# Genie-Kim/PintheMemory

Measured on AMD Instinct MI355X. Metric: train imgs/sec 768x768 bs=8 R50-DeepLabV3+ +mem, higher is better.
Workload: dtype f32

## Files before the change

### include/pinmem_hip.h

```cpp
#ifndef PINMEM_HIP_H
#define PINMEM_HIP_H
#include <stddef.h>
#include <stdint.h>

#ifdef __cplusplus
extern "C" {
#endif

typedef enum pm_status { PM_OK = 0, PM_EINVAL = -1, PM_EWORKSPACE = -2, PM_ELAUNCH = -3, PM_EUNSUPPORTED = -4 } pm_status;

typedef enum pm_dtype { PM_F32 = 0, PM_BF16 = 1 } pm_dtype;
#define PM_TF_ZERO_PAD64 1

typedef struct pm_tensor {
  void* ptr;
  int32_t n, h, w, c;
  int64_t pitch;
  int32_t dtype;
  int32_t flags;
} pm_tensor;

#define PM_ABI_VERSION 400

typedef struct pm_conv_params {
// ... 11 lines not shown
  int64_t struct_size;
  const float* bias;
  const float* scale;
  const float* shift;
  const float* residual;
  int64_t residual_pitch;
  int32_t relu;
  float* bn_partials;
  int64_t bn_partials_bytes;
} pm_conv_epilogue;

const char* pm_last_error(void);
int pm_version(void);

size_t pm_conv_workspace(const pm_tensor* x, const pm_tensor* y, const pm_conv_params* p, int which );
size_t pm_conv_winograd_v_bytes(const pm_tensor* x, const pm_tensor* y, const pm_conv_params* p);
size_t pm_conv_wxf_bytes(const pm_tensor* x, const pm_tensor* y, const pm_conv_params* p);
size_t pm_conv_wxf_bytes_dgrad(const pm_tensor* dy, const pm_tensor* dx, const pm_conv_params* p);
typedef struct pm_wxf_job {
  const float* w;
  void* wxf;
  int64_t wxf_bytes;
  int32_t cout, kh, kw, cin;
  int32_t dgrad;
  int32_t reserved;
} pm_wxf_job;
int pm_conv_wxf_refresh_bf16(const pm_wxf_job* jobs, int n, void* stream);
int pm_conv_wxf_refresh_f32(const pm_wxf_job* jobs, int n, void* stream);
size_t pm_conv_bn_partials_bytes(const pm_tensor* x, const pm_tensor* y, const pm_conv_params* p);
int pm_conv_fwd(const pm_tensor* x, const float* w_krsc, const pm_tensor* y, const pm_conv_params* p,
                const pm_conv_epilogue* ep, void* ws, size_t ws_bytes, void* stream);
int pm_conv_bwd_data(const pm_tensor* dy, const float* w_krsc, const pm_tensor* dx, const pm_conv_params* p,
                     const pm_tensor* add, void* ws, size_t ws_bytes, void* stream);
int pm_conv_bwd_weight(const pm_tensor* x, const pm_tensor* dy, float* dw_krsc, float* dbias, const pm_conv_params* p,
                       void* ws, size_t ws_bytes, void* stream);

typedef struct pm_routing {
  int32_t struct_size;
  int32_t winograd;
  int32_t winograd_fused;
  int32_t conv16;
  int32_t conv16_wide;
  int32_t conv16_persistent;
  int32_t wgrad16;
  int32_t bf16_wgrad;
  int32_t split;
} pm_routing;
int pm_routing_get(pm_routing* out);
int pm_routing_set(const pm_routing* r);


int pm_set_winograd(int mode);
int pm_set_winograd_fused(int on);
int pm_set_conv16(int on);
int pm_set_bf16_wgrad(int on);
int pm_set_wgrad16(int on);
int pm_set_split(int on);

int pm_profile_enable(int on);
int pm_profile_dump(const char* csv_path);
int pm_profile_read(int mode, int bm, int bn, int km, int nst, double* total_ms, double* total_flops, int64_t* launches, int clear);
int pm_profile_read_prec(int mode, int bm, int bn, int km, int nst, int prec, double* total_ms, double* total_flops, int64_t* launches, int clear);
int pm_profile_read_bytes(int mode, int bm, int bn, int km, int nst, int prec, double* total_bytes);

size_t pm_bn_workspace(const pm_tensor* x);
int pm_bn_stats(const pm_tensor* x, float* moments, void* ws, size_t ws_bytes, void* stream);
int pm_bn_stats_finalize(const pm_tensor* x, float eps, float* mean, float* invstd, float* running_mean , float* running_var ,
                         float momentum, void* ws, size_t ws_bytes, void* stream);
int pm_bn_merge(const float* parts, int world, int c, float* moments, void* stream);
int pm_bn_merge_finalize(const float* parts, int world, int c, float eps, float* mean, float* invstd, float* running_mean ,
                         float* running_var , float momentum, void* stream);
int pm_bn_finalize(const float* moments, int c, float eps, float* mean, float* invstd,
                   float* running_mean, float* running_var, float momentum, void* stream);
int pm_bn_apply(const pm_tensor* x, const float* mean, const float* invstd, const float* gamma, const float* beta,
                const pm_tensor* residual , int relu, const pm_tensor* y, void* stream);
int pm_bn_apply_mask(const pm_tensor* x, const float* mean, const float* invstd, const float* gamma, const float* beta,
                     const pm_tensor* residual , int relu, const pm_tensor* y, uint8_t* mask , void* stream);
int pm_bn_bwd_reduce_mask(const pm_tensor* dy, const uint8_t* mask, const pm_tensor* x, const float* mean, const float* invstd,
                          const pm_tensor* gmask , float* sums, void* ws, size_t ws_bytes, void* stream);
int pm_bn_bwd_reduce(const pm_tensor* dy, const pm_tensor* y , const pm_tensor* x, const float* mean, const float* invstd,
                     const float* gamma , const float* beta , int relu, const pm_tensor* gmask ,
                     float* sums, void* ws, size_t ws_bytes, void* stream);
int pm_bn_bwd_apply(const pm_tensor* dy, const pm_tensor* y , const pm_tensor* x, const float* mean, const float* invstd,
                    const float* gamma, const float* beta , const float* sums, float count, int relu, const pm_tensor* dx,
                    const pm_tensor* dres , void* stream);
int pm_bn_partials_finalize(const float* partials, int64_t pixels, int c, float eps, float* mean, float* invstd, float* running_mean ,
                            float* running_var , float momentum, float* moments , void* stream);
int pm_bn_fold(const float* gamma, const float* beta, const float* running_mean, const float* running_var, const float* conv_bias,
               int c, float eps, float* scale, float* shift, void* stream);
int pm_bn_fold_multi(const void* table, const int* cs, const int* offs, int n, int max_c, int total, float eps, float* arena, void* stream);
int pm_relu_bwd(const pm_tensor* dy, const pm_tensor* y, const pm_tensor* dx, void* stream);
int pm_add(const pm_tensor* a, const pm_tensor* b, const pm_tensor* y, void* stream);
int pm_add_n(const pm_tensor* const* xs, int n, const pm_tensor* y, void* stream);
int pm_copy(const pm_tensor* src, const pm_tensor* dst, void* stream);
int pm_scale_shift_act(const pm_tensor* x, const float* scale, const float* shift, const pm_tensor* residual, int relu,
                       const pm_tensor* y, void* stream);

int pm_cast(const pm_tensor* x, const pm_tensor* y, void* stream);

int pm_maxpool3x3s2_fwd(const pm_tensor* x, const pm_tensor* y, uint8_t* argmax, void* stream);
int pm_maxpool3x3s2_bwd(const pm_tensor* dy, const uint8_t* argmax, const pm_tensor* dx, void* stream);
int pm_global_avgpool_fwd(const pm_tensor* x, const pm_tensor* y , void* stream);
int pm_global_avgpool_bwd(const pm_tensor* dy, const pm_tensor* dx, int accumulate, void* stream);

int pm_resize_bilinear_fwd(const pm_tensor* x, const pm_tensor* y, void* stream);
int pm_resize_bilinear_bwd(const pm_tensor* dy, const pm_tensor* dx, int accumulate, void* stream);
size_t pm_resize_bilinear_bwd_workspace(const pm_tensor* dy, const pm_tensor* dx);
int pm_resize_bilinear_bwd_separable(const pm_tensor* dy, const pm_tensor* dx, int accumulate, void* ws, size_t ws_bytes, void* stream);

int pm_resize_bilinear_hp_fwd(const pm_tensor* x, const pm_tensor* y, int flip_w, void* stream);
int pm_softmax_mean_update(const pm_tensor* logits, double* buffer, int counter, void* stream);
int pm_sliding_stitch(const pm_tensor* logits, const int32_t* tiles_xyxy, int ntiles, int H, int W, int flip_w, double* acc, int accumulate, void* stream);
int pm_argmax_f64(const double* buffer, int n, int h, int w, int c, int64_t* out_cls, double* out_prob , void* stream);

int pm_image_u8_to_nhwc4(const uint8_t* img_nhw3, int64_t pixels, const float* mean3, const float* std3, float* out_nhwc4, void* stream);
int pm_labels_u8_to_i64(const uint8_t* lab, int64_t n, int64_t* out, void* stream);

int pm_nchw_to_nhwc(const float* x_nchw, int c_src, const pm_tensor* y, void* stream);
int pm_nhwc_to_nchw(const pm_tensor* x, float* y_nchw, void* stream);
int pm_label_nearest(const int64_t* lab, int n, int H, int W, int64_t* out, int h, int w, void* stream);

size_t pm_upsample_ce_workspace(int n, int H, int W);
int pm_upsample_ce_fwd(const pm_tensor* logits, float inv_temp, const int64_t* labels, int H, int W, float* loss_out,
                       void* ws, size_t ws_bytes, void* stream);
size_t pm_upsample_ce_bwd_workspace(const pm_tensor* logits, int H, int W);
int pm_upsample_ce_bwd(const pm_tensor* logits, float inv_temp, const int64_t* labels, int H, int W, const float* loss_out,
                       const float* gscale, const pm_tensor* dlogits, void* ws, size_t ws_bytes, void* stream);

size_t pm_upsample_ce_field_bytes(const pm_tensor* logits, int H, int W);
int pm_upsample_ce_fwd_field(const pm_tensor* logits, float inv_temp, const int64_t* labels, int H, int W, float* loss_out, float* field,
                             void* ws , size_t ws_bytes, void* stream);
int pm_upsample_ce_bwd_field(const pm_tensor* logits , float inv_temp, int H, int W, const float* loss_out, const float* gscale,
                             const float* field, const pm_tensor* dlogits, void* stream);

// ... 52 lines not shown
```

### pinthememory_amd/csrc/bn.hip

```cpp
#include "pm_common.h"

namespace {

constexpr int CB = 64;
constexpr int RL = 16;

__device__ __forceinline__ float bn_affine(float v, float mu, float is, float ga, float be) {
  const float s = is * ga;
  return fmaf(v, s, fmaf(-mu, s, be));
}

inline int chunk_rows(long P, int C) {
  const long colblocks = std::max<long>(1, (C + CB - 1) / CB);
  const long want = std::max<long>(512, 2048 / colblocks);
  long r = (P + want - 1) / want;
  r = std::max<long>(r, 64);
  return (int)((r + RL - 1) / RL * RL);
}

__global__ __launch_bounds__(256) void bn_stats_partial(const float* __restrict__ x, long pitch, long P, int C, int rows, float* __restrict__ part) {
  __shared__ float sm[RL][CB][2];
  const int g = threadIdx.x & 15, r = threadIdx.x >> 4;
  const int c = blockIdx.y * CB + g * 4;
  const long p0 = (long)blockIdx.x * rows, p1 = min(P, p0 + rows);
  float s1[4] = {0, 0, 0, 0}, s2[4] = {0, 0, 0, 0};
  if (c < C) {
    const float4 k = PM_LD4(x + c);
    for (long p = p0 + r; p < p1; p += RL) {
      const float4 v = PM_LD4(x + p * pitch + c);
      const float d0 = v.x - k.x, d1 = v.y - k.y, d2 = v.z - k.z, d3 = v.w - k.w;
      s1[0] += d0, s1[1] += d1, s1[2] += d2, s1[3] += d3;
      s2[0] += d0 * d0, s2[1] += d1 * d1, s2[2] += d2 * d2, s2[3] += d3 * d3;
    }
  }
#pragma unroll
  for (int j = 0; j < 4; ++j) sm[r][g * 4 + j][0] = s1[j], sm[r][g * 4 + j][1] = s2[j];
  __syncthreads();
  if (threadIdx.x < CB * 2) {
    const int cc = threadIdx.x >> 1, w = threadIdx.x & 1;
    float s = 0.f;
#pragma unroll
    for (int i = 0; i < RL; ++i) s += sm[i][cc][w];
    const int ch = blockIdx.y * CB + cc;
// ... 107 lines not shown
    float4 ga = make_float4(0.f, 0.f, 0.f, 0.f), be = ga;
    if (RELU == 2) ga = PM_LD4(gamma + c), be = PM_LD4(beta + c);
    for (long p = p0 + r; p < p1; p += RL) {
      float4 d = PM_LD4(dy + p * dpitch + c);
      const float4 v = PM_LD4(x + p * xpitch + c);
      if (RELU == 1) {
        const float4 o = PM_LD4(y + p * ypitch + c);
        d.x = o.x > 0.f ? d.x : 0.f, d.y = o.y > 0.f ? d.y : 0.f, d.z = o.z > 0.f ? d.z : 0.f, d.w = o.w > 0.f ? d.w : 0.f;
      } else if (RELU == 3) {
        const unsigned mb = reinterpret_cast<const unsigned char*>(y)[p * (C >> 2) + (c >> 2)];
        d.x = (mb & 1u) ? d.x : 0.f, d.y = (mb & 2u) ? d.y : 0.f, d.z = (mb & 4u) ? d.z : 0.f, d.w = (mb & 8u) ? d.w : 0.f;
      } else if (RELU == 2) {
        d.x = bn_affine(v.x, mu.x, is.x, ga.x, be.x) > 0.f ? d.x : 0.f, d.y = bn_affine(v.y, mu.y, is.y, ga.y, be.y) > 0.f ? d.y : 0.f;
        d.z = bn_affine(v.z, mu.z, is.z, ga.z, be.z) > 0.f ? d.z : 0.f, d.w = bn_affine(v.w, mu.w, is.w, ga.w, be.w) > 0.f ? d.w : 0.f;
      }
      if (GOUT) PM_ST4(gout + p * gpitch + c, d);
      s1[0] += d.x, s1[1] += d.y, s1[2] += d.z, s1[3] += d.w;
      s2[0] += d.x * ((v.x - mu.x) * is.x), s2[1] += d.y * ((v.y - mu.y) * is.y);
      s2[2] += d.z * ((v.z - mu.z) * is.z), s2[3] += d.w * ((v.w - mu.w) * is.w);
    }
  }
#pragma unroll
  for (int j = 0; j < 4; ++j) sm[r][g * 4 + j][0] = s1[j], sm[r][g * 4 + j][1] = s2[j];
  __syncthreads();
  if (threadIdx.x < CB * 2) {
    const int cc = threadIdx.x >> 1, w = threadIdx.x & 1;
    float s = 0.f;
#pragma unroll
    for (int i = 0; i < RL; ++i) s += sm[i][cc][w];
    const int ch = blockIdx.y * CB + cc;
    if (ch < C) part[((long)blockIdx.x * C + ch) * 2 + w] = s;
  }
}
__global__ __launch_bounds__(256) void bn_bwd_final(const float* __restrict__ part, int nb, int C, float* __restrict__ sums) {
  const int c = blockIdx.x * FC + (threadIdx.x & (FC - 1)), lane = threadIdx.x / FC;
  double s1, s2;
  final_sums(part, nb, C, c, lane, s1, s2);
  if (lane != 0 || c >= C) return;
  sums[c] = (float)s1;
  sums[C + c] = (float)s2;
}

template <bool FIN>
__global__ void bn_merge_kernel(const float* __restrict__ parts, int W, int C, float* __restrict__ out, float eps, float* __restrict__ mean,
                                float* __restrict__ invstd, float* running_mean, float* running_var, float momentum) {
  const int c = blockIdx.x * blockDim.x + threadIdx.x;
  if (c >= C) return;
  double n = 0.0, s = 0.0;
  for (int r = 0; r < W; ++r) {
    const double cnt = parts[(long)r * 3 * C + 2 * C + c];
    n += cnt, s += cnt * (double)parts[(long)r * 3 * C + c];
  }
  const double gmean = s / n;
  double m2d = 0.0;
  for (int r = 0; r < W; ++r) {
    const double cnt = parts[(long)r * 3 * C + 2 * C + c], d = (double)parts[(long)r * 3 * C + c] - gmean;
    m2d += (double)parts[(long)r * 3 * C + C + c] + cnt * d * d;
  }
  const float m = (float)gmean, m2 = (float)m2d, nf = (float)n;
  if constexpr (!FIN) {
    out[c] = m, out[C + c] = m2, out[2 * C + c] = nf;
  } else {
    const float var = m2 / nf;
    mean[c] = m;
    invstd[c] = 1.f / sqrtf(var + eps);
    if (running_mean) running_mean[c] = (1.f - momentum) * running_mean[c] + momentum * m;
// ... 96 lines not shown
extern "C" int pm_bn_partials_finalize(const float* partials, int64_t pixels, int c, float eps, float* mean, float* invstd, float* running_mean,
                                       float* running_var, float momentum, float* moments, void* stream) {
  PM_REQUIRE(partials && pixels > 0 && c > 0 && (moments || (mean && invstd)), PM_EINVAL, "bn_partials_finalize: bad args");
  PM_REQUIRE(moments || pixels > 1, PM_EINVAL, "bn_partials_finalize: expected more than 1 value per channel when training, got %ld", (long)pixels);
  hipStream_t st = (hipStream_t)stream;
  if (moments)
    hipLaunchKernelGGL(bn_partials_final<true>, dim3(pm_cdiv(c, FC)), dim3(256), 0, st, partials, (long)pixels, c, eps, (float*)nullptr, (float*)nullptr,
                       (float*)nullptr, (float*)nullptr, 0.f, moments);
  else
    hipLaunchKernelGGL(bn_partials_final<false>, dim3(pm_cdiv(c, FC)), dim3(256), 0, st, partials, (long)pixels, c, eps, mean, invstd, running_mean, running_var,
                       momentum, (float*)nullptr);
  return pm_check_launch("bn_partials_finalize");
}

extern "C" int pm_bn_fold(const float* gamma, const float* beta, const float* rm, const float* rv, const float* conv_bias, int c, float eps, float* scale,
                          float* shift, void* stream) {
  PM_REQUIRE(gamma && beta && rm && rv && scale && shift && c > 0, PM_EINVAL, "bn_fold: bad args");
  hipLaunchKernelGGL(bn_fold_kernel, dim3(pm_cdiv(c, 64)), dim3(64), 0, (hipStream_t)stream, gamma, beta, rm, rv, conv_bias, c, eps, scale, shift);
  return pm_check_launch("bn_fold");
}

extern "C" int pm_bn_fold_multi(const void* table, const int* cs, const int* offs, int n, int max_c, int total, float eps, float* arena, void* stream) {
  PM_REQUIRE(table && cs && offs && arena && n > 0 && max_c > 0 && total > 0, PM_EINVAL, "bn_fold_multi: bad args");
  hipLaunchKernelGGL(bn_fold_multi_kernel, dim3(n, pm_cdiv(max_c, 256)), dim3(256), 0, (hipStream_t)stream, (const unsigned long long*)table, cs, offs, total, eps,
                     arena);
  return pm_check_launch("bn_fold_multi");
}

extern "C" int pm_bn_apply(const pm_tensor* x, const float* mean, const float* invstd, const float* gamma, const float* beta, const pm_tensor* res,
                           int relu, const pm_tensor* y, void* stream) {
  return pm_bn_apply_mask(x, mean, invstd, gamma, beta, res, relu, y, nullptr, stream);
}

extern "C" int pm_bn_apply_mask(const pm_tensor* x, const float* mean, const float* invstd, const float* gamma, const float* beta, const pm_tensor* res,
                                int relu, const pm_tensor* y, uint8_t* mask, void* stream) {
  PM_REQUIRE(x && y, PM_EINVAL, "bn_apply: null");
  if (pm_is_bf16(x)) return pm16_bn_apply_mask(x, mean, invstd, gamma, beta, res, relu, y, mask, (hipStream_t)stream);
  if (int e = check_bn(x, "bn_apply")) return e;
  if (int e = check_bn(y, "bn_apply")) return e;
  PM_REQUIRE(pm_same_shape(x, y) && mean && invstd && gamma && beta, PM_EINVAL, "bn_apply: bad args");
  if (res) {
    if (int e = check_bn(res, "bn_apply")) return e;
    PM_REQUIRE(pm_same_shape(x, res), PM_EINVAL, "bn_apply: residual shape mismatch");
  }
  const float *px = (const float*)x->ptr, *pr = res ? (const float*)res->ptr : nullptr;
  float* py = (float*)y->ptr;
  const long a = x->pitch, b = res ? res->pitch : 0, c = y->pitch, cq = x->c >> 2;
  return pm_ew_launch(true, pm_pixels(x), x->c, (hipStream_t)stream, "bn_apply", [=] __device__(long p, int ch) {
    const float4 v = PM_LD4(px + p * a + ch), mu = PM_LD4(mean + ch), is = PM_LD4(invstd + ch), ga = PM_LD4(gamma + ch), be = PM_LD4(beta + ch);
    float4 o = make_float4(bn_affine(v.x, mu.x, is.x, ga.x, be.x), bn_affine(v.y, mu.y, is.y, ga.y, be.y), bn_affine(v.z, mu.z, is.z, ga.z, be.z),
                           bn_affine(v.w, mu.w, is.w, ga.w, be.w));
    if (pr) {
      const float4 q = PM_LD4(pr + p * b + ch);
      o.x += q.x, o.y += q.y, o.z += q.z, o.w += q.w;
    }
    if (mask) mask[p * cq + (ch >> 2)] = (unsigned char)((o.x > 0.f ? 1 : 0) | (o.y > 0.f ? 2 : 0) | (o.z > 0.f ? 4 : 0) | (o.w > 0.f ? 8 : 0));
    if (relu) o.x = fmaxf(o.x, 0.f), o.y = fmaxf(o.y, 0.f), o.z = fmaxf(o.z, 0.f), o.w = fmaxf(o.w, 0.f);
    PM_ST4(py + p * c + ch, o);
  });
}

extern "C" int pm_bn_bwd_reduce(const pm_tensor* dy, const pm_tensor* y, const pm_tensor* x, const float* mean, const float* invstd, const float* gamma,
                                const float* beta, int relu, const pm_tensor* gmask, float* sums, void* ws, size_t ws_bytes, void* stream) {
  PM_REQUIRE(dy && x, PM_EINVAL, "bn_bwd_reduce: null");
  PM_REQUIRE(relu >= 0 && relu <= 2, PM_EINVAL, "bn_bwd_reduce: relu mode %d (0 none, 1 mask from y, 2 mask rebuilt from x)", relu);
  if (pm_is_bf16(x)) return pm16_bn_bwd_reduce(dy, y, nullptr, x, mean, invstd, gamma, beta, relu, gmask, sums, ws, ws_bytes, (hipStream_t)stream);
  if (int e = check_bn(dy, "bn_bwd_reduce")) return e;
  if (int e = check_bn(x, "bn_bwd_reduce")) return e;
  PM_REQUIRE(pm_same_shape(dy, x) && mean && invstd && sums, PM_EINVAL, "bn_bwd_reduce: bad args");
  PM_REQUIRE(relu >= 0 && relu <= 2, PM_EINVAL, "bn_bwd_reduce: relu mode %d (0 none, 1 mask from y, 2 mask rebuilt from x)", relu);
  PM_REQUIRE(relu != 1 || (y && pm_vec4(y) && pm_same_shape(y, x)), PM_EINVAL, "bn_bwd_reduce: relu mode 1 needs the forward output");
  PM_REQUIRE(relu != 2 || (gamma && beta), PM_EINVAL, "bn_bwd_reduce: relu mode 2 needs gamma and beta");
  PM_REQUIRE(!gmask || (relu != 0 && pm_vec4(gmask) && pm_same_shape(gmask, x)), PM_EINVAL, "bn_bwd_reduce: gmask needs a ReLU mode and the shape of x");
  PM_REQUIRE(ws && ws_bytes >= pm_bn_workspace(x), PM_EWORKSPACE, "bn_bwd_reduce: workspace too small");
  const long P = pm_pixels(x);
  const int rows = chunk_rows(P, x->c), nb = pm_cdiv(P, rows);
  hipStream_t st = (hipStream_t)stream;
  dim3 grid(nb, pm_cdiv(x->c, CB));
  const float *pdy = (const float*)dy->ptr, *py = relu == 1 ? (const float*)y->ptr : nullptr, *px = (const float*)x->ptr;
  const long yp = relu == 1 ? y->pitch : 0;
  float* pg = gmask ? (float*)gmask->ptr : nullptr;
  const long gp = gmask ? gmask->pitch : 0;
#define PM_BN_BWD_PARTIAL(R, G)                                                                                                                         \
  hipLaunchKernelGGL((bn_bwd_partial<R, G>), grid, dim3(256), 0, st, pdy, (long)dy->pitch, py, yp, px, (long)x->pitch, mean, invstd, gamma, beta, pg, gp, P, \
                     x->c, rows, (float*)ws)
  if (relu == 0) PM_BN_BWD_PARTIAL(0, false);
  else if (relu == 1 && gmask) PM_BN_BWD_PARTIAL(1, true);
  else if (relu == 1) PM_BN_BWD_PARTIAL(1, false);
  else if (gmask) PM_BN_BWD_PARTIAL(2, true);
  else PM_BN_BWD_PARTIAL(2, false);
#undef PM_BN_BWD_PARTIAL
  hipLaunchKernelGGL(bn_bwd_final, dim3(pm_cdiv(x->c, FC)), dim3(256), 0, st, (const float*)ws, nb, x->c, sums);
// ... 37 lines not shown
  PM_REQUIRE(relu != 1 || (y && pm_vec4(y) && pm_same_shape(y, x)), PM_EINVAL, "bn_bwd_apply: relu mode 1 needs the forward output");
  PM_REQUIRE(relu != 2 || beta, PM_EINVAL, "bn_bwd_apply: relu mode 2 needs beta");
  PM_REQUIRE(!dres || (pm_vec4(dres) && pm_same_shape(dres, x)), PM_EINVAL, "bn_bwd_apply: dres shape mismatch");
  const float *pd = (const float*)dy->ptr, *po = relu == 1 ? (const float*)y->ptr : nullptr, *px = (const float*)x->ptr;
  float *pdx = (float*)dx->ptr, *pdr = dres ? (float*)dres->ptr : nullptr;
  const long a = dy->pitch, b = relu == 1 ? y->pitch : 0, c = x->pitch, d = dx->pitch, e2 = dres ? dres->pitch : 0;
  const bool from_x = relu == 2;
  const int C = x->c;
  const bool dev_count = !(count > 0.f);
  const float host_inv_n = dev_count ? 0.f : 1.f / count;
  return pm_ew_launch(true, pm_pixels(x), C, (hipStream_t)stream, "bn_bwd_apply", [=] __device__(long p, int ch) {
    const float inv_n = dev_count ? 1.f / sums[2 * C] : host_inv_n;
    float4 g = PM_LD4(pd + p * a + ch);
    if (po) {
      const float4 o = PM_LD4(po + p * b + ch);
      g.x = o.x > 0.f ? g.x : 0.f, g.y = o.y > 0.f ? g.y : 0.f, g.z = o.z > 0.f ? g.z : 0.f, g.w = o.w > 0.f ? g.w : 0.f;
    }
    const float4 v = PM_LD4(px + p * c + ch), mu = PM_LD4(mean + ch), is = PM_LD4(invstd + ch), ga = PM_LD4(gamma + ch);
    if (from_x) {
      const float4 be = PM_LD4(beta + ch);
      g.x = bn_affine(v.x, mu.x, is.x, ga.x, be.x) > 0.f ? g.x : 0.f, g.y = bn_affine(v.y, mu.y, is.y, ga.y, be.y) > 0.f ? g.y : 0.f;
      g.z = bn_affine(v.z, mu.z, is.z, ga.z, be.z) > 0.f ? g.z : 0.f, g.w = bn_affine(v.w, mu.w, is.w, ga.w, be.w) > 0.f ? g.w : 0.f;
    }
    if (pdr) PM_ST4(pdr + p * e2 + ch, g);
    const float4 s1 = PM_LD4(sums + ch), s2 = PM_LD4(sums + C + ch);
    float4 r;
    r.x = (g.x - s1.x * inv_n - (v.x - mu.x) * is.x * (s2.x * inv_n)) * (is.x * ga.x);
    r.y = (g.y - s1.y * inv_n - (v.y - mu.y) * is.y * (s2.y * inv_n)) * (is.y * ga.y);
    r.z = (g.z - s1.z * inv_n - (v.z - mu.z) * is.z * (s2.z * inv_n)) * (is.z * ga.z);
    r.w = (g.w - s1.w * inv_n - (v.w - mu.w) * is.w * (s2.w * inv_n)) * (is.w * ga.w);
    PM_ST4(pdx + p * d + ch, r);
  });
}
```

### pinthememory_amd/csrc/conv_igemm.hip

```cpp
#include <stdlib.h>
#include <algorithm>
#include <type_traits>
#include <vector>

#include "pm_common.h"

#include "conv_igemm_kernel.h"

namespace {

template <int ZL, bool O16 = false>
__global__ __launch_bounds__(256) void splitk_reduce_vec_kernel(const float* __restrict__ ws, int ksplit, long slab, int M, int Nn,
                                                                float* __restrict__ C, long c_pitch, const float* bias,
                                                                const float* scale, const float* shift, const float* residual,
                                                                long res_pitch, int relu) {
  constexpr int GP = 256 / ZL;
  __shared__ float4 red[ZL > 1 ? ZL : 1][GP];
  const int gl = threadIdx.x % GP, zl = threadIdx.x / GP;
  const long groups = (long)M * Nn / 4;
  for (long g0 = (long)blockIdx.x * GP; g0 < groups; g0 += (long)gridDim.x * GP) {
    const long grp = g0 + gl;
    float4 v = make_float4(0.f, 0.f, 0.f, 0.f);
    if (grp < groups)
#pragma unroll 8
      for (int z = zl; z < ksplit; z += ZL) {
        const float4 q = PM_LD4(ws + (long)z * slab + grp * 4);
        v.x += q.x, v.y += q.y, v.z += q.z, v.w += q.w;
      }
    if constexpr (ZL > 1) {
      red[zl][gl] = v;
      __syncthreads();
      if (zl == 0) {
#pragma unroll
        for (int l = 1; l < ZL; ++l) {
          const float4 q = red[l][gl];
          v.x += q.x, v.y += q.y, v.z += q.z, v.w += q.w;
        }
      }
    }
    if (zl == 0 && grp < groups) {
      const long i = grp * 4;
      const int row = (int)(i / Nn), col = (int)(i - (long)row * Nn);
      if (bias) {
        const float4 b = PM_LD4(bias + col);
        v.x += b.x, v.y += b.y, v.z += b.z, v.w += b.w;
      }
      if (scale) {
        const float4 sc = PM_LD4(scale + col), sh = PM_LD4(shift + col);
        v.x = v.x * sc.x + sh.x, v.y = v.y * sc.y + sh.y, v.z = v.z * sc.z + sh.z, v.w = v.w * sc.w + sh.w;
      }
      if (residual) {
        if constexpr (O16) {
          const uint2 q = *reinterpret_cast<const uint2*>(reinterpret_cast<const pm_bf16*>(residual) + (long)row * res_pitch + col);
          v.x += __uint_as_float(q.x << 16), v.y += __uint_as_float(q.x & 0xffff0000u), v.z += __uint_as_float(q.y << 16), v.w += __uint_as_float(q.y & 0xffff0000u);
        } else {
          const float4 r = PM_LD4(residual + (long)row * res_pitch + col);
          v.x += r.x, v.y += r.y, v.z += r.z, v.w += r.w;
        }
      }
      if (relu) v.x = fmaxf(v.x, 0.f), v.y = fmaxf(v.y, 0.f), v.z = fmaxf(v.z, 0.f), v.w = fmaxf(v.w, 0.f);
      if constexpr (O16) *reinterpret_cast<uint2*>(reinterpret_cast<pm_bf16*>(C) + (long)row * c_pitch + col) = make_uint2(pm_pack_bf16(v.x, v.y), pm_pack_bf16(v.z, v.w));
      else PM_ST4(C + (long)row * c_pitch + col, v);
    }
    if constexpr (ZL > 1) __syncthreads();
  }
}

__global__ __launch_bounds__(256) void splitk_reduce_kernel(const float* __restrict__ ws, int ksplit, long slab, int M, int Nn,
                                                            float* __restrict__ C, long c_pitch, const float* bias,
                                                            const float* scale, const float* shift, const float* residual,
                                                            long res_pitch, int relu) {
  const long total = (long)M * Nn;
  for (long i = (long)blockIdx.x * 256 + threadIdx.x; i < total; i += (long)gridDim.x * 256) {
    const int row = (int)(i / Nn), col = (int)(i - (long)row * Nn);
    float v = 0.f;
    for (int z = 0; z < ksplit; ++z) v += ws[(long)z * slab + i];
    if (bias) v += bias[col];
    if (scale) v = v * scale[col] + shift[col];
    if (residual) v += residual[(long)row * res_pitch + col];
    if (relu) v = fmaxf(v, 0.f);
    C[(long)row * c_pitch + col] = v;
  }
}

int splitk_reduce(const float* ws, int ksplit, long M, long Nn, float* C, long c_pitch, const float* bias, const float* scale, const float* shift,
                  const float* residual, long res_pitch, int relu, hipStream_t st, bool out16 = false) {
  const long total = M * Nn;
  if (out16) {
    PM_REQUIRE((Nn % 4 == 0) && (c_pitch % 4 == 0) && (res_pitch % 4 == 0) && pm_aligned16(ws) && (reinterpret_cast<uintptr_t>(C) & 7) == 0 &&
                   (reinterpret_cast<uintptr_t>(residual) & 7) == 0 && (!bias || pm_aligned16(bias)) && (!scale || (pm_aligned16(scale) && pm_aligned16(shift))),
               PM_EUNSUPPORTED, "splitk_reduce(bf16): unaligned output");
    const long groups = total / 4;
    const int zl = (ksplit >= 32 && groups < (1 << 18)) ? 16 : (ksplit >= 8 && groups < (1 << 20) ? 4 : 1);
    const int nb = (int)std::min<long>((groups + 256 / zl - 1) / (256 / zl), 8192);
    if (zl == 16)
      hipLaunchKernelGGL((splitk_reduce_vec_kernel<16, true>), dim3(nb), dim3(256), 0, st, ws, ksplit, total, (int)M, (int)Nn, C, c_pitch, bias, scale, shift, residual, res_pitch, relu);
    else if (zl == 4)
      hipLaunchKernelGGL((splitk_reduce_vec_kernel<4, true>), dim3(nb), dim3(256), 0, st, ws, ksplit, total, (int)M, (int)Nn, C, c_pitch, bias, scale, shift, residual, res_pitch, relu);
    else
      hipLaunchKernelGGL((splitk_reduce_vec_kernel<1, true>), dim3(nb), dim3(256), 0, st, ws, ksplit, total, (int)M, (int)Nn, C, c_pitch, bias, scale, shift, residual, res_pitch, relu);
    return pm_check_launch("splitk_reduce(bf16)");
  }
  const bool vec = (Nn % 4 == 0) && (c_pitch % 4 == 0) && (res_pitch % 4 == 0) && pm_aligned16(ws) && pm_aligned16(C) &&
                   (!bias || pm_aligned16(bias)) && (!scale || (pm_aligned16(scale) && pm_aligned16(shift))) && (!residual || pm_aligned16(residual));
  if (!vec) {
    const int nb = (int)std::min<long>((total + 255) / 256, 4096);
    hipLaunchKernelGGL(splitk_reduce_kernel, dim3(nb), dim3(256), 0, st, ws, ksplit, total, (int)M, (int)Nn, C, c_pitch, bias, scale, shift, residual,
                       res_pitch, relu);
  } else {
    const long groups = total / 4;
    const int zl = (ksplit >= 32 && groups < (1 << 18)) ? 16 : (ksplit >= 8 && groups < (1 << 20) ? 4 : 1);
    const int gp = 256 / zl;
    const int nb = (int)std::min<long>((groups + gp - 1) / gp, 8192);
    if (zl == 16)
      hipLaunchKernelGGL(splitk_reduce_vec_kernel<16>, dim3(nb), dim3(256), 0, st, ws, ksplit, total, (int)M, (int)Nn, C, c_pitch, bias, scale, shift, residual, res_pitch, relu);
    else if (zl == 4)
      hipLaunchKernelGGL(splitk_reduce_vec_kernel<4>, dim3(nb), dim3(256), 0, st, ws, ksplit, total, (int)M, (int)Nn, C, c_pitch, bias, scale, shift, residual, res_pitch, relu);
    else
      hipLaunchKernelGGL(splitk_reduce_vec_kernel<1>, dim3(nb), dim3(256), 0, st, ws, ksplit, total, (int)M, (int)Nn, C, c_pitch, bias, scale, shift, residual, res_pitch, relu);
  }
  return pm_check_launch("splitk_reduce");
}

inline int colsum_rows(long P, int C) {
  const long col_blocks = std::max<long>(1, (C + 63) / 64);
  const long want = col_blocks == 1 ? 256 : std::max<long>(1, 1024 / col_blocks);
  return (int)std::min<long>(2048, std::max<long>(64, (P + want - 1) / want));
}

__global__ __launch_bounds__(256) void colsum_partial_kernel(const float* __restrict__ x, long pitch, long P, int C, int rows_per_block,
                                                             float* __restrict__ part) {
  __shared__ float sm[4][64];
  const int c = blockIdx.y * 64 + (threadIdx.x & 63), r = threadIdx.x >> 6;
  const long p0 = (long)blockIdx.x * rows_per_block, p1 = min(P, p0 + rows_per_block);
  float s = 0.f;
  if (c < C)
    for (long p = p0 + r; p < p1; p += 4) s += x[p * pitch + c];
  sm[r][threadIdx.x & 63] = s;
  __syncthreads();
  if (r == 0 && c < C) part[(long)blockIdx.x * C + c] = sm[0][threadIdx.x] + sm[1][threadIdx.x] + sm[2][threadIdx.x] + sm[3][threadIdx.x];
}
__global__ __launch_bounds__(256) void colsum_partial_narrow_kernel(const float* __restrict__ x, int p4, long P, int C, int rows_per_block,
                                                                    float* __restrict__ part) {
  __shared__ float4 sm[256];
  const int RL = 256 / p4, t = threadIdx.x;
  const int g = t % p4, rl = t / p4;
  const long p0 = (long)blockIdx.x * rows_per_block, p1 = min(P, p0 + rows_per_block);
  float4 s = make_float4(0.f, 0.f, 0.f, 0.f);
  if (rl < RL)
    for (long p = p0 + rl; p < p1; p += RL) {
      const float4 v = PM_LD4(x + (p * p4 + g) * 4);
      s.x += v.x, s.y += v.y, s.z += v.z, s.w += v.w;
// ... 193 lines not shown
  }
  void done() {
    if (!g_prof_on) return;
    (void)hipEventRecord(rec.b, st);
    g_prof.push_back(rec);
  }
};

inline bool split_takes(int mode, const Plan& p, const ConvK& k, int batch) {
  return pm_route.split != 0 && p.bn >= 64 && !k.io16 && (batch > 1 || split_k_ok(mode, k.K));
}

template <int MODE>
int launch(const ConvK& k0, const Plan& p, hipStream_t st, int batch = 1, double flops = -1.0) {
  ConvK k = k0;
  k.tiles_m = p.tiles_m;
  k.tiles_n = p.tiles_n;
  k.ksplit = p.ksplit;
  k.kper = p.kper;
  dim3 grid(p.tiles_m * p.tiles_n, batch, p.ksplit);
  if (batch != 1) k.stage_ep = 0;
  if (k.prec == 0 && split_takes(MODE, p, k, batch)) k.prec = 5;
  {
    const int units = batch * p.ksplit, rem = units & 7, ntile = p.tiles_m * p.tiles_n;
    k.batch_xcd = units >= 8 && (rem == 0 || ((rem == 1 || rem == 2 || rem == 4) && ntile % (8 / rem) == 0));
  }
  const int km = (MODE == MODE_WGRAD && k.kmode == K_FAST) ? K_MID : ((k.prec == 5 && MODE != MODE_WGRAD && k.kmode == K_FAST && k.kh * k.kw == 1 && k.stride == 1 && k.pad == 0 && !k.sub) ? K_PW : k.kmode);
  ProfScope prof(st, MODE, p.bm, p.bn, km, k.prec, lds_stages(MODE, k.kmode, p.bn, k.kper), k.M, k.Nn, k.K, batch, p.ksplit,
                 flops >= 0.0 ? flops : 2.0 * (double)k.M * (double)k.Nn * (double)k.K * batch,
                 (double)batch * ((double)k.a_bytes + (double)k.b_bytes + ((k.io16 && p.ksplit == 1) ? 2.0 : 4.0) * (double)k.M * (double)k.Nn * (double)p.ksplit));
  if constexpr (MODE != MODE_WGRAD) {
    if (pm_route.split && (k.prec == 0 || k.prec == 5) && !k.io16 && batch == 1 && p.ksplit == 1 && !k.stats && k.kh * k.kw == 1 && k.stride == 1 && k.pad == 0 && !k.sub) {
      pm_gemm_pw g;
      g.A = k.A, g.B = k.B, g.C = k.C, g.bias = k.bias, g.scale = k.scale, g.shift = k.shift, g.residual = k.residual;
      g.a_pitch = MODE == MODE_FWD ? k.x_pitch : k.y_pitch, g.c_pitch = k.c_pitch, g.res_pitch = k.res_pitch;
      g.b_sn = MODE == MODE_FWD ? k.K : 1, g.b_sk = MODE == MODE_FWD ? 1 : k.Nn;
      g.M = k.M, g.Nn = k.Nn, g.K = k.K, g.relu = k.relu;
      if (pm_pwstream_ok(&g)) {
        prof.rec.bm = 32, prof.rec.bn = 64, prof.rec.km = 4, prof.rec.prec = 5, prof.rec.nst = 0;
        const int e = pm_pwstream_launch(&g, st);
        prof.done();
        return e;
      }
    }
  }
  constexpr bool akc = MODE != MODE_WGRAD, bkc = MODE == MODE_FWD;
  if (k.prec == 5) {
    if (int e = pm_conv_split_launch(MODE, p.bm, p.bn, k, grid.x, grid.y, grid.z, pm_conv_split_stage_bytes(MODE, p.bm, p.bn), st)) return e;
    prof.rec.nst = 1;
    prof.done();
    return pm_check_launch("conv_split");
  }
  const bool tr = MODE == MODE_WGRAD && (k.prec == 3 || k.prec == 4) && p.bn >= 64;
  auto smem = [&](int bm, int bn) {
    if (tr) return (size_t)2 * ((k.prec == 4 ? 2 : 1) * BK * (bm + 32) + (k.prec == 4 ? 2 : 1) * BK * (bn + 32)) * 2;
    return (size_t)2 * ((akc ? bm * LDK : BK * bm) + (bkc ? bn * LDK : BK * bn)) * sizeof(float);
  };
  if (p.bm == 64) {
    if (p.bn == 128) launch_one<MODE, 64, 128, 2, 2>(k, grid, smem(64, 128), st);
    else launch_one<MODE, 64, 64, 2, 2>(k, grid, smem(64, 64), st);
  } else if (p.bn == 128) {
    launch_one<MODE, 128, 128, 2, 2>(k, grid, smem(128, 128), st);
  } else if (p.bn == 64) {
    launch_one<MODE, 128, 64, 2, 2>(k, grid, smem(128, 64), st);
  } else {
    launch_one<MODE, 128, 32, 4, 1>(k, grid, smem(128, 32), st);
  }
// ... 2 lines not shown
}

int check_common(const pm_tensor* x, const pm_tensor* y, const pm_conv_params* p) {
  PM_REQUIRE(x && y && p && x->ptr && y->ptr, PM_EINVAL, "conv: null tensor");
  PM_REQUIRE(p->struct_size == (int32_t)sizeof(pm_conv_params), PM_EINVAL, "conv: pm_conv_params.struct_size %d != %zu -- caller built against another pinmem_hip.h (library ABI %d)",
             p->struct_size, sizeof(pm_conv_params), PM_ABI_VERSION);
  PM_REQUIRE(p->kh >= 1 && p->kw >= 1 && p->dil >= 1 && p->pad >= 0, PM_EINVAL, "conv: bad geometry");
  PM_REQUIRE(p->stride == 1 || p->stride == 2, PM_EUNSUPPORTED, "conv: stride %d unsupported (1 or 2)", p->stride);
  const int ho = (x->h + 2 * p->pad - p->dil * (p->kh - 1) - 1) / p->stride + 1;
  const int wo = (x->w + 2 * p->pad - p->dil * (p->kw - 1) - 1) / p->stride + 1;
  PM_REQUIRE(ho == y->h && wo == y->w && x->n == y->n, PM_EINVAL, "conv: output %dx%d does not match geometry (%dx%d)", y->h, y->w, ho, wo);
  PM_REQUIRE((x->dtype == PM_F32 || x->dtype == PM_BF16) && (y->dtype == PM_F32 || y->dtype == PM_BF16), PM_EUNSUPPORTED, "conv: dtype %d / %d", x->dtype, y->dtype);
  for (const pm_tensor* t : {x, y}) {
    if (pm_is_bf16(t)) PM_REQUIRE(pm_vec8(t), PM_EINVAL, "conv: bf16 tensors must be 16B aligned with pitch %% 8 == 0 and channels %% 8 == 0");
    else PM_REQUIRE(pm_vec_ok(t), PM_EINVAL, "conv: tensors must be 16B aligned with pitch %% 4 == 0");
  }
  PM_REQUIRE(x->c % 4 == 0, PM_EUNSUPPORTED, "conv: Cin %% 4 != 0 unsupported (pad the input channels)");
  PM_REQUIRE((y->c % 4 == 0) || (p->kh * p->kw == 1), PM_EUNSUPPORTED, "conv: Cout %% 4 != 0 only for 1x1");
  PM_REQUIRE(x->pitch >= x->c && y->pitch >= y->c, PM_EINVAL, "conv: pitch < channels");
  PM_REQUIRE(pm_pixels(x) * x->pitch < (1ll << 29) && pm_pixels(y) * y->pitch < (1ll << 29) && (int64_t)y->c * x->c * p->kh * p->kw < (1ll << 29),
             PM_EUNSUPPORTED, "conv: tensor too large for 32-bit byte offsets (2 GiB per tensor)");
  return PM_OK;
}

void fill_geom(ConvK& k, const pm_tensor* x, const pm_tensor* y, const pm_conv_params* p) {
  k.N = x->n, k.H = x->h, k.W = x->w, k.Cin = x->c, k.x_pitch = x->pitch;
  k.Ho = y->h, k.Wo = y->w, k.Cout = y->c, k.y_pitch = y->pitch;
  k.kh = p->kh, k.kw = p->kw, k.stride = p->stride, k.pad = p->pad, k.dil = p->dil;
  k.sshift = p->stride == 2 ? 1 : 0;
  k.prec = p->prec != 0 ? 1 : 0;
  k.T_eff = p->kh * p->kw, k.tk_w = p->kw, k.ky0 = k.kx0 = 0, k.ksy = k.ksx = 1;
  k.sub = k.sub_cy = k.sub_cx = 0, k.Hc = x->h, k.Wc = x->w;
  k.bias = k.scale = k.shift = k.residual = nullptr;
  k.res_pitch = 0, k.relu = 0, k.stats = nullptr, k.io16 = 0;
  k.stage_ep = 1;
  k.spl_prio = 1;
  k.n_group = 8;
  k.batch_xcd = 0;
  k.a_bs = k.b_bs = k.c_bs = 0;
}

struct WinoPlan {
  bool use;
  pm_wino_geom g;
  int Kp, P;
  size_t v_bytes, m_bytes, u_bytes;
  Plan pl;
};
inline bool wino_wgrad_pays(int cin, int cout) { return (long)cin * cout >= 256 * 256; }
WinoPlan wino_plan(const pm_tensor* xin, int cout, const pm_conv_params* p, bool wgrad = false) {
  WinoPlan wp{};
  if (wgrad && !wino_wgrad_pays(xin->c, cout)) return wp;
  if (pm_route.winograd == 0 || p->kh != 3 || p->kw != 3 || p->stride != 1 || p->pad != p->dil || p->prec != 0) return wp;
  const int cin = xin->c;
  if (cin < 128 || cout < 128 || (cout & 3) || (cin & 3)) return wp;
  int m = 0;
  double best_ratio = 0.6;
  for (int cand = pm_route.winograd; cand >= 2; cand -= 2) {
    const pm_wino_geom g = pm_wino_make_geom(xin->n, xin->h, xin->w, p->dil, cand);
    const double cover = (double)(cand * g.TY * p->dil) * (double)(cand * g.TX * p->dil) / ((double)xin->h * xin->w);
    const double ratio = cover * (cand + 2) * (cand + 2) / (9.0 * cand * cand);
    if (ratio <= best_ratio) best_ratio = ratio, m = cand, wp.g = g;
  }
  if (!m) return wp;
  wp.P = (m + 2) * (m + 2);
  wp.Kp = (cin + BK - 1) / BK * BK;
  if (wp.g.tiles * (long)std::max(wp.Kp, cout) * 4 >= (1ll << 31)) return wp;
// ... 463 lines not shown

int dgrad_s2_parity(const pm_tensor* dy0, const float* w, const pm_tensor* dx, const pm_conv_params* p, const pm_tensor* add, const ConvRoute& r, void* ws, hipStream_t st) {
  pm_tensor dy32;
  if (int e = upcast(dy0, (char*)ws + r.dy32_off, &dy32, st)) return e;
  const pm_tensor* dy = &dy32;
  float* tmp = (float*)((char*)ws + r.class_off);
  float* slab = (float*)((char*)ws + r.slab_off);
  for (int cls = 0; cls < 4; ++cls) {
    if (!r.s2p.valid[cls]) continue;
    const S2Class& c = r.s2p.c[cls];
    const Plan& pl = r.s2p.pl[cls];
    ConvK k;
    fill_geom(k, dx, dy, p);
    k.A = (const float*)dy->ptr, k.B = w;
    k.M = (int)c.M, k.Nn = dx->c, k.K = c.nky * c.nkx * dy->c;
    k.a_bytes = (unsigned)(pm_pixels(dy) * dy->pitch * 4), k.b_bytes = (unsigned)((long)dy->c * p->kh * p->kw * dx->c * 4);
    k.kmode = dy->c >= BK ? K_MID : K_SMALL;
    k.T_eff = c.nky * c.nkx, k.tk_w = c.nkx, k.ky0 = c.ky0, k.kx0 = c.kx0, k.ksy = c.ksy, k.ksx = c.ksx;
    k.sub = 1, k.sub_cy = c.cy, k.sub_cx = c.cx, k.Hc = c.Hc, k.Wc = c.Wc;
    float* out = (float*)((char*)tmp + cls * r.s2p.tmp_bytes);
    if (pl.ksplit > 1) {
      k.C = slab, k.c_pitch = dx->c, k.c_split = c.M * dx->c;
      if (int e = launch<MODE_DGRAD>(k, pl, st)) return e;
      if (int e = splitk_reduce(slab, pl.ksplit, c.M, dx->c, out, (long)dx->c, nullptr, nullptr, nullptr, nullptr, 0l, 0, st)) return e;
    } else {
      k.C = out, k.c_pitch = dx->c, k.c_split = 0;
      if (int e = launch<MODE_DGRAD>(k, pl, st)) return e;
    }
  }
  return s2_interleave(tmp, (long)(r.s2p.tmp_bytes / sizeof(float)), r.s2p.valid, dx, add, st, "dgrad_s2_interleave");
}

template <int MODE>
int conv_direct(const pm_tensor* x, const pm_tensor* y, const float* w, const pm_conv_params* p, const Plan& pl, const pm_conv_epilogue& e, void* ws, hipStream_t st) {
  const pm_tensor *xin = MODE == MODE_FWD ? x : y, *out = MODE == MODE_FWD ? y : x;
  long M, Nn, K;
  gemm_dims(MODE, x, y, p, M, Nn, K);
  ConvK k;
  fill_geom(k, x, y, p);
  k.io16 = pm_is_bf16(out) ? 1 : 0;
  k.A = (const float*)xin->ptr, k.B = w;
  k.M = (int)M, k.Nn = (int)Nn, k.K = (int)K;
  k.a_bytes = (unsigned)(pm_pixels(xin) * xin->pitch * 4), k.b_bytes = (unsigned)((long)y->c * p->kh * p->kw * x->c * 4);
  k.kmode = (xin->c % BK == 0 && (MODE == MODE_FWD || p->stride == 1)) ? 0 : (xin->c >= BK ? 1 : 2);
  if (pl.ksplit > 1) {
    k.C = (float*)ws, k.c_pitch = Nn, k.c_split = M * Nn;
    if (int err = launch<MODE>(k, pl, st)) return err;
    return splitk_reduce((const float*)ws, pl.ksplit, M, Nn, (float*)out->ptr, (long)out->pitch, e.bias, e.scale, e.shift, e.residual, (long)e.residual_pitch, e.relu, st, k.io16 != 0);
  }
  k.C = (float*)out->ptr, k.c_pitch = out->pitch, k.c_split = 0;
  k.bias = e.bias, k.scale = e.scale, k.shift = e.shift, k.residual = e.residual, k.res_pitch = e.residual_pitch, k.relu = e.relu;
  k.stats = e.bn_partials;
  return launch<MODE>(k, pl, st);
}

int conv_wgrad_direct(const pm_tensor* x, const pm_tensor* dy, float* dw, const pm_conv_params* p, const ConvRoute& r, void* ws, hipStream_t st) {
  long M, Nn, K;
  gemm_dims(MODE_WGRAD, x, dy, p, M, Nn, K);
  if (r.w16.use) {
    pm_wgrad16 w16 = r.w16.k;
    w16.C = w16.ksplit > 1 ? (float*)ws : dw;
    ProfScope prof(st, MODE_WGRAD, w16.bm, w16.bn, 2, 4, 3, M, Nn, K, 1, w16.ksplit, 2.0 * (double)M * (double)Nn * (double)K);
    const int e = pm_wgrad16_launch(&w16, st);
    prof.done();
    if (e || w16.ksplit == 1) return e;
    return splitk_reduce((const float*)ws, w16.ksplit, M, Nn, dw, (long)Nn, nullptr, nullptr, nullptr, nullptr, 0l, 0, st);
  }
  ConvK k;
  fill_geom(k, x, dy, p);
  if (p->prec == 2) k.prec = 3;
  if (r.native16) {
    PM_REQUIRE(x->c % 8 == 0 && dy->c % 8 == 0 && r.pl.bn >= 64, PM_EUNSUPPORTED, "conv_bwd_weight(bf16): channels %% 8 != 0 or a tile narrower than 64");
    k.prec = 4;
  }
  const int esz = r.native16 ? 2 : 4;
  k.A = (const float*)dy->ptr, k.B = (const float*)x->ptr;
  k.M = (int)M, k.Nn = (int)Nn, k.K = (int)K;
  k.a_bytes = (unsigned)(pm_pixels(dy) * dy->pitch * esz), k.b_bytes = (unsigned)(pm_pixels(x) * x->pitch * esz), k.kmode = dy->w >= (r.native16 ? 2 * BK : BK) ? 1 : 2;
  k.C = r.pl.ksplit > 1 ? (float*)ws : dw, k.c_pitch = Nn, k.c_split = r.pl.ksplit > 1 ? M * Nn : 0;
  if (int e = launch<MODE_WGRAD>(k, r.pl, st)) return e;
  if (r.pl.ksplit == 1) return PM_OK;
  return splitk_reduce((const float*)ws, r.pl.ksplit, M, Nn, dw, (long)Nn, nullptr, nullptr, nullptr, nullptr, 0l, 0, st);
}

// ... 165 lines not shown
  const pm_conv_params* p = &tp;
  PM_REQUIRE(!ep || ep->struct_size == (int64_t)sizeof(pm_conv_epilogue), PM_EINVAL,
             "conv_fwd: pm_conv_epilogue.struct_size %ld != %zu -- caller built against another pinmem_hip.h (library ABI %d)", ep ? (long)ep->struct_size : 0l,
             sizeof(pm_conv_epilogue), PM_ABI_VERSION);
  PM_REQUIRE(w && pm_aligned16(w), PM_EINVAL, "conv_fwd: weight null or unaligned");
  pm_conv_epilogue e0 = {(int64_t)sizeof(pm_conv_epilogue), nullptr, nullptr, nullptr, nullptr, 0, 0};
  if (ep) e0 = *ep;
  PM_REQUIRE((e0.scale == nullptr) == (e0.shift == nullptr), PM_EINVAL, "conv_fwd: scale and shift go together");
  const ConvRoute r = route_conv(MODE_FWD, x, y, p);
  if (e0.bn_partials) {
    PM_REQUIRE(!e0.relu && !e0.residual, PM_EINVAL, "conv_fwd: bn_partials are the statistics of the convolution output (no residual / ReLU)");
    PM_REQUIRE(r.bn_bytes != 0 && (size_t)e0.bn_partials_bytes >= r.bn_bytes, PM_EINVAL, "conv_fwd: this call cannot emit bn_partials (ask pm_conv_bn_partials_bytes): %zu needed", r.bn_bytes);
  }
  PM_REQUIRE(ws_bytes >= r.ws_bytes && (ws || r.ws_bytes == 0), PM_EWORKSPACE, "conv_fwd: workspace %zu < %zu", ws_bytes, r.ws_bytes);
  hipStream_t st = (hipStream_t)stream;
  switch (r.kind) {
    case R_WINO: {
      float* keep = (p->wino_v && (size_t)p->wino_v_bytes >= r.wino.v_bytes) ? (float*)p->wino_v : nullptr;
      float* uext = (p->wxf && (size_t)p->wxf_bytes >= r.wino.u_bytes) ? (float*)p->wxf : nullptr;
      return wino_conv(x, w, y->c, x->c, false, y, r.wino, e0, ws, st, keep, uext, p->wxf_valid != 0);
    }
    case R_BF16: {
      char* wext = (p->wxf && (size_t)p->wxf_bytes >= r.b16.wb_bytes) ? (char*)p->wxf : nullptr;
      return conv_bf16(x, w, y->c, x->c, false, y, &r.pe, r.b16, e0, ws, st, wext, p->wxf_valid != 0);
    }
    default:
      PM_REQUIRE(pm_is_f32(x), PM_EUNSUPPORTED, "conv_fwd: a bf16 input needs at least 32 channels (got %d)", x->c);
      return conv_direct<MODE_FWD>(x, y, w, p, r.pl, e0, ws, st);
  }
}

extern "C" int pm_conv_bwd_data(const pm_tensor* dy, const float* w, const pm_tensor* dx, const pm_conv_params* p0, const pm_tensor* add,
                                void* ws, size_t ws_bytes, void* stream) {
  if (int e = check_common(dx, dy, p0)) return e;
  const pm_conv_params tp = tier_params(p0, dy, dx);
  const pm_conv_params* p = &tp;
  PM_REQUIRE(!add || (add->ptr && pm_same_shape(add, dx) && add->dtype == dx->dtype), PM_EINVAL, "conv_bwd_data: `add` must match dx (shape and dtype)");
  PM_REQUIRE(!add || !pm_is_bf16(add) || pm_vec8(add), PM_EINVAL, "conv_bwd_data: bf16 `add` must be 16B aligned with pitch %% 8 == 0");
  PM_REQUIRE(w && pm_aligned16(w), PM_EINVAL, "conv_bwd_data: weight null or unaligned");
  const ConvRoute r = route_conv(MODE_DGRAD, dx, dy, p);
  PM_REQUIRE(ws_bytes >= r.ws_bytes && (ws || r.ws_bytes == 0), PM_EWORKSPACE, "conv_bwd_data: workspace %zu < %zu", ws_bytes, r.ws_bytes);
  hipStream_t st = (hipStream_t)stream;
  const pm_conv_epilogue e1 = {(int64_t)sizeof(pm_conv_epilogue), nullptr, nullptr, nullptr, add ? (const float*)add->ptr : nullptr, add ? add->pitch : 0, 0};
  switch (r.kind) {
    case R_S2_NATIVE: return dgrad_s2_bf16(dy, w, dx, p, add, r.s2n, ws, st);
    case R_S2_PARITY: return dgrad_s2_parity(dy, w, dx, p, add, r, ws, st);
    case R_BF16: {
      char* wext = (p->wxf && (size_t)p->wxf_bytes >= r.b16.wb_bytes) ? (char*)p->wxf : nullptr;
      return conv_bf16(dy, w, dy->c, dx->c, true, dx, &r.pe, r.b16, e1, ws, st, wext, p->wxf_valid != 0);
    }
    case R_WINO: return wino_conv(dy, w, dy->c, dx->c, true, dx, r.wino, e1, ws, st);
    default:
      PM_REQUIRE(pm_is_f32(dy), PM_EUNSUPPORTED, "conv_bwd_data: a bf16 dy needs at least 32 channels and a stride-1 geometry the forward form covers");
      return conv_direct<MODE_DGRAD>(dx, dy, w, p, r.pl, e1, ws, st);
  }
}

extern "C" int pm_conv_bwd_weight(const pm_tensor* x0, const pm_tensor* dy0, float* dw, float* dbias, const pm_conv_params* p0, void* ws,
                                  size_t ws_bytes, void* stream) {
  if (int e = check_common(x0, dy0, p0)) return e;
  const pm_conv_params tp = tier_params(p0, x0, dy0);
  const pm_conv_params* p = &tp;
  PM_REQUIRE(dw && pm_aligned16(dw), PM_EINVAL, "conv_bwd_weight: dw null or unaligned");
  const ConvRoute r = route_conv(MODE_WGRAD, x0, dy0, p);
  PM_REQUIRE(ws && ws_bytes >= r.ws_bytes, PM_EWORKSPACE, "conv_bwd_weight: workspace %zu < %zu", ws_bytes, r.ws_bytes);
  hipStream_t st = (hipStream_t)stream;
  const pm_tensor *x = x0, *dy = dy0;
  pm_tensor x32, dy32;
  if (!r.native16 && pm_is_bf16(x0)) {
    if (int e = upcast(x0, (char*)ws + r.x32_off, &x32, st)) return e;
    x = &x32;
  }
  if (pm_is_bf16(dy0) && (!r.native16 || dbias)) {
    if (int e = upcast(dy0, (char*)ws + r.dy32_off, &dy32, st)) return e;
    if (!r.native16) dy = &dy32;
  }
  int e;
  switch (r.kind) {
    case R_BF16_WGRAD: e = conv_wgrad_bf16(x, dy, dw, p, r.b16w, ws, st); break;
    case R_WINO_WGRAD: e = wino_wgrad(x, dy, dw, r.wino, r.wino_w, ws, st, (p->wino_v && (size_t)p->wino_v_bytes >= r.wino.v_bytes) ? (float*)p->wino_v : nullptr); break;
    default: e = conv_wgrad_direct(x, dy, dw, p, r, ws, st);
  }
  if (e || !dbias) return e;
  const pm_tensor* dyb = pm_is_bf16(dy0) ? &dy32 : dy0;
  const long P = pm_pixels(dyb);
  const int rpb = colsum_rows(P, dyb->c), nb = pm_cdiv(P, rpb);
  float* part = (float*)((char*)ws + r.bias_off);
// ... 8 lines not shown
```

### pinthememory_amd/csrc/conv_igemm_kernel.h

```cpp
#pragma once
#include <stdint.h>
#include <type_traits>

#include "pm_common.h"

typedef float f32x16 __attribute__((ext_vector_type(16)));
typedef __bf16 bf16x8 __attribute__((ext_vector_type(8)));

struct ConvK {
  const float* A;
  const float* B;
  float* C;
  int N, H, W, Cin;
  int Ho, Wo, Cout;
  long x_pitch, y_pitch;
  int kh, kw, stride, pad, dil, sshift;
  int M, Nn, K;
  int ksplit;
  int kper;
  long c_pitch;
  long c_split;
  long a_bs, b_bs, c_bs;
  int tiles_m, tiles_n;
  unsigned a_bytes, b_bytes;
  int kmode;
  int prec;
  int T_eff, tk_w, ky0, kx0, ksy, ksx;
  int sub, sub_cy, sub_cx, Hc, Wc;
  const float* bias;
  const float* scale;
  const float* shift;
  const float* residual;
  long res_pitch;
  int relu;
  float* stats;
  int io16;
  int stage_ep;
  int n_group;
  int batch_xcd;
  int spl_prio;
};

int pm_conv_split_launch(int mode, int bm, int bn, const ConvK& k, unsigned gx, unsigned gy, unsigned gz, size_t smem, hipStream_t st);
size_t pm_conv_split_stage_bytes(int mode, int bm, int bn);

namespace {

enum { MODE_FWD = 0, MODE_DGRAD = 1, MODE_WGRAD = 2 };
constexpr int BK = 32;
constexpr int LDK = 36;


typedef float v4f __attribute__((ext_vector_type(4)));
constexpr int OOB = 0x7fffffff;

__device__ __forceinline__ float4 bload(__amdgpu_buffer_rsrc_t r, int off) {
  const v4f v = __builtin_bit_cast(v4f, __builtin_amdgcn_raw_buffer_load_b128(r, off, 0, 0));
  return make_float4(v.x, v.y, v.z, v.w);
}

__device__ __forceinline__ int xcd_remap(int bid, int nwg) {
  const int q = nwg >> 3, r = nwg & 7, xcd = bid & 7, idx = bid >> 3;
  const int base = xcd < r ? xcd * (q + 1) : r * (q + 1) + (xcd - r) * q;
  return base + idx;
}

// ... 762 lines not shown
  const bool vec = a.stage_ep && ((a.c_pitch | a.Nn | (a.residual ? a.res_pitch : 0)) & 3) == 0 &&
                   ((reinterpret_cast<uintptr_t>(Cb) | reinterpret_cast<uintptr_t>(a.residual)) & 15) == 0;
  if (vec) {
    constexpr int WC = BN / WN, LDC = WC + 4, LPR = WC / 4, RPI = 64 / LPR;
    static_assert(32 % RPI == 0, "row segments must tile the 32-row slab");
    __syncthreads();
    float* Ws = smem + wave * 32 * LDC;
    const int rr0 = lane / LPR, cc = (lane % LPR) * 4;
    const int col = n0 + wn * WC + cc;
    const bool cok = col < a.Nn;
    const bool aff = !plain && (a.bias || a.scale), res = !plain && a.residual, relu = !plain && a.relu;
    float bi[4] = {0.f, 0.f, 0.f, 0.f}, sc[4] = {1.f, 1.f, 1.f, 1.f}, sh[4] = {0.f, 0.f, 0.f, 0.f};
    if (aff && cok) {
#pragma unroll
      for (int e = 0; e < 4; ++e) {
        if (a.bias) bi[e] = a.bias[col + e];
        if (a.scale) sc[e] = a.scale[col + e], sh[e] = a.shift[col + e];
      }
    }
#pragma unroll
    for (int i = 0; i < TM; ++i) {
#pragma unroll
      for (int n = 0; n < TN; ++n)
#pragma unroll
        for (int q = 0; q < 16; ++q) Ws[((q & 3) + 8 * (q >> 2) + 4 * half) * LDC + n * 32 + l31] = acc[i][n][q];
#pragma unroll
      for (int r0 = 0; r0 < 32; r0 += RPI) {
        const int rr = r0 + rr0;
        const long row = m0 + wm * (BM / WM) + i * 32 + rr;
        float4 v = *reinterpret_cast<const float4*>(Ws + rr * LDC + cc);
        if (row < a.M && cok) {
          if (aff) v.x = (v.x + bi[0]) * sc[0] + sh[0], v.y = (v.y + bi[1]) * sc[1] + sh[1], v.z = (v.z + bi[2]) * sc[2] + sh[2], v.w = (v.w + bi[3]) * sc[3] + sh[3];
          if (res) {
            const float4 qv = PM_LD4(a.residual + row * a.res_pitch + col);
            v.x += qv.x, v.y += qv.y, v.z += qv.z, v.w += qv.w;
          }
          if (relu) v.x = fmaxf(v.x, 0.f), v.y = fmaxf(v.y, 0.f), v.z = fmaxf(v.z, 0.f), v.w = fmaxf(v.w, 0.f);
          PM_ST4(Cb + row * a.c_pitch + col, v);
        }
      }
      if constexpr (STATS) {
        const long slab_row0 = m0 + wm * (BM / WM) + i * 32;
        const float cnt = (float)max(0l, min(32l, (long)a.M - slab_row0));
        auto slab_row = [&](int r0, bool& rok) {
          float4 v = *reinterpret_cast<const float4*>(Ws + (r0 + rr0) * LDC + cc);
          v.x = (v.x + bi[0]) * sc[0] + sh[0], v.y = (v.y + bi[1]) * sc[1] + sh[1], v.z = (v.z + bi[2]) * sc[2] + sh[2], v.w = (v.w + bi[3]) * sc[3] + sh[3];
          rok = slab_row0 + r0 + rr0 < a.M;
          return v;
        };
        float s1[4] = {0.f, 0.f, 0.f, 0.f};
#pragma unroll
        for (int r0 = 0; r0 < 32; r0 += RPI) {
          bool rok;
          const float4 v = slab_row(r0, rok);
          s1[0] += rok ? v.x : 0.f, s1[1] += rok ? v.y : 0.f, s1[2] += rok ? v.z : 0.f, s1[3] += rok ? v.w : 0.f;
        }
#pragma unroll
        for (int o = LPR; o < 64; o <<= 1)
#pragma unroll
          for (int e = 0; e < 4; ++e) s1[e] += __shfl_xor(s1[e], o, 64);
        float mu[4], m2[4] = {0.f, 0.f, 0.f, 0.f};
#pragma unroll
        for (int e = 0; e < 4; ++e) mu[e] = cnt > 0.f ? s1[e] / cnt : 0.f;
#pragma unroll
        for (int r0 = 0; r0 < 32; r0 += RPI) {
          bool rok;
          const float4 v = slab_row(r0, rok);
// ... 82 lines not shown
```

### pinthememory_amd/csrc/pm_common.h

```cpp
#pragma once
#include <hip/hip_runtime.h>
#include <algorithm>
#include <atomic>
#include <stdarg.h>
#include <stdint.h>
#include <stdio.h>

#include "../../include/pinmem_hip.h"

void pm_set_error(const char* fmt, ...);

#define PM_REQUIRE(cond, code, ...)      \
  do {                                   \
    if (!(cond)) {                       \
      pm_set_error(__VA_ARGS__);         \
      return (code);                     \
    }                                    \
  } while (0)

static inline int pm_check_launch(const char* what) {
  hipError_t e = hipGetLastError();
  if (e != hipSuccess) {
    pm_set_error("%s: launch failed: %s", what, hipGetErrorString(e));
    return PM_ELAUNCH;
// ... 77 lines not shown
  int relu;
  float* stats;
  int bm, bn, tiles_m, tiles_n, ksplit, ksteps_per;
  long c_split;
  int wide;
};
void pm_conv16_plan(pm_conv16* k);
int pm_conv16w_launch(const pm_conv16* k, hipStream_t st);
int pm_conv16w_persistent(const pm_conv16* k);
size_t pm_conv16_slab_bytes(const pm_conv16* k);
double pm_conv16_executed_fraction(const pm_conv16* k);
int pm_conv16_launch(const pm_conv16* k, hipStream_t st);

struct pm_wgrad16 {
  const pm_bf16* X;
  const pm_bf16* DY;
  float* C;
  int N, H, W, Ho, Wo;
  long x_pitch, dy_pitch;
  int Cin, Cout, kh, kw, stride, pad, dil;
  int M, Nn, P;
  int kper, ksplit;
  long c_split;
  int bm, bn, tiles_m, tiles_n;
};
bool pm_wgrad16_plan(pm_wgrad16* k);
int pm_wgrad16_launch(const pm_wgrad16* k, hipStream_t st);

struct pm_gemm_pw {
  const float* A;
  const float* B;
  float* C;
  const float *bias, *scale, *shift, *residual;
  long a_pitch, c_pitch, res_pitch;
  int b_sn, b_sk;
  long M;
  int Nn, K, relu;
};
bool pm_pwstream_ok(const pm_gemm_pw* g);
int pm_pwstream_launch(const pm_gemm_pw* g, hipStream_t st);

constexpr int PM_MAX_DEVICES = 64;
inline int pm_device_cus(int dev) {
  static std::atomic<int> cached[PM_MAX_DEVICES];
  const bool keep = dev >= 0 && dev < PM_MAX_DEVICES;
  int n = keep ? cached[dev].load(std::memory_order_relaxed) : 0;
  if (n > 0) return n;
  if (hipDeviceGetAttribute(&n, hipDeviceAttributeMultiprocessorCount, dev) != hipSuccess || n <= 0) n = 256;
  if (keep) cached[dev].store(n, std::memory_order_relaxed);
  return n;
}
struct pm_lds_optin {
  std::atomic<bool> done[PM_MAX_DEVICES] = {};
  int operator()(const void* kernel, int lds_bytes) {
    int dev = 0;
    if (hipGetDevice(&dev) != hipSuccess) dev = 0;
    const bool keep = dev >= 0 && dev < PM_MAX_DEVICES;
    if (!keep || !done[dev].load(std::memory_order_acquire)) {
      if (hipFuncSetAttribute(kernel, hipFuncAttributeMaxDynamicSharedMemorySize, lds_bytes) != hipSuccess) (void)hipGetLastError();
      else if (keep) done[dev].store(true, std::memory_order_release);
    }
    return pm_device_cus(dev);
  }
};

extern pm_routing pm_route;
// ... 34 lines not shown
  };
#pragma unroll
  for (int r0 = 0; r0 < 32; r0 += RPI) {
    float v[8];
    const bool rok = slab_row(r0, v);
#pragma unroll
    for (int e = 0; e < 8; ++e) s1[e] += rok ? v[e] : 0.f;
  }
#pragma unroll
  for (int o = LPR; o < 64; o <<= 1)
#pragma unroll
    for (int e = 0; e < 8; ++e) s1[e] += __shfl_xor(s1[e], o, 64);
#pragma unroll
  for (int e = 0; e < 8; ++e) mu[e] = cnt > 0.f ? s1[e] / cnt : 0.f;
#pragma unroll
  for (int r0 = 0; r0 < 32; r0 += RPI) {
    float v[8];
    const bool rok = slab_row(r0, v);
#pragma unroll
    for (int e = 0; e < 8; ++e) {
      const float d = v[e] - mu[e];
      m2[e] += rok ? d * d : 0.f;
    }
  }
#pragma unroll
  for (int o = LPR; o < 64; o <<= 1)
#pragma unroll
    for (int e = 0; e < 8; ++e) m2[e] += __shfl_xor(m2[e], o, 64);
  if (rr0 == 0 && cok && cnt > 0.f) {
    float* dst = stats + ((slab_row0 >> 5) * Nn + col) * 2;
#pragma unroll
    for (int e = 0; e < 8; e += 2) *reinterpret_cast<float4*>(dst + 2 * e) = make_float4(mu[e], m2[e], mu[e + 1], m2[e + 1]);
  }
}

__device__ __forceinline__ float pm_wave_sum(float v) {
#pragma unroll
  for (int o = 32; o > 0; o >>= 1) v += __shfl_xor(v, o, 64);
  return v;
}
__device__ __forceinline__ float pm_wave_max(float v) {
#pragma unroll
  for (int o = 32; o > 0; o >>= 1) v = fmaxf(v, __shfl_xor(v, o, 64));
  return v;
}

struct pm_lerp {
  int i0, i1;
  float w0, w1;
};
__host__ __device__ __forceinline__ float pm_ac_scale(int in, int out) {
  return out > 1 ? (float)(in - 1) / (float)(out - 1) : 0.f;
}
__device__ __forceinline__ pm_lerp pm_ac_lerp(float scale, int dst, int in) {
  float src = scale * (float)dst;
  int i0 = (int)src;
  if (i0 > in - 1) i0 = in - 1;
  int i1 = i0 + (i0 < in - 1 ? 1 : 0);
  float l1 = src - (float)i0;
  if (l1 < 0.f) l1 = 0.f;
  if (l1 > 1.f) l1 = 1.f;
  pm_lerp r;
  r.i0 = i0;
  r.i1 = i1;
  r.w1 = l1;
  r.w0 = 1.f - l1;
// ... 26 lines not shown
```

### pinthememory_amd/csrc/pool_resize.hip

```cpp
#include "pm_common.h"

namespace {

template <bool VEC>
__global__ __launch_bounds__(256) void maxpool_fwd_kernel(const float* __restrict__ x, long xp, int H, int W, float* __restrict__ y, long yp, int Ho,
                                                          int Wo, int C, long total, uint8_t* __restrict__ arg) {
  constexpr int V = VEC ? 4 : 1;
  const int cg = C / V;
  for (long i = (long)blockIdx.x * 256 + threadIdx.x; i < total; i += (long)gridDim.x * 256) {
    const long op = i / cg;
    const int ch = (int)(i - op * cg) * V;
    const int ox = (int)(op % Wo), oy = (int)((op / Wo) % Ho), n = (int)(op / ((long)Wo * Ho));
    float best[V];
    uint8_t bi[V];
#pragma unroll
    for (int v = 0; v < V; ++v) best[v] = -INFINITY, bi[v] = 0;
    bool first = true;
#pragma unroll
    for (int ky = 0; ky < 3; ++ky) {
      const int iy = oy * 2 - 1 + ky;
      if ((unsigned)iy >= (unsigned)H) continue;
#pragma unroll
      for (int kx = 0; kx < 3; ++kx) {
        const int ix = ox * 2 - 1 + kx;
        if ((unsigned)ix >= (unsigned)W) continue;
        const float* p = x + ((long)(n * H + iy) * W + ix) * xp + ch;
        float v[V];
        if constexpr (VEC) {
          const float4 q = PM_LD4(p);
          v[0] = q.x;
          if (V > 1) v[1 % V] = q.y, v[2 % V] = q.z, v[3 % V] = q.w;
        } else {
          v[0] = *p;
        }
#pragma unroll
        for (int e = 0; e < V; ++e)
          if (first || v[e] > best[e] || v[e] != v[e]) best[e] = v[e], bi[e] = (uint8_t)(ky * 3 + kx);
        first = false;
      }
    }
    float* o = y + op * yp + ch;
    uint8_t* a = arg + op * C + ch;
#pragma unroll
    for (int e = 0; e < V; ++e) o[e] = best[e], a[e] = bi[e];
  }
}

__global__ __launch_bounds__(256) void maxpool_bwd_vec_kernel(const float* __restrict__ dy, long dp, int Ho, int Wo, const uint8_t* __restrict__ arg,
                                                              float* __restrict__ dx, long xp, int H, int W, int C, long total) {
  const int cg = C >> 2;
  for (long i = (long)blockIdx.x * 256 + threadIdx.x; i < total; i += (long)gridDim.x * 256) {
    const long ip = i / cg;
    const int ch = (int)(i - ip * cg) * 4;
    const int ix = (int)(ip % W), iy = (int)((ip / W) % H), n = (int)(ip / ((long)W * H));
    float4 g = make_float4(0.f, 0.f, 0.f, 0.f);
    const int oy_hi = min((iy + 1) >> 1, Ho - 1), ox_hi = min((ix + 1) >> 1, Wo - 1);
    for (int oy = iy >> 1; oy <= oy_hi; ++oy) {
      const int ky = iy + 1 - 2 * oy;
      if (ky < 0 || ky > 2) continue;
      for (int ox = ix >> 1; ox <= ox_hi; ++ox) {
        const int kx = ix + 1 - 2 * ox;
        if (kx < 0 || kx > 2) continue;
        const long op = (long)(n * Ho + oy) * Wo + ox;
        const unsigned a = *reinterpret_cast<const unsigned*>(arg + op * C + ch), want = (unsigned)(ky * 3 + kx);
        const float4 d = PM_LD4(dy + op * dp + ch);
        g.x += (a & 255u) == want ? d.x : 0.f;
        g.y += ((a >> 8) & 255u) == want ? d.y : 0.f;
        g.z += ((a >> 16) & 255u) == want ? d.z : 0.f;
        g.w += (a >> 24) == want ? d.w : 0.f;
      }
    }
    PM_ST4(dx + ip * xp + ch, g);
  }
}

__global__ __launch_bounds__(256) void maxpool_bwd_kernel(const float* __restrict__ dy, long dp, int Ho, int Wo, const uint8_t* __restrict__ arg,
                                                          float* __restrict__ dx, long xp, int H, int W, int C, long total) {
  for (long i = (long)blockIdx.x * 256 + threadIdx.x; i < total; i += (long)gridDim.x * 256) {
    const long ip = i / C;
    const int ch = (int)(i - ip * C);
    const int ix = (int)(ip % W), iy = (int)((ip / W) % H), n = (int)(ip / ((long)W * H));
    float g = 0.f;
    const int oy_hi = min((iy + 1) >> 1, Ho - 1), ox_hi = min((ix + 1) >> 1, Wo - 1);
    for (int oy = max(iy >> 1, 0); oy <= oy_hi; ++oy) {
      const int ky = iy + 1 - 2 * oy;
      if (ky < 0 || ky > 2) continue;
      for (int ox = max(ix >> 1, 0); ox <= ox_hi; ++ox) {
        const int kx = ix + 1 - 2 * ox;
        if (kx < 0 || kx > 2) continue;
        const long op = (long)(n * Ho + oy) * Wo + ox;
        if (arg[op * C + ch] == (uint8_t)(ky * 3 + kx)) g += dy[op * dp + ch];
      }
    }
    dx[ip * xp + ch] = g;
  }
}

__global__ __launch_bounds__(256) void gap_fwd_kernel(const float* __restrict__ x, long xp, long HW, int C, float* __restrict__ y, long yp, float scale,
                                                      int accumulate) {
  __shared__ float sm[16][64];
  const int g = threadIdx.x & 15, r = threadIdx.x >> 4;
  const int c = blockIdx.y * 64 + g * 4, n = blockIdx.x;
  float s[4] = {0, 0, 0, 0};
  if (c < C) {
// ... 221 lines not shown
    for (int Y = ylo; Y <= yhi; ++Y) {
      const float wy = tap_weight(pm_ac_lerp(sy, Y, h), y);
      if (wy == 0.f) continue;
      const float4 q = PM_LD4(T + (((long)n * H + Y) * w + x) * C + ch);
      g.x += wy * q.x, g.y += wy * q.y, g.z += wy * q.z, g.w += wy * q.w;
    }
    float* o = dx + ip * xp + ch;
    if (accumulate) {
      const float4 q = PM_LD4(o);
      g.x += q.x, g.y += q.y, g.z += q.z, g.w += q.w;
    }
    PM_ST4(o, g);
  }
}

}

extern "C" int pm_maxpool3x3s2_fwd(const pm_tensor* x, const pm_tensor* y, uint8_t* argmax, void* stream) {
  PM_REQUIRE(x && y && argmax && x->ptr && y->ptr, PM_EINVAL, "maxpool_fwd: null");
  PM_REQUIRE(y->h == (x->h + 2 - 3) / 2 + 1 && y->w == (x->w + 2 - 3) / 2 + 1 && x->n == y->n && x->c == y->c, PM_EINVAL, "maxpool_fwd: shape mismatch");
  if (pm_is_bf16(x) && pm_is_bf16(y)) return pm16_maxpool_fwd(x, y, argmax, (hipStream_t)stream);
  PM_REQUIRE_F32(x, "maxpool_fwd"); PM_REQUIRE_F32(y, "maxpool_fwd");
  const bool v = pm_vec4(x) && pm_vec4(y);
  const long total = pm_pixels(y) * (v ? y->c / 4 : y->c);
  if (v)
    hipLaunchKernelGGL(maxpool_fwd_kernel<true>, dim3(grid_for(total)), dim3(256), 0, (hipStream_t)stream, (const float*)x->ptr, (long)x->pitch, x->h, x->w,
                       (float*)y->ptr, (long)y->pitch, y->h, y->w, y->c, total, argmax);
  else
    hipLaunchKernelGGL(maxpool_fwd_kernel<false>, dim3(grid_for(total)), dim3(256), 0, (hipStream_t)stream, (const float*)x->ptr, (long)x->pitch, x->h, x->w,
                       (float*)y->ptr, (long)y->pitch, y->h, y->w, y->c, total, argmax);
  return pm_check_launch("maxpool_fwd");
}

extern "C" int pm_maxpool3x3s2_bwd(const pm_tensor* dy, const uint8_t* argmax, const pm_tensor* dx, void* stream) {
  PM_REQUIRE(dy && dx && argmax && dy->ptr && dx->ptr && dy->n == dx->n && dy->c == dx->c, PM_EINVAL, "maxpool_bwd: bad args");
  if (pm_is_bf16(dy) && pm_is_bf16(dx)) return pm16_maxpool_bwd(dy, argmax, dx, (hipStream_t)stream);
  PM_REQUIRE_F32(dy, "maxpool_bwd"); PM_REQUIRE_F32(dx, "maxpool_bwd");
  const long total = pm_pixels(dx) * dx->c;
  if (pm_vec4(dy) && pm_vec4(dx) && (reinterpret_cast<uintptr_t>(argmax) & 3u) == 0)
    hipLaunchKernelGGL(maxpool_bwd_vec_kernel, dim3(grid_for(total / 4)), dim3(256), 0, (hipStream_t)stream, (const float*)dy->ptr, (long)dy->pitch, dy->h, dy->w,
                       argmax, (float*)dx->ptr, (long)dx->pitch, dx->h, dx->w, dx->c, total / 4);
  else
    hipLaunchKernelGGL(maxpool_bwd_kernel, dim3(grid_for(total)), dim3(256), 0, (hipStream_t)stream, (const float*)dy->ptr, (long)dy->pitch, dy->h, dy->w, argmax,
                       (float*)dx->ptr, (long)dx->pitch, dx->h, dx->w, dx->c, total);
  return pm_check_launch("maxpool_bwd");
}

extern "C" int pm_global_avgpool_fwd(const pm_tensor* x, const pm_tensor* y, void* stream) {
  PM_REQUIRE(x && y && y->ptr && y->h == 1 && y->w == 1 && y->n == x->n && y->c == x->c, PM_EINVAL, "global_avgpool_fwd: bad args");
  if (pm_is_bf16(x) && pm_is_bf16(y)) return pm16_gap_fwd(x, y, (hipStream_t)stream);
  PM_REQUIRE_F32(x, "global_avgpool_fwd"); PM_REQUIRE_F32(y, "global_avgpool_fwd");
  PM_REQUIRE(pm_vec4(x), PM_EINVAL, "global_avgpool_fwd: bad args");
  hipLaunchKernelGGL(gap_fwd_kernel, dim3(x->n, pm_cdiv(x->c, 64)), dim3(256), 0, (hipStream_t)stream, (const float*)x->ptr, (long)x->pitch,
                     (long)x->h * x->w, x->c, (float*)y->ptr, (long)y->pitch, 1.f / (float)((long)x->h * x->w), 0);
  return pm_check_launch("global_avgpool_fwd");
}

extern "C" int pm_global_avgpool_bwd(const pm_tensor* dy, const pm_tensor* dx, int accumulate, void* stream) {
  PM_REQUIRE(dy && dx && dy->ptr && dy->h == 1 && dy->w == 1 && dy->n == dx->n && dy->c == dx->c, PM_EINVAL, "global_avgpool_bwd: bad args");
  if (pm_is_bf16(dy) && pm_is_bf16(dx)) return pm16_gap_bwd(dy, dx, accumulate, (hipStream_t)stream);
  PM_REQUIRE_F32(dy, "global_avgpool_bwd"); PM_REQUIRE_F32(dx, "global_avgpool_bwd");
  PM_REQUIRE(pm_vec4(dx), PM_EINVAL, "global_avgpool_bwd: bad args");
  const float* pd = (const float*)dy->ptr;
  float* px = (float*)dx->ptr;
  const long dp = dy->pitch, xp = dx->pitch, HW = (long)dx->h * dx->w;
  const float inv = 1.f / (float)HW;
// ... 135 lines not shown
```

### pinthememory_amd/csrc/pwstream.hip

```cpp
#include <hip/hip_runtime.h>

#include <algorithm>

#include "pm_common.h"

namespace {

typedef float f32x16 __attribute__((ext_vector_type(16)));
typedef __bf16 bf16x8 __attribute__((ext_vector_type(8)));
typedef float v4f __attribute__((ext_vector_type(4)));

struct PwsK {
  const float* A;
  const float* B;
  float* C;
  const float *bias, *scale, *shift, *residual;
  long a_pitch, c_pitch, res_pitch;
  unsigned a_bytes, c_bytes, res_bytes;
  int b_sn, b_sk;
  int M, Nn, row_tiles, relu;
};

__device__ __forceinline__ v4f pws_load(__amdgpu_buffer_rsrc_t r, unsigned off) {
  return __builtin_bit_cast(v4f, __builtin_amdgcn_raw_buffer_load_b128(r, (int)off, 0, 0));
}

__device__ __forceinline__ void pws_split4(const v4f& v, unsigned* hi, unsigned* mid, unsigned* lo) {
  const unsigned u0 = __float_as_uint(v.x), u1 = __float_as_uint(v.y), u2 = __float_as_uint(v.z), u3 = __float_as_uint(v.w);
  hi[0] = __builtin_amdgcn_perm(u1, u0, 0x07060302), hi[1] = __builtin_amdgcn_perm(u3, u2, 0x07060302);
  const float r0 = v.x - __uint_as_float(u0 & 0xffff0000u), r1 = v.y - __uint_as_float(u1 & 0xffff0000u);
  const float r2 = v.z - __uint_as_float(u2 & 0xffff0000u), r3 = v.w - __uint_as_float(u3 & 0xffff0000u);
  const unsigned q0 = __float_as_uint(r0), q1 = __float_as_uint(r1), q2 = __float_as_uint(r2), q3 = __float_as_uint(r3);
  mid[0] = __builtin_amdgcn_perm(q1, q0, 0x07060302), mid[1] = __builtin_amdgcn_perm(q3, q2, 0x07060302);
  const float s0 = r0 - __uint_as_float(q0 & 0xffff0000u), s1 = r1 - __uint_as_float(q1 & 0xffff0000u);
  const float s2 = r2 - __uint_as_float(q2 & 0xffff0000u), s3 = r3 - __uint_as_float(q3 & 0xffff0000u);
  lo[0] = __builtin_amdgcn_perm(__float_as_uint(s1), __float_as_uint(s0), 0x07060302);
  lo[1] = __builtin_amdgcn_perm(__float_as_uint(s3), __float_as_uint(s2), 0x07060302);
}

template <int KG, int NB>
__global__ __launch_bounds__(256, 2) void pwstream_kernel(PwsK a) {
  extern __shared__ __attribute__((aligned(16))) char lds[];
  const int t = threadIdx.x, lane = t & 63, wave = __builtin_amdgcn_readfirstlane(t >> 6), l31 = lane & 31, h = lane >> 5;
  const int slabs = a.Nn >> 6;
  const int xcd = blockIdx.x & 7, j = blockIdx.x >> 3;
  const int slab = j % slabs, grp = xcd + 8 * (j / slabs), groups = 8 * ((int)(gridDim.x >> 3) / slabs);
  const int n0 = slab * 64;

  {
    const int cb = (t >> 6) & 1, n = n0 + cb * 32 + l31;
#pragma unroll
    for (int e = 0; e < KG / 2; ++e) {
      const int m = (t >> 7) + 2 * e;
      v4f w0, w1;
      const float* bp = a.B + (long)n * a.b_sn + (long)(16 * m + 4 * h) * a.b_sk;
      w0.x = bp[0], w0.y = bp[a.b_sk], w0.z = bp[2 * a.b_sk], w0.w = bp[3 * a.b_sk];
      bp += 8 * a.b_sk;
      w1.x = bp[0], w1.y = bp[a.b_sk], w1.z = bp[2 * a.b_sk], w1.w = bp[3 * a.b_sk];
      unsigned hi[4], mid[4], lo[4];
      pws_split4(w0, hi, mid, lo), pws_split4(w1, hi + 2, mid + 2, lo + 2);
      char* dst = lds + ((m * 2 + cb) * 3) * 1024 + lane * 16;
      *reinterpret_cast<uint4*>(dst) = make_uint4(hi[0], hi[1], hi[2], hi[3]);
      *reinterpret_cast<uint4*>(dst + 1024) = make_uint4(mid[0], mid[1], mid[2], mid[3]);
      *reinterpret_cast<uint4*>(dst + 2048) = make_uint4(lo[0], lo[1], lo[2], lo[3]);
    }
  }
  float* epi = reinterpret_cast<float*>(lds + KG * 2 * 3 * 1024);
  if (t < 64) epi[t] = a.bias ? a.bias[n0 + t] : 0.f;
  else if (t < 128) epi[t] = a.scale ? a.scale[n0 + t - 64] : 1.f;
  else if (t < 192) epi[t] = a.scale ? a.shift[n0 + t - 128] : 0.f;
  __syncthreads();

  const __amdgpu_buffer_rsrc_t rA = __builtin_amdgcn_make_buffer_rsrc(const_cast<float*>(a.A), 0, (int)a.a_bytes, 0x00020000);
  const __amdgpu_buffer_rsrc_t rC = __builtin_amdgcn_make_buffer_rsrc(a.C, 0, (int)a.c_bytes, 0x00020000);
  const __amdgpu_buffer_rsrc_t rR = __builtin_amdgcn_make_buffer_rsrc(const_cast<float*>(a.residual ? a.residual : a.A), 0, (int)(a.residual ? a.res_bytes : 0u), 0x00020000);
  const unsigned a_row = (unsigned)(a.a_pitch * 4), c_row = (unsigned)(a.c_pitch * 4), r_row = (unsigned)(a.res_pitch * 4);
  const bool aff = a.bias || a.scale, res = a.residual != nullptr, relu = a.relu != 0;
  const int first = grp * 4 + wave, stride = groups * 4;
  v4f raw[NB][2 * KG];
  auto load = [&](v4f* dst, int tile) {
    const unsigned off = (unsigned)(tile * 32 + l31) * a_row + (unsigned)h * 16u;
#pragma unroll
    for (int q = 0; q < 2 * KG; ++q) dst[q] = pws_load(rA, off + (unsigned)q * 32u);
  };
  auto tile_out = [&](const v4f* src, int tile) {
    asm volatile("" ::: "memory");
    f32x16 acc[2];
#pragma unroll
    for (int cb = 0; cb < 2; ++cb)
#pragma unroll
      for (int r = 0; r < 16; ++r) acc[cb][r] = 0.f;
#pragma unroll
    for (int m = 0; m < KG; ++m) {
      if (m) asm volatile("" ::: "memory");
      unsigned ah[4], am[4], al[4];
      pws_split4(src[2 * m], ah, am, al), pws_split4(src[2 * m + 1], ah + 2, am + 2, al + 2);
      const bf16x8 fah = __builtin_bit_cast(bf16x8, make_uint4(ah[0], ah[1], ah[2], ah[3]));
      const bf16x8 fam = __builtin_bit_cast(bf16x8, make_uint4(am[0], am[1], am[2], am[3]));
      const bf16x8 fal = __builtin_bit_cast(bf16x8, make_uint4(al[0], al[1], al[2], al[3]));
#pragma unroll
      for (int cb = 0; cb < 2; ++cb) {
        const char* src_b = lds + ((m * 2 + cb) * 3) * 1024 + lane * 16;
        const bf16x8 fbh = *reinterpret_cast<const bf16x8*>(src_b);
        const bf16x8 fbm = *reinterpret_cast<const bf16x8*>(src_b + 1024);
        const bf16x8 fbl = *reinterpret_cast<const bf16x8*>(src_b + 2048);
        acc[cb] = __builtin_amdgcn_mfma_f32_32x32x16_bf16(fbh, fal, acc[cb], 0, 0, 0);
        acc[cb] = __builtin_amdgcn_mfma_f32_32x32x16_bf16(fbl, fah, acc[cb], 0, 0, 0);
        acc[cb] = __builtin_amdgcn_mfma_f32_32x32x16_bf16(fbm, fam, acc[cb], 0, 0, 0);
        acc[cb] = __builtin_amdgcn_mfma_f32_32x32x16_bf16(fbh, fam, acc[cb], 0, 0, 0);
        acc[cb] = __builtin_amdgcn_mfma_f32_32x32x16_bf16(fbm, fah, acc[cb], 0, 0, 0);
        acc[cb] = __builtin_amdgcn_mfma_f32_32x32x16_bf16(fbh, fah, acc[cb], 0, 0, 0);
      }
    }
    char* stg = lds + KG * 2 * 3 * 1024 + 3 * 64 * 4 + wave * (32 * 144);
    const int rr = lane >> 3, cg = lane & 7;
#pragma unroll
    for (int cb = 0; cb < 2; ++cb) {
#pragma unroll
      for (int j = 0; j < 4; ++j)
        *reinterpret_cast<v4f*>(stg + l31 * 144 + (8 * j + 4 * h) * 4) = v4f{acc[cb][4 * j], acc[cb][4 * j + 1], acc[cb][4 * j + 2], acc[cb][4 * j + 3]};
      const int c = cb * 32 + cg * 4;
      v4f bi, sc, sh;
      if (aff) bi = *reinterpret_cast<const v4f*>(epi + c), sc = *reinterpret_cast<const v4f*>(epi + 64 + c), sh = *reinterpret_cast<const v4f*>(epi + 128 + c);
#pragma unroll
      for (int ps = 0; ps < 4; ++ps) {
        const unsigned row = (unsigned)(tile * 32 + rr + 8 * ps);
        v4f v = *reinterpret_cast<const v4f*>(stg + (rr + 8 * ps) * 144 + cg * 16);
        if (aff) v = (v + bi) * sc + sh;
        if (res) v += __builtin_bit_cast(v4f, __builtin_amdgcn_raw_buffer_load_b128(rR, (int)(row * r_row + (unsigned)(n0 + c) * 4u), 0, 0));
        if (relu) v.x = fmaxf(v.x, 0.f), v.y = fmaxf(v.y, 0.f), v.z = fmaxf(v.z, 0.f), v.w = fmaxf(v.w, 0.f);
        __builtin_amdgcn_raw_buffer_store_b128(__builtin_bit_cast(__attribute__((ext_vector_type(4))) unsigned, v), rC, (int)(row * c_row + (unsigned)(n0 + c) * 4u), 0, 0);
      }
    }
  };

  int tile = first;
#pragma unroll
  for (int b = 0; b < NB - 1; ++b)
    if (tile + b * stride < a.row_tiles) load(raw[b], tile + b * stride);
  while (tile < a.row_tiles) {
#pragma unroll
    for (int b = 0; b < NB; ++b) {
      const int ahead = tile + (NB - 1) * stride;
      if (ahead < a.row_tiles) load(raw[(b + NB - 1) % NB], ahead);
      tile_out(raw[b], tile);
      tile += stride;
      if (tile >= a.row_tiles) break;
    }
  }
}

template <int KG, int NB>
void pws_launch(const PwsK& k, int grid, hipStream_t st) {
  const size_t smem = (size_t)KG * 2 * 3 * 1024 + 3 * 64 * sizeof(float) + 4 * 32 * 144;
  static pm_lds_optin optin;
  (void)optin(reinterpret_cast<const void*>(&pwstream_kernel<KG, NB>), 80 * 1024);
  hipLaunchKernelGGL((pwstream_kernel<KG, NB>), dim3(grid), dim3(256), smem, st, k);
}

}

bool pm_pwstream_ok(const pm_gemm_pw* g) {
  constexpr long MIN_ROWS = 65536;
  if (g->K != 64 && g->K != 128) return false;
  const int slabs = g->Nn / 64;
  if (g->Nn % 64 || (slabs != 1 && slabs != 2 && slabs != 4 && slabs != 8)) return false;
  if (g->M < MIN_ROWS || (g->a_pitch & 3) || ((uintptr_t)g->A & 15) || (g->c_pitch & 3) || ((uintptr_t)g->C & 15)) return false;
  if (g->residual && ((g->res_pitch & 3) || ((uintptr_t)g->residual & 15))) return false;
  if ((double)g->M * (double)g->a_pitch * 4.0 >= 4.0e9 || (double)g->M * (double)g->c_pitch * 4.0 >= 4.0e9) return false;
  if (g->residual && (double)g->M * (double)g->res_pitch * 4.0 >= 4.0e9) return false;
  return true;
}

int pm_pwstream_launch(const pm_gemm_pw* g, hipStream_t st) {
  PwsK k;
  k.A = g->A, k.B = g->B, k.C = g->C, k.bias = g->bias, k.scale = g->scale, k.shift = g->shift, k.residual = g->residual;
  k.a_pitch = g->a_pitch, k.c_pitch = g->c_pitch, k.res_pitch = g->res_pitch;
  k.a_bytes = (unsigned)((g->M - 1) * g->a_pitch * 4 + (long)g->K * 4);
  k.c_bytes = (unsigned)((g->M - 1) * g->c_pitch * 4 + (long)g->Nn * 4);
  k.res_bytes = g->residual ? (unsigned)((g->M - 1) * g->res_pitch * 4 + (long)g->Nn * 4) : 0u;
  k.b_sn = g->b_sn, k.b_sk = g->b_sk, k.M = (int)g->M, k.Nn = g->Nn, k.row_tiles = (int)((g->M + 31) / 32), k.relu = g->relu;

  const int slabs = g->Nn / 64, grid = 8 * slabs * std::max(1, 64 / slabs);
  if (g->K == 64) pws_launch<4, 2>(k, grid, st);
  else pws_launch<8, 2>(k, grid, st);
  return pm_check_launch("pwstream");
}
```

### pinthememory_amd/hip/kernels.py

```python
import ctypes
from ctypes import byref

import os

import torch

from . import lib as L
from .lib import PmConvEpilogue, PmConvParams, check, ptr, stream, tdesc, workspace


def _lib():
    return L.load()


CONV_PREC = 0
ACT_DTYPE = torch.float32


def set_conv_precision(name):
    global CONV_PREC, ACT_DTYPE
    CONV_PREC = {'f32': 0, 'fp32': 0, 'bf16': 2, 'bf16_operands': 2, 'bf16_staged': 1}[name]
    ACT_DTYPE = torch.bfloat16 if name == 'bf16' else torch.float32


# ... 196 lines not shown
    if keep_v is not None:
        nbv = nbv if KEEP_WINOGRAD_V else 0
        v = torch.empty(nbv // 4, dtype=torch.float32, device=x.device) if nbv else None
        keep_v.append(v)
        if v is not None:
            p.wino_v, p.wino_v_bytes = v.data_ptr(), nbv
    u_ent = None
    if (kh == 3 and CONV_PREC == 0) or CONV_PREC == 2:
        u_ent = _wino_u(p, w_krsc, nbu)
    if _XFORM_COUNT[1] and p.wxf_valid == 0 and nbu:
        _XFORM_COUNT[0] += 1
    ws = workspace(nb, x.device) if nb else None
    part = None
    if bn_partials is not None:
        ep16 = BN_EPILOGUE16 or (BN_EP16_MIN_BYTES > 0 and y.numel() * 2 >= BN_EP16_MIN_BYTES)
        ep32 = BN_EPILOGUE or (BN_EP_MIN_BYTES > 0 and y.numel() * 4 >= BN_EP_MIN_BYTES)
        npb = npb if ((ep16 if y.dtype == torch.bfloat16 else ep32) and residual is None and not relu and scale is None) else 0
        part = torch.empty(npb // 4, dtype=torch.float32, device=x.device) if npb else None
        bn_partials.append(part)
    ep = None
    if bias is not None or scale is not None or residual is not None or relu or part is not None:
        rd = tdesc(residual) if residual is not None else None
        ep = L.conv_epilogue(ptr(bias), ptr(scale), ptr(shift), rd.ptr if rd else None, rd.pitch if rd else 0, 1 if relu else 0, ptr(part),
                            part.numel() * 4 if part is not None else 0)
    check(lib.pm_conv_fwd(byref(xd), w_krsc.data_ptr(), byref(yd), byref(p), byref(ep) if ep else None, ptr(ws), nb, stream()), 'pm_conv_fwd')
    if u_ent is not None:
        ent, version = u_ent
        cur = L.stream_obj()
        ent[3], ent[4] = cur.record_event(), cur.cuda_stream
        ent[1] = version
    return y


def conv_bwd_data(dy, w_krsc, x_shape, stride, pad, dil, add=None, dtype=None):
    cout, kh, kw, cin = w_krsc.shape
    dx = new(x_shape, dy, dtype=dtype)
    dyd, dxd = tdesc(dy), tdesc(dx)
    p = L.conv_params(kh, kw, stride, pad, dil, CONV_PREC)
    lib = _lib()
    nb, nbu = _sizes(('d', dy.shape, dy.stride(), dy.dtype, dyd.flags, w_krsc.shape, dx.shape, dx.stride(), dx.dtype, stride, pad, dil, CONV_PREC, _GEN[0]),
                     lambda: (lib.pm_conv_workspace(byref(dxd), byref(dyd), byref(p), 1), lib.pm_conv_wxf_bytes_dgrad(byref(dyd), byref(dxd), byref(p))))
    ws = workspace(nb, dy.device) if nb else None
    ad = tdesc(add) if add is not None else None
    u_ent = _wino_u(p, w_krsc, nbu, dgrad=True) if CONV_PREC == 2 else None
    check(lib.pm_conv_bwd_data(byref(dyd), w_krsc.data_ptr(), byref(dxd), byref(p), byref(ad) if ad else None, ptr(ws), nb, stream()), 'pm_conv_bwd_data')
    if u_ent is not None:
        ent, version = u_ent
        cur = L.stream_obj()
        ent[3], ent[4] = cur.record_event(), cur.cuda_stream
        ent[1] = version
    return dx


def conv_bwd_weight(x, dy, w_shape_krsc, stride, pad, dil, want_bias=False, wino_v=None, on_stream=None):
    cout, kh, kw, cin = w_shape_krsc
    dw = torch.empty(w_shape_krsc, dtype=torch.float32, device=x.device)
    db = torch.empty(cout, dtype=torch.float32, device=x.device) if want_bias else None
    xd, dyd = tdesc(x), tdesc(dy)
    p = L.conv_params(kh, kw, stride, pad, dil, CONV_PREC)
    if wino_v is not None:
        p.wino_v, p.wino_v_bytes = wino_v.data_ptr(), wino_v.numel() * 4
    lib = _lib()
    nb = _sizes(('w', x.shape, x.stride(), x.dtype, dy.shape, dy.stride(), dy.dtype, w_shape_krsc, stride, pad, dil, CONV_PREC, wino_v is not None, _GEN[0]),
                lambda: lib.pm_conv_workspace(byref(xd), byref(dyd), byref(p), 2))
    raw = stream() if on_stream is None else on_stream.cuda_stream
    ws = workspace(nb, x.device, on_stream)
    check(lib.pm_conv_bwd_weight(byref(xd), byref(dyd), dw.data_ptr(), ptr(db), byref(p), ptr(ws), nb, raw), 'pm_conv_bwd_weight')
    return dw, db


def bn_stats(x):
    c = x.shape[3]
    mom = torch.empty(3 * c, dtype=torch.float32, device=x.device)
    xd = tdesc(x)
    lib = _lib()
    nb = _sizes(('bn', x.shape, x.dtype), lambda: lib.pm_bn_workspace(byref(xd)))
    ws = workspace(nb, x.device)
    check(lib.pm_bn_stats(byref(xd), mom.data_ptr(), ptr(ws), nb, stream()), 'pm_bn_stats')
# ... 42 lines not shown


def bn_finalize(moments, c, eps, running_mean=None, running_var=None, momentum=0.1):
    mean = torch.empty(c, dtype=torch.float32, device=moments.device)
    invstd = torch.empty_like(mean)
    check(_lib().pm_bn_finalize(moments.data_ptr(), c, eps, mean.data_ptr(), invstd.data_ptr(), ptr(running_mean), ptr(running_var), momentum, stream()),
          'pm_bn_finalize')
    return mean, invstd


def bn_fold_multi(table, cs, offs, n, max_c, total, eps):
    arena = torch.empty(2 * total, dtype=torch.float32, device=table.device)
    check(_lib().pm_bn_fold_multi(table.data_ptr(), cs.data_ptr(), offs.data_ptr(), n, max_c, total, eps, arena.data_ptr(), stream()), 'pm_bn_fold_multi')
    return arena


def bn_fold(gamma, beta, running_mean, running_var, eps, conv_bias=None):
    c = gamma.numel()
    scale = torch.empty(c, dtype=torch.float32, device=gamma.device)
    shift = torch.empty_like(scale)
    check(_lib().pm_bn_fold(gamma.data_ptr(), beta.data_ptr(), running_mean.data_ptr(), running_var.data_ptr(), ptr(conv_bias), c, eps, scale.data_ptr(),
                            shift.data_ptr(), stream()), 'pm_bn_fold')
    return scale, shift


def bn_apply(x, mean, invstd, gamma, beta, residual=None, relu=False, out=None, want_mask=False):
    y = out if out is not None else torch.empty_like(x, memory_format=torch.contiguous_format)
    rd = tdesc(residual) if residual is not None else None
    grp = 8 if x.dtype == torch.bfloat16 else 4
    mask = torch.empty((x.shape[0] * x.shape[1] * x.shape[2], x.shape[3] // grp), dtype=torch.uint8, device=x.device) if want_mask else None
    check(_lib().pm_bn_apply_mask(byref(tdesc(x)), mean.data_ptr(), invstd.data_ptr(), gamma.data_ptr(), beta.data_ptr(), byref(rd) if rd else None,
                                  1 if relu else 0, byref(tdesc(y)), ptr(mask), stream()), 'pm_bn_apply_mask')
    return (y, mask) if want_mask else y


def bn_bwd_reduce_mask(dy, mask, x, mean, invstd, want_gmask=True, with_count=False):
    c = x.shape[3]
    sums = torch.empty(2 * c + (1 if with_count else 0), dtype=torch.float32, device=x.device)
    if with_count:
        sums[2 * c:].fill_(float(x.shape[0] * x.shape[1] * x.shape[2]))
    xd = tdesc(x)
    lib = _lib()
    nb = _sizes(('bn', x.shape, x.dtype), lambda: lib.pm_bn_workspace(byref(xd)))
    ws = workspace(nb, x.device)
    gm = torch.empty(x.shape, dtype=x.dtype, device=x.device) if want_gmask else None
    gd = tdesc(gm) if want_gmask else None
    check(lib.pm_bn_bwd_reduce_mask(byref(tdesc(dy)), mask.data_ptr(), byref(xd), mean.data_ptr(), invstd.data_ptr(), byref(gd) if gd else None,
                                    sums.data_ptr(), ptr(ws), nb, stream()), 'pm_bn_bwd_reduce_mask')
    return sums, gm


def scale_shift_act(x, scale, shift, residual=None, relu=False):
    y = torch.empty(x.shape, dtype=torch.float32, device=x.device)
    rd = tdesc(residual) if residual is not None else None
    check(_lib().pm_scale_shift_act(byref(tdesc(x)), scale.data_ptr(), shift.data_ptr(), byref(rd) if rd else None, 1 if relu else 0, byref(tdesc(y)), stream()),
          'pm_scale_shift_act')
    return y


def bn_bwd_reduce(dy, y, x, mean, invstd, relu, gamma=None, beta=None, want_gmask=False, with_count=False):
    relu = int(relu)
    c = x.shape[3]
    sums = torch.empty(2 * c + (1 if with_count else 0), dtype=torch.float32, device=x.device)
    if with_count:
        sums[2 * c:].fill_(float(x.shape[0] * x.shape[1] * x.shape[2]))
    xd = tdesc(x)
# ... 22 lines not shown
def relu_bwd(dy, y):
    dx = torch.empty(y.shape, dtype=torch.float32, device=y.device)
    check(_lib().pm_relu_bwd(byref(tdesc(dy)), byref(tdesc(y)), byref(tdesc(dx)), stream()), 'pm_relu_bwd')
    return dx


def add_n(xs):
    from .lib import PmTensor
    from ctypes import POINTER, pointer
    descs = [tdesc(x) for x in xs]
    arr = (POINTER(PmTensor) * len(xs))(*[pointer(d) for d in descs])
    y = torch.empty(xs[0].shape, dtype=xs[0].dtype, device=xs[0].device)
    check(_lib().pm_add_n(arr, len(xs), byref(tdesc(y)), stream()), 'pm_add_n')
    return y


def add(a, b, out=None):
    y = out if out is not None else torch.empty(a.shape, dtype=a.dtype, device=a.device)
    check(_lib().pm_add(byref(tdesc(a)), byref(tdesc(b)), byref(tdesc(y)), stream()), 'pm_add')
    return y


def copy(src, dst):
    check(_lib().pm_copy(byref(tdesc(src)), byref(tdesc(dst)), stream()), 'pm_copy')
    return dst


def maxpool_fwd(x):
    n, h, w, c = x.shape
    y = torch.empty((n, (h - 1) // 2 + 1, (w - 1) // 2 + 1, c), dtype=x.dtype, device=x.device)
    arg = torch.empty(y.shape, dtype=torch.uint8, device=x.device)
    check(_lib().pm_maxpool3x3s2_fwd(byref(tdesc(x)), byref(tdesc(y)), arg.data_ptr(), stream()), 'pm_maxpool3x3s2_fwd')
    return y, arg


def maxpool_bwd(dy, arg, x_shape):
    dx = torch.empty(x_shape, dtype=dy.dtype, device=dy.device)
    check(_lib().pm_maxpool3x3s2_bwd(byref(tdesc(dy)), arg.data_ptr(), byref(tdesc(dx)), stream()), 'pm_maxpool3x3s2_bwd')
    return dx


def global_avgpool_fwd(x):
    n, h, w, c = x.shape
    y = torch.empty((n, 1, 1, c), dtype=x.dtype, device=x.device)
    check(_lib().pm_global_avgpool_fwd(byref(tdesc(x)), byref(tdesc(y)), stream()), 'pm_global_avgpool_fwd')
    return y


def global_avgpool_bwd(dy, x_shape):
    dx = torch.empty(x_shape, dtype=dy.dtype, device=dy.device)
    check(_lib().pm_global_avgpool_bwd(byref(tdesc(dy)), byref(tdesc(dx)), 0, stream()), 'pm_global_avgpool_bwd')
    return dx


def resize_fwd(x, size, out=None):
    n, h, w, c = x.shape
    own_pad = c % 4 != 0 and x.stride(2) == (c + 3) // 4 * 4
    y = out if out is not None else new((n, size[0], size[1], c), x, pitch_pad=True, zero_pad=not own_pad)
    check(_lib().pm_resize_bilinear_fwd(byref(tdesc(x)), byref(tdesc(y)), stream()), 'pm_resize_bilinear_fwd')
    return y


RESIZE_SEPARABLE = os.environ.get('PM_RESIZE_SEP', '1') == '1'


def resize_bwd(dy, x_shape, separable=None):
# ... 393 lines not shown
```

### pinthememory_amd/hip/lib.py

```python
import ctypes
import os
from ctypes import POINTER, byref, c_char_p, c_float, c_int, c_int32, c_int64, c_size_t, c_void_p

import torch

_HERE = os.path.dirname(os.path.dirname(os.path.abspath(__file__)))
LIB_PATH = os.environ.get('PM_LIB') or os.path.join(_HERE, 'libpinmem_hip.so')


class PmTensor(ctypes.Structure):
    _fields_ = [('ptr', c_void_p), ('n', c_int32), ('h', c_int32), ('w', c_int32), ('c', c_int32), ('pitch', c_int64), ('dtype', c_int32), ('flags', c_int32)]


PM_F32, PM_BF16 = 0, 1
PM_TF_ZERO_PAD64 = 1


class PmSgdEntry(ctypes.Structure):
    _fields_ = [('param', c_void_p), ('grad', c_void_p), ('momentum_buffer', c_void_p), ('numel', c_int64)]


class PmWxfJob(ctypes.Structure):
    _fields_ = [('w', c_void_p), ('wxf', c_void_p), ('wxf_bytes', c_int64), ('cout', c_int32), ('kh', c_int32), ('kw', c_int32), ('cin', c_int32),
                ('dgrad', c_int32), ('reserved', c_int32)]
# ... 14 lines not shown
    _fields_ = [('struct_size', c_int64), ('bias', c_void_p), ('scale', c_void_p), ('shift', c_void_p), ('residual', c_void_p),
                ('residual_pitch', c_int64), ('relu', c_int32), ('bn_partials', c_void_p), ('bn_partials_bytes', c_int64)]


def conv_params(kh, kw, stride, pad, dil, prec=0):
    return PmConvParams(ctypes.sizeof(PmConvParams), kh, kw, stride, pad, dil, prec)


def conv_epilogue(*fields):
    return PmConvEpilogue(ctypes.sizeof(PmConvEpilogue), *fields)


ABI_VERSION = 400


class PinmemError(RuntimeError):
    pass


_T, _P, _E = POINTER(PmTensor), POINTER(PmConvParams), POINTER(PmConvEpilogue)
_vp, _sz, _i, _f, _i64 = c_void_p, c_size_t, c_int, c_float, c_int64

SIGNATURES = {
    'pm_last_error': (c_char_p, []),
    'pm_version': (c_int, []),
    'pm_conv_winograd_v_bytes': (_sz, [_T, _T, _P]),
    'pm_conv_wxf_bytes': (_sz, [_T, _T, _P]),
    'pm_conv_wxf_bytes_dgrad': (_sz, [_T, _T, _P]),
    'pm_conv_wxf_refresh_bf16': (_i, [_vp, _i, _vp]),
    'pm_conv_wxf_refresh_f32': (_i, [_vp, _i, _vp]),
    'pm_conv_workspace': (_sz, [_T, _T, _P, _i]),
    'pm_conv_fwd': (_i, [_T, _vp, _T, _P, _E, _vp, _sz, _vp]),
    'pm_conv_bwd_data': (_i, [_T, _vp, _T, _P, _T, _vp, _sz, _vp]),
    'pm_conv_bwd_weight': (_i, [_T, _T, _vp, _vp, _P, _vp, _sz, _vp]),
    'pm_set_winograd': (_i, [_i]),
    'pm_set_winograd_fused': (_i, [_i]),
    'pm_set_conv16': (_i, [_i]),
    'pm_profile_enable': (_i, [_i]),
    'pm_profile_dump': (_i, [ctypes.c_char_p]),
    'pm_profile_read': (_i, [_i, _i, _i, _i, _i, POINTER(ctypes.c_double), POINTER(ctypes.c_double), POINTER(c_int64), _i]),
    'pm_profile_read_prec': (_i, [_i, _i, _i, _i, _i, _i, POINTER(ctypes.c_double), POINTER(ctypes.c_double), POINTER(c_int64), _i]),
    'pm_profile_read_bytes': (_i, [_i, _i, _i, _i, _i, _i, POINTER(ctypes.c_double)]),
    'pm_bn_workspace': (_sz, [_T]),
    'pm_bn_stats': (_i, [_T, _vp, _vp, _sz, _vp]),
    'pm_bn_merge': (_i, [_vp, _i, _i, _vp, _vp]),
    'pm_bn_merge_finalize': (_i, [_vp, _i, _i, _f, _vp, _vp, _vp, _vp, _f, _vp]),
    'pm_bn_finalize': (_i, [_vp, _i, _f, _vp, _vp, _vp, _vp, _f, _vp]),
    'pm_bn_stats_finalize': (_i, [_T, _f, _vp, _vp, _vp, _vp, _f, _vp, _sz, _vp]),
    'pm_bn_fold': (_i, [_vp, _vp, _vp, _vp, _vp, _i, _f, _vp, _vp, _vp]),
    'pm_bn_fold_multi': (_i, [_vp, _vp, _vp, _i, _i, _i, _f, _vp, _vp]),
    'pm_bn_apply': (_i, [_T, _vp, _vp, _vp, _vp, _T, _i, _T, _vp]),
    'pm_bn_apply_mask': (_i, [_T, _vp, _vp, _vp, _vp, _T, _i, _T, _vp, _vp]),
    'pm_bn_bwd_reduce_mask': (_i, [_T, _vp, _T, _vp, _vp, _T, _vp, _vp, _sz, _vp]),
    'pm_bn_bwd_reduce': (_i, [_T, _T, _T, _vp, _vp, _vp, _vp, _i, _T, _vp, _vp, _sz, _vp]),
    'pm_bn_bwd_apply': (_i, [_T, _T, _T, _vp, _vp, _vp, _vp, _vp, _f, _i, _T, _T, _vp]),
    'pm_relu_bwd': (_i, [_T, _T, _T, _vp]),
    'pm_add': (_i, [_T, _T, _T, _vp]),
    'pm_add_n': (_i, [POINTER(_T), _i, _T, _vp]),
    'pm_copy': (_i, [_T, _T, _vp]),
    'pm_scale_shift_act': (_i, [_T, _vp, _vp, _T, _i, _T, _vp]),
    'pm_maxpool3x3s2_fwd': (_i, [_T, _T, _vp, _vp]),
    'pm_maxpool3x3s2_bwd': (_i, [_T, _vp, _T, _vp]),
    'pm_global_avgpool_fwd': (_i, [_T, _T, _vp]),
    'pm_global_avgpool_bwd': (_i, [_T, _T, _i, _vp]),
    'pm_resize_bilinear_fwd': (_i, [_T, _T, _vp]),
    'pm_resize_bilinear_bwd': (_i, [_T, _T, _i, _vp]),
    'pm_resize_bilinear_bwd_workspace': (_sz, [_T, _T]),
    'pm_resize_bilinear_bwd_separable': (_i, [_T, _T, _i, _vp, _sz, _vp]),
    'pm_resize_bilinear_hp_fwd': (_i, [_T, _T, _i, _vp]),
    'pm_softmax_mean_update': (_i, [_T, _vp, _i, _vp]),
    'pm_sliding_stitch': (_i, [_T, _vp, _i, _i, _i, _i, _vp, _i, _vp]),
    'pm_argmax_f64': (_i, [_vp, _i, _i, _i, _i, _vp, _vp, _vp]),
    'pm_image_u8_to_nhwc4': (_i, [_vp, _i64, POINTER(c_float), POINTER(c_float), _vp, _vp]),
    'pm_labels_u8_to_i64': (_i, [_vp, _i64, _vp, _vp]),
    'pm_nchw_to_nhwc': (_i, [_vp, _i, _T, _vp]),
    'pm_nhwc_to_nchw': (_i, [_T, _vp, _vp]),
    'pm_label_nearest': (_i, [_vp, _i, _i, _i, _vp, _i, _i, _vp]),
    'pm_upsample_ce_workspace': (_sz, [_i, _i, _i]),
    'pm_upsample_ce_fwd': (_i, [_T, _f, _vp, _i, _i, _vp, _vp, _sz, _vp]),
    'pm_upsample_ce_bwd_workspace': (_sz, [_T, _i, _i]),
    'pm_upsample_ce_bwd': (_i, [_T, _f, _vp, _i, _i, _vp, _vp, _T, _vp, _sz, _vp]),
    'pm_upsample_ce_field_bytes': (_sz, [_T, _i, _i]),
    'pm_upsample_ce_fwd_field': (_i, [_T, _f, _vp, _i, _i, _vp, _vp, _vp, _sz, _vp]),
    'pm_upsample_ce_bwd_field': (_i, [_T, _f, _i, _i, _vp, _vp, _vp, _T, _vp]),
    'pm_upsample_wce_loss_floats': (_sz, [_i]),
    'pm_upsample_wce_workspace': (_sz, [_i, _i, _i]),
    'pm_upsample_wce_fwd': (_i, [_T, _f, _vp, _i, _i, _vp, _i64, _i, _vp, _vp, _sz, _vp]),
    'pm_upsample_wce_fwd_field': (_i, [_T, _f, _vp, _i, _i, _vp, _i64, _i, _vp, _vp, _vp, _sz, _vp]),
    'pm_upsample_wce_bwd_field': (_i, [_T, _f, _i, _i, _i, _vp, _vp, _vp, _T, _vp]),
    'pm_label_class_weights_workspace': (_sz, [_i]),
    'pm_label_class_weights': (_i, [_vp, _i, _i, _i, _i, ctypes.c_double, _i, _i, _vp, _vp, _sz, _vp]),
    'pm_mem_read_fwd': (_i, [_T, _vp, _i, _vp, _T, _vp, _vp, _vp]),
    'pm_mem_read_fwd_pq_workspace': (_sz, [_i64, _i]),
    'pm_mem_read_fwd_pq': (_i, [_T, _vp, _i, _vp, _vp, _T, _vp, _vp, _vp, _vp, _sz, _vp]),
    'pm_mem_colsoftmax_workspace': (_sz, [_i64, _i]),
# ... 120 lines not shown
```

### pinthememory_amd/hip/ops.py

```python
import os as _os

import torch

from . import kernels as K
from . import lib as L
from .. import dist as D


def nhwc(t):
    v = t.permute(0, 2, 3, 1)
    n, h, w, c = v.shape
    sn, sh, sw, sc = v.stride()
    pitch = sw if w > 1 else (sh if h > 1 else (sn if n > 1 else c))
    ok = (sc == 1 or c == 1) and pitch >= c and (h == 1 or w == 1 or sh == w * pitch) and (n == 1 or h * w == 1 or sn == h * w * pitch)
    if ok and v.dtype == torch.float32:
        return v
    if v.dtype == torch.bfloat16:
        if ok and pitch % 8 == 0 and c % 8 == 0 and v.data_ptr() % 16 == 0:
            return v
        return v.contiguous()
    if h * w == 1:
        return v.contiguous().float()
    return K.nchw_to_nhwc(t.float())

# ... 129 lines not shown
    if not commit_done or not torch.cuda.is_available():
        return
    ev = commit_done.pop(torch.cuda.current_device(), None)
    if ev is not None:
        torch.cuda.current_stream().wait_event(ev)


BN_FUSED_FINALIZE = _os.environ.get('PM_BN_FUSED', '1') == '1'


RELU_MASK_BYTES = _os.environ.get('PM_BN_MASK', '1') == '1'


MERGE_SYNCBN = _os.environ.get('PM_MERGE_SYNCBN', '1') == '1'


def _bn_train_stats_multi(ys, bns, partials):
    c = ys[0].shape[3]
    moms = []
    for y, part in zip(ys, partials):
        pixels = y.shape[0] * y.shape[1] * y.shape[2]
        moms.append(K.bn_partials_moments(part, pixels, c) if part is not None else K.bn_stats(y))
    n = len(ys)
    flat, world = D.gather_moments(torch.cat(moms), bns[0].group)
    parts = flat.view(world, n, 3 * c)
    return [K.bn_merge_finalize(parts[:, i].contiguous().view(-1), world, c, bn.eps, bn.running_mean, bn.running_var, bn.momentum) for i, bn in enumerate(bns)]


def _mergeable(bns, ys):
    return (MERGE_SYNCBN and BN_FUSED_FINALIZE and D.is_dist() and len(bns) > 1 and all(b.group is not None and b.group is bns[0].group for b in bns)
            and len({y.shape[3] for y in ys}) == 1)


def _bn_train_fwd(y, gamma, beta, bn, residual, relu, out=None, partials=None, want_mask=False):
    c = y.shape[3]
    pixels = y.shape[0] * y.shape[1] * y.shape[2]
    if bn.group is None and BN_FUSED_FINALIZE:
        if partials is not None:
            mean, invstd = K.bn_partials_finalize(partials, pixels, c, bn.eps, bn.running_mean, bn.running_var, bn.momentum)
        else:
            mean, invstd = K.bn_stats_finalize(y, bn.eps, bn.running_mean, bn.running_var, bn.momentum)
    elif bn.group is not None and D.is_dist() and BN_FUSED_FINALIZE:
        mom = K.bn_partials_moments(partials, pixels, c) if partials is not None else K.bn_stats(y)
        flat, world = D.gather_moments(mom, bn.group)
        mean, invstd = K.bn_merge_finalize(flat, world, c, bn.eps, bn.running_mean, bn.running_var, bn.momentum)
    else:
        mom = K.bn_partials_moments(partials, pixels, c) if partials is not None else K.bn_stats(y)
        if bn.group is not None:
            mom = D.merge_moments(mom, c, bn.group)
        mean, invstd = K.bn_finalize(mom, c, bn.eps, bn.running_mean, bn.running_var, bn.momentum)
    if want_mask:
        o, mask = K.bn_apply(y, mean, invstd, gamma, beta, residual=residual, relu=relu, out=out, want_mask=True)
        return o, mean, invstd, mask
    return K.bn_apply(y, mean, invstd, gamma, beta, residual=residual, relu=relu, out=out), mean, invstd


def _bn_train_bwd(dv, o, y, mean, invstd, gamma, beta, relu, group, want_dres, has_res, mask=None):
    c = y.shape[3]
    mode = 0 if not relu else (1 if has_res else 2)
    hand_over = mode == 1 and want_dres
    if hand_over and mask is not None:
        sums, gm = K.bn_bwd_reduce_mask(dv, mask, y, mean, invstd, want_gmask=True, with_count=group is not None)
    else:
        sums, gm = K.bn_bwd_reduce(dv, o, y, mean, invstd, mode, gamma, beta, want_gmask=hand_over, with_count=group is not None)
    local = sums
    if group is not None:
        sums = D.all_reduce_sum_copy(local, group)
    count = float(y.shape[0] * y.shape[1] * y.shape[2]) if group is None else -1.0
    if hand_over:
        dy, _ = K.bn_bwd_apply(gm, None, y, mean, invstd, gamma, sums, count, 0, False)
        dres = gm
    else:
        dy, dres = K.bn_bwd_apply(dv, o, y, mean, invstd, gamma, sums, count, mode, want_dres, beta)
    return dy, dres, local[c:2 * c], local[:c]


class _Bottleneck(torch.autograd.Function):

    @staticmethod
    def forward(ctx, x, w1, g1, b1, w2, g2, b2, w3, g3, b3, wd, gd, bd, geoms, bns, deferred):
        xv = nhwc(x)
        k1, k2, k3 = K.krsc(w1), K.krsc(w2), K.krsc(w3)
        ps = []
        y1 = K.conv_fwd(xv, k1, *geoms[0], bn_partials=ps)
        o1, m1, i1 = _bn_train_fwd(y1, g1, b1, bns[0], None, True, partials=ps[0])
        kv = []
        y2 = K.conv_fwd(o1, k2, *geoms[1], keep_v=kv, bn_partials=ps)
        o2, m2, i2 = _bn_train_fwd(y2, g2, b2, bns[1], None, True, partials=ps[1])
        y3 = K.conv_fwd(o2, k3, *geoms[2], bn_partials=ps)
        merged = False
        if wd is not None:
            kd = K.krsc(wd)
            yd = K.conv_fwd(xv, kd, *geoms[3], bn_partials=ps)
            merged = _mergeable([bns[3], bns[2]], [yd, y3])
            if merged:
                (md, idd), (m3, i3) = _bn_train_stats_multi([yd, y3], [bns[3], bns[2]], [ps[3], ps[2]])
                res = K.bn_apply(yd, md, idd, gd, bd, residual=None, relu=False)
            else:
                res, md, idd = _bn_train_fwd(yd, gd, bd, bns[3], None, False, partials=ps[3])
        else:
            kd = yd = md = idd = None
            res = xv
        if merged:
            out, mask3 = K.bn_apply(y3, m3, i3, g3, b3, residual=res, relu=True, want_mask=True) if RELU_MASK_BYTES else (K.bn_apply(y3, m3, i3, g3, b3, residual=res, relu=True), None)
        elif RELU_MASK_BYTES:
            out, m3, i3, mask3 = _bn_train_fwd(y3, g3, b3, bns[2], res, True, partials=ps[2], want_mask=True)
        else:
            (out, m3, i3), mask3 = _bn_train_fwd(y3, g3, b3, bns[2], res, True, partials=ps[2]), None
        ctx.geoms, ctx.groups, ctx.has_ds, ctx.deferred = geoms, [b.group for b in bns], wd is not None, deferred
        ctx.save_for_backward(xv, k1, k2, k3, kd, y1, o1, y2, o2, y3, yd, out, m1, i1, m2, i2, m3, i3, md, idd, g1, g2, g3, gd, b1, b2, b3, kv[0], mask3)
        return nchw(out)

    @staticmethod
    def backward(ctx, dout):
        xv, k1, k2, k3, kd, y1, o1, y2, o2, y3, yd, out, m1, i1, m2, i2, m3, i3, md, idd, g1, g2, g3, gd, b1, b2, b3, v2, mask3 = ctx.saved_tensors
        ge, gr, df = ctx.geoms, ctx.groups, ctx.deferred
        dv = _grad_view(dout)
        pair = None
        if ctx.has_ds and MERGE_SYNCBN and D.is_dist() and gr[2] is not None and gr[3] is gr[2] and y3.shape[3] == yd.shape[3]:
            c3 = y3.shape[3]
            if mask3 is not None:
                s3, gm = K.bn_bwd_reduce_mask(dv, mask3, y3, m3, i3, want_gmask=True, with_count=True)
            else:
                s3, gm = K.bn_bwd_reduce(dv, out, y3, m3, i3, 1, g3, b3, want_gmask=True, with_count=True)
            sd, _ = K.bn_bwd_reduce(gm, None, yd, md, idd, 0, gd, None, want_gmask=False, with_count=True)
            both = D.all_reduce_sum_copy(torch.cat([s3, sd]), gr[2])
            g3sum, gdsum = both[:s3.numel()], both[s3.numel():]
            dy3, _ = K.bn_bwd_apply(gm, None, y3, m3, i3, g3, g3sum, -1.0, 0, False)
            dres, dg3, db3 = gm, s3[c3:2 * c3], s3[:c3]
            dyd, _ = K.bn_bwd_apply(gm, None, yd, md, idd, gd, gdsum, -1.0, 0, False, None)
            pair = (dyd, sd[c3:2 * c3], sd[:c3])
        else:
            dy3, dres, dg3, db3 = _bn_train_bwd(dv, out, y3, m3, i3, g3, b3, True, gr[2], True, True, mask=mask3)
        dw3, _ = _wgrad(o2, dy3, tuple(k3.shape), ge[2], deferred=df[2])
        do2 = K.conv_bwd_data(dy3, k3, tuple(o2.shape), *ge[2])
        dy2, _, dg2, db2 = _bn_train_bwd(do2, o2, y2, m2, i2, g2, b2, True, gr[1], False, False)
        dw2, _ = _wgrad(o1, dy2, tuple(k2.shape), ge[1], deferred=df[1], wino_v=v2)
        do1 = K.conv_bwd_data(dy2, k2, tuple(o1.shape), *ge[1])
        dy1, _, dg1, db1 = _bn_train_bwd(do1, o1, y1, m1, i1, g1, b1, True, gr[0], False, False)
        dw1, _ = _wgrad(xv, dy1, tuple(k1.shape), ge[0], deferred=df[0])
        dwd = dgd = dbd = None
        skip = dres
        if ctx.has_ds:
            if pair is not None:
                dyd, dgd, dbd = pair
            else:
                dyd, _, dgd, dbd = _bn_train_bwd(dres, None, yd, md, idd, gd, None, False, gr[3], False, False)
            dwdk, _ = _wgrad(xv, dyd, tuple(kd.shape), ge[3], deferred=df[3])
            dwd = dwdk.permute(0, 3, 1, 2)
            skip = K.conv_bwd_data(dyd, kd, tuple(xv.shape), *ge[3]) if ctx.needs_input_grad[0] else None
        dx = nchw(K.conv_bwd_data(dy1, k1, tuple(xv.shape), *ge[0], add=skip)) if ctx.needs_input_grad[0] else None
        p = lambda d: d.permute(0, 3, 1, 2)
        return dx, p(dw1), dg1, db1, p(dw2), dg2, db2, p(dw3), dg3, db3, dwd, dgd, dbd, None, None, None


FOLD_BATCH = _os.environ.get('PM_FOLD_BATCH', '1') == '1'
_fold_cache = None
fold_misses = 0
last_prefold_event = None


class prefold:
    def __init__(self, model):
        self.model, self.active = model, False

    def __enter__(self):
        global _fold_cache, last_prefold_event
        last_prefold_event = None
        m = self.model
        if not FOLD_BATCH or m.training or torch.is_grad_enabled() or _fold_cache is not None:
            return self
        bns = getattr(m, '_pm_bn_list', None)
        if bns is None:
            bns = [b for b in m.modules() if isinstance(b, torch.nn.modules.batchnorm._BatchNorm)]
            m.__dict__['_pm_bn_list'] = bns
        bns = [b for b in bns if b.running_mean is not None and b.weight is not None and b.running_mean.is_cuda and not b.training]
        if not bns or len({b.eps for b in bns}) != 1:
            return self
        ptrs = tuple(t.data_ptr() for b in bns for t in (b.weight, b.bias, b.running_mean, b.running_var))
        plan = m.__dict__.get('_pm_fold_plan')
        if plan is None or plan[0] != ptrs:
            dev = bns[0].running_mean.device
            cs = [b.num_features for b in bns]
            offs, tot = [], 0
# ... 40 lines not shown
        y = K.conv_fwd(xv, wk, stride, pad, dil, bias=bias, keep_v=kv if ctx.needs_input_grad[1] else None, bn_partials=ps if bn.training else None)
        if bn.training:
            o, mean, invstd = _bn_train_fwd(y, gamma, beta, bn, rv, relu, ov, partials=ps[0])
        else:
            mean, invstd = bn.running_mean, torch.rsqrt(bn.running_var + bn.eps)
            o = K.bn_apply(y, mean, invstd, gamma, beta, residual=rv, relu=relu, out=ov)
        ctx.group, ctx.has_bias, ctx.has_res = bn.group, bias is not None, residual is not None
        ctx.save_for_backward(xv, wk, y, o, mean, invstd, gamma, beta, kv[0] if kv else None)
        return nchw(o)

    @staticmethod
    def backward(ctx, dout):
        xv, wk, y, o, mean, invstd, gamma, beta, vk = ctx.saved_tensors
        stride, pad, dil = ctx.geom
        dv = _grad_view(dout)
        want_dres = ctx.has_res and ctx.needs_input_grad[5]
        if ctx.train:
            dy, dres, dgamma, dbeta = _bn_train_bwd(dv, o, y, mean, invstd, gamma, beta, ctx.relu, ctx.group, want_dres, ctx.has_res)
        else:
            c = y.shape[3]
            mode = 0 if not ctx.relu else (1 if ctx.has_res else 2)
            sums, g = K.bn_bwd_reduce(dv, o, y, mean, invstd, mode, gamma, beta, want_gmask=mode != 0)
            g = dv if g is None else g
            dy = K.scale_shift_act(g, gamma * invstd, torch.zeros_like(gamma))
            dres, dgamma, dbeta = (g if want_dres else None), sums[c:], sums[:c]
        dx = nchw(K.conv_bwd_data(dy, wk, tuple(xv.shape), stride, pad, dil, dtype=xv.dtype)) if ctx.needs_input_grad[0] else None
        dw = db = None
        if ctx.needs_input_grad[1] or (ctx.has_bias and ctx.needs_input_grad[2]):
            dwk, db = _wgrad(xv, dy, tuple(wk.shape), (stride, pad, dil), want_bias=ctx.has_bias, deferred=ctx.deferred, wino_v=vk)
            dw = dwk.permute(0, 3, 1, 2)
        return dx, dw, db, dgamma, dbeta, (nchw(dres) if dres is not None else None), None, None, None, None, None


class _ConvBnActN(torch.autograd.Function):

    @staticmethod
    def forward(ctx, n, geoms, bns, outs, deferreds, *ts):
        xs, ws, gammas, betas = ts[0:n], ts[n:2 * n], ts[2 * n:3 * n], ts[3 * n:4 * n]
        xvs, wks = [nhwc(x) for x in xs], [K.krsc(w) for w in ws]
        ys, kvs, parts = [], [], []
        for i in range(n):
            kv, ps = [], []
            ys.append(K.conv_fwd(xvs[i], wks[i], *geoms[i], keep_v=kv if ctx.needs_input_grad[5 + n + i] else None, bn_partials=ps))
            kvs.append(kv[0] if kv else None)
            parts.append(ps[0])
        stats = _bn_train_stats_multi(ys, bns, parts)
        os_ = [K.bn_apply(ys[i], stats[i][0], stats[i][1], gammas[i], betas[i], residual=None, relu=True, out=nhwc(outs[i]) if outs[i] is not None else None) for i in range(n)]
        ctx.n, ctx.geoms, ctx.group, ctx.deferreds = n, geoms, bns[0].group, deferreds
        ctx.save_for_backward(*xvs, *wks, *ys, *os_, *[st[0] for st in stats], *[st[1] for st in stats], *gammas, *betas, *kvs)
        return tuple(nchw(o) for o in os_)

    @staticmethod
    def backward(ctx, *douts):
        n = ctx.n
        sv = ctx.saved_tensors
        xvs, wks, ys, os_, means, invs, gammas, betas, kvs = (sv[i * n:(i + 1) * n] for i in range(9))
        c = ys[0].shape[3]
        red = [K.bn_bwd_reduce(_grad_view(douts[i]), os_[i], ys[i], means[i], invs[i], 2, gammas[i], betas[i], want_gmask=False, with_count=True) for i in range(n)]
        tot = D.all_reduce_sum_copy(torch.cat([r[0] for r in red]), ctx.group)
        ln = red[0][0].numel()
        dxs, dws, dgs, dbs = [], [], [], []
        for i in range(n):
            dy, _ = K.bn_bwd_apply(_grad_view(douts[i]), os_[i], ys[i], means[i], invs[i], gammas[i], tot[i * ln:(i + 1) * ln], -1.0, 2, False, betas[i])
            dxs.append(nchw(K.conv_bwd_data(dy, wks[i], tuple(xvs[i].shape), *ctx.geoms[i], dtype=xvs[i].dtype)) if ctx.needs_input_grad[5 + i] else None)
            dwk, _ = _wgrad(xvs[i], dy, tuple(wks[i].shape), ctx.geoms[i], deferred=ctx.deferreds[i], wino_v=kvs[i])
            dws.append(dwk.permute(0, 3, 1, 2))
# ... 357 lines not shown
```

### pinthememory_amd/network/Resnet.py

```python
import torch
import torch.nn as nn

from . import mynn
from ..hip import ops

__all__ = ['ResNet', 'Bottleneck', 'resnet50', 'resnet101']


class Bottleneck(nn.Module):
    expansion = 4

    def __init__(self, inplanes, planes, stride=1, downsample=None, iw=0):
        super().__init__()
        assert iw == 0, 'instance whitening is out of scope of the pinmem hot path'
        self.conv1 = nn.Conv2d(inplanes, planes, kernel_size=1, bias=False)
        self.bn1 = mynn.Norm2d(planes)
        self.conv2 = nn.Conv2d(planes, planes, kernel_size=3, stride=stride, padding=1, bias=False)
        self.bn2 = mynn.Norm2d(planes)
        self.conv3 = nn.Conv2d(planes, planes * self.expansion, kernel_size=1, bias=False)
        self.bn3 = mynn.Norm2d(planes * self.expansion)
        self.downsample = downsample
        self.stride = stride
        self.iw = iw
        self.relu = nn.ReLU(inplace=True)
# ... 30 lines not shown
        self.fc = nn.Linear(512 * block.expansion, num_classes)
        self.wt_layer = wt_layer
        for m in self.modules():
            if isinstance(m, nn.Conv2d):
                nn.init.kaiming_normal_(m.weight, mode='fan_out', nonlinearity='relu')
            elif isinstance(m, (nn.BatchNorm2d, nn.SyncBatchNorm)):
                if m.weight is not None:
                    nn.init.constant_(m.weight, 1)
                if m.bias is not None:
                    nn.init.constant_(m.bias, 0)

    def _make_layer(self, block, planes, blocks, stride=1):
        downsample = None
        if stride != 1 or self.inplanes != planes * block.expansion:
            downsample = nn.Sequential(nn.Conv2d(self.inplanes, planes * block.expansion, kernel_size=1, stride=stride, bias=False),
                                       mynn.Norm2d(planes * block.expansion))
        layers = [block(self.inplanes, planes, stride, downsample, iw=0)]
        self.inplanes = planes * block.expansion
        for _ in range(1, blocks):
            layers.append(block(self.inplanes, planes, iw=0))
        return nn.Sequential(*layers)

    def forward(self, x):
        x = stem(self.conv1, self.bn1, x)
        x_tuple = self.layer4(self.layer3(self.layer2(self.layer1([x, []]))))
        return x_tuple[0]


def stem(conv1, bn1, x):
    import torch.nn.functional as F
    from ..hip import kernels as K
    x4 = ops.nchw(K.nchw_to_nhwc(x.float(), c_pad=4)) if x.shape[1] == 3 else x
    w4 = F.pad(conv1.weight, (0, 0, 0, 0, 0, 4 - conv1.weight.shape[1])) if conv1.weight.shape[1] == 3 else conv1.weight
    y = ops._ConvBnAct.apply(x4, w4, None, bn1.weight, bn1.bias, None, ops._geom(conv1), ops.BNState(bn1), True, None)
    return ops.maxpool3x3s2(y)


def _pretrained(model, name):
    return model


def resnet50(pretrained=True, wt_layer=None, **kwargs):
    return _pretrained(ResNet(Bottleneck, [3, 4, 6, 3], wt_layer=wt_layer, **kwargs), 'resnet50')


def resnet101(pretrained=True, wt_layer=None, **kwargs):
    return _pretrained(ResNet(Bottleneck, [3, 4, 23, 3], wt_layer=wt_layer, **kwargs), 'resnet101')
```

Measured before the change: 153.1.

## Fuse stem BN+ReLU into maxpool and fold downsample BN into residual apply

Adds a custom stem autograd function that fuses BN apply and ReLU into the 3x3/s2 maxpool in forward, and in backward gathers the pooled gradient through argmax directly into the BN reduce and apply kernels. This avoids materialising the full-resolution post-BN activation and its gradient. In bottlenecks with f32 activations, the downsample branch's BN affine is computed inside the main residual apply instead of as a separate pass. The backward uses the ReLU mask to drive a masked BN backward and a masked add in conv dgrad. The change adds several new kernels and code paths with more conditional branching.

```diff
diff --git a/include/pinmem_hip.h b/include/pinmem_hip.h
--- a/include/pinmem_hip.h
+++ b/include/pinmem_hip.h
@@ -67,6 +67,8 @@
                 const pm_conv_epilogue* ep, void* ws, size_t ws_bytes, void* stream);
 int pm_conv_bwd_data(const pm_tensor* dy, const float* w_krsc, const pm_tensor* dx, const pm_conv_params* p,
                      const pm_tensor* add, void* ws, size_t ws_bytes, void* stream);
+int pm_conv_bwd_data_masked(const pm_tensor* dy, const float* w_krsc, const pm_tensor* dx, const pm_conv_params* p,
+                            const pm_tensor* add, const uint8_t* add_mask, void* ws, size_t ws_bytes, void* stream);
 int pm_conv_bwd_weight(const pm_tensor* x, const pm_tensor* dy, float* dw_krsc, float* dbias, const pm_conv_params* p,
                        void* ws, size_t ws_bytes, void* stream);
 
@@ -113,6 +115,11 @@
                      const pm_tensor* residual , int relu, const pm_tensor* y, uint8_t* mask , void* stream);
 int pm_bn_bwd_reduce_mask(const pm_tensor* dy, const uint8_t* mask, const pm_tensor* x, const float* mean, const float* invstd,
                           const pm_tensor* gmask , float* sums, void* ws, size_t ws_bytes, void* stream);
+int pm_bn_apply_mask_affine(const pm_tensor* x, const float* mean, const float* invstd, const float* gamma, const float* beta,
+                            const pm_tensor* r, const float* r_mean, const float* r_invstd, const float* r_gamma, const float* r_beta,
+                            int relu, const pm_tensor* y, uint8_t* mask , void* stream);
+int pm_bn_bwd_apply_mask(const pm_tensor* dy, const uint8_t* mask, const pm_tensor* x, const float* mean, const float* invstd, const float* gamma,
+                         const float* sums, float count, const pm_tensor* dx, void* stream);
 int pm_bn_bwd_reduce(const pm_tensor* dy, const pm_tensor* y , const pm_tensor* x, const float* mean, const float* invstd,
                      const float* gamma , const float* beta , int relu, const pm_tensor* gmask ,
                      float* sums, void* ws, size_t ws_bytes, void* stream);
@@ -135,6 +142,12 @@
 
 int pm_maxpool3x3s2_fwd(const pm_tensor* x, const pm_tensor* y, uint8_t* argmax, void* stream);
 int pm_maxpool3x3s2_bwd(const pm_tensor* dy, const uint8_t* argmax, const pm_tensor* dx, void* stream);
+int pm_maxpool3x3s2_bn_relu_fwd(const pm_tensor* x, const float* mean, const float* invstd, const float* gamma, const float* beta, const pm_tensor* y,
+                                uint8_t* argmax, void* stream);
+int pm_bn_bwd_reduce_pool(const pm_tensor* dy_pooled, const uint8_t* argmax, const pm_tensor* x, const float* mean, const float* invstd, const float* gamma,
+                          const float* beta, float* sums, void* ws, size_t ws_bytes, void* stream);
+int pm_bn_bwd_apply_pool(const pm_tensor* dy_pooled, const uint8_t* argmax, const pm_tensor* x, const float* mean, const float* invstd, const float* gamma,
+                         const float* beta, const float* sums, float count, const pm_tensor* dx, void* stream);
 int pm_global_avgpool_fwd(const pm_tensor* x, const pm_tensor* y , void* stream);
 int pm_global_avgpool_bwd(const pm_tensor* dy, const pm_tensor* dx, int accumulate, void* stream);
 
diff --git a/pinthememory_amd/csrc/bn.hip b/pinthememory_amd/csrc/bn.hip
--- a/pinthememory_amd/csrc/bn.hip
+++ b/pinthememory_amd/csrc/bn.hip
@@ -5,10 +5,7 @@
 constexpr int CB = 64;
 constexpr int RL = 16;
 
-__device__ __forceinline__ float bn_affine(float v, float mu, float is, float ga, float be) {
-  const float s = is * ga;
-  return fmaf(v, s, fmaf(-mu, s, be));
-}
+__device__ __forceinline__ float bn_affine(float v, float mu, float is, float ga, float be) { return pm_bn_affine(v, mu, is, ga, be); }
 
 inline int chunk_rows(long P, int C) {
   const long colblocks = std::max<long>(1, (C + CB - 1) / CB);
@@ -182,6 +179,39 @@
     if (ch < C) part[((long)blockIdx.x * C + ch) * 2 + w] = s;
   }
 }
+__global__ __launch_bounds__(256) void bn_bwd_partial_pool(const float* __restrict__ dyp, long dpitch, int Ho, int Wo, const uint8_t* __restrict__ arg, int H, int W,
+                                                           const float* __restrict__ x, long xpitch, const float* __restrict__ mean, const float* __restrict__ invstd,
+                                                           const float* __restrict__ gamma, const float* __restrict__ beta, long P, int C, int rows,
+                                                           float* __restrict__ part) {
+  __shared__ float sm[RL][CB][2];
+  const int g = threadIdx.x & 15, r = threadIdx.x >> 4;
+  const int c = blockIdx.y * CB + g * 4;
+  const long p0 = (long)blockIdx.x * rows, p1 = min(P, p0 + rows);
+  float s1[4] = {0, 0, 0, 0}, s2[4] = {0, 0, 0, 0};
+  if (c < C) {
+    const float4 mu = PM_LD4(mean + c), is = PM_LD4(invstd + c), ga = PM_LD4(gamma + c), be = PM_LD4(beta + c);
+    for (long p = p0 + r; p < p1; p += RL) {
+      float4 d = pm_maxpool_gather4(dyp, dpitch, Ho, Wo, arg, H, W, C, p, c);
+      const float4 v = PM_LD4(x + p * xpitch + c);
+      d.x = bn_affine(v.x, mu.x, is.x, ga.x, be.x) > 0.f ? d.x : 0.f, d.y = bn_affine(v.y, mu.y, is.y, ga.y, be.y) > 0.f ? d.y : 0.f;
+      d.z = bn_affine(v.z, mu.z, is.z, ga.z, be.z) > 0.f ? d.z : 0.f, d.w = bn_affine(v.w, mu.w, is.w, ga.w, be.w) > 0.f ? d.w : 0.f;
+      s1[0] += d.x, s1[1] += d.y, s1[2] += d.z, s1[3] += d.w;
+      s2[0] += d.x * ((v.x - mu.x) * is.x), s2[1] += d.y * ((v.y - mu.y) * is.y);
+      s2[2] += d.z * ((v.z - mu.z) * is.z), s2[3] += d.w * ((v.w - mu.w) * is.w);
+    }
+  }
+#pragma unroll
+  for (int j = 0; j < 4; ++j) sm[r][g * 4 + j][0] = s1[j], sm[r][g * 4 + j][1] = s2[j];
+  __syncthreads();
+  if (threadIdx.x < CB * 2) {
+    const int cc = threadIdx.x >> 1, w = threadIdx.x & 1;
+    float s = 0.f;
+#pragma unroll
+    for (int i = 0; i < RL; ++i) s += sm[i][cc][w];
+    const int ch = blockIdx.y * CB + cc;
+    if (ch < C) part[((long)blockIdx.x * C + ch) * 2 + w] = s;
+  }
+}
 __global__ __launch_bounds__(256) void bn_bwd_final(const float* __restrict__ part, int nb, int C, float* __restrict__ sums) {
   const int c = blockIdx.x * FC + (threadIdx.x & (FC - 1)), lane = threadIdx.x / FC;
   double s1, s2;
@@ -344,6 +374,35 @@
   return pm_bn_apply_mask(x, mean, invstd, gamma, beta, res, relu, y, nullptr, stream);
 }
 
+namespace {
+
+template <bool RAFF>
+int bn_apply_launch(const pm_tensor* x, const float* mean, const float* invstd, const float* gamma, const float* beta, const pm_tensor* res, const float* rmean,
+                    const float* rinvstd, const float* rgamma, const float* rbeta, int relu, const pm_tensor* y, uint8_t* mask, hipStream_t stream) {
+  const float *px = (const float*)x->ptr, *pr = res ? (const float*)res->ptr : nullptr;
+  float* py = (float*)y->ptr;
+  const long a = x->pitch, b = res ? res->pitch : 0, c = y->pitch, cq = x->c >> 2;
+  return pm_ew_launch(true, pm_pixels(x), x->c, stream, "bn_apply", [=] __device__(long p, int ch) {
+    const float4 v = PM_LD4(px + p * a + ch), mu = PM_LD4(mean + ch), is = PM_LD4(invstd + ch), ga = PM_LD4(gamma + ch), be = PM_LD4(beta + ch);
+    float4 o = make_float4(bn_affine(v.x, mu.x, is.x, ga.x, be.x), bn_affine(v.y, mu.y, is.y, ga.y, be.y), bn_affine(v.z, mu.z, is.z, ga.z, be.z),
+                           bn_affine(v.w, mu.w, is.w, ga.w, be.w));
+    if (pr) {
+      float4 q = PM_LD4(pr + p * b + ch);
+      if constexpr (RAFF) {
+        const float4 rm = PM_LD4(rmean + ch), ri = PM_LD4(rinvstd + ch), rg = PM_LD4(rgamma + ch), rb = PM_LD4(rbeta + ch);
+        q = make_float4(bn_affine(q.x, rm.x, ri.x, rg.x, rb.x), bn_affine(q.y, rm.y, ri.y, rg.y, rb.y), bn_affine(q.z, rm.z, ri.z, rg.z, rb.z),
+                        bn_affine(q.w, rm.w, ri.w, rg.w, rb.w));
+      }
+      o.x += q.x, o.y += q.y, o.z += q.z, o.w += q.w;
+    }
+    if (mask) mask[p * cq + (ch >> 2)] = (unsigned char)((o.x > 0.f ? 1 : 0) | (o.y > 0.f ? 2 : 0) | (o.z > 0.f ? 4 : 0) | (o.w > 0.f ? 8 : 0));
+    if (relu) o.x = fmaxf(o.x, 0.f), o.y = fmaxf(o.y, 0.f), o.z = fmaxf(o.z, 0.f), o.w = fmaxf(o.w, 0.f);
+    PM_ST4(py + p * c + ch, o);
+  });
+}
+
+}
+
 extern "C" int pm_bn_apply_mask(const pm_tensor* x, const float* mean, const float* invstd, const float* gamma, const float* beta, const pm_tensor* res,
                                 int relu, const pm_tensor* y, uint8_t* mask, void* stream) {
   PM_REQUIRE(x && y, PM_EINVAL, "bn_apply: null");
@@ -355,21 +414,19 @@
     if (int e = check_bn(res, "bn_apply")) return e;
     PM_REQUIRE(pm_same_shape(x, res), PM_EINVAL, "bn_apply: residual shape mismatch");
   }
-  const float *px = (const float*)x->ptr, *pr = res ? (const float*)res->ptr : nullptr;
-  float* py = (float*)y->ptr;
-  const long a = x->pitch, b = res ? res->pitch : 0, c = y->pitch, cq = x->c >> 2;
-  return pm_ew_launch(true, pm_pixels(x), x->c, (hipStream_t)stream, "bn_apply", [=] __device__(long p, int ch) {
-    const float4 v = PM_LD4(px + p * a + ch), mu = PM_LD4(mean + ch), is = PM_LD4(invstd + ch), ga = PM_LD4(gamma + ch), be = PM_LD4(beta + ch);
-    float4 o = make_float4(bn_affine(v.x, mu.x, is.x, ga.x, be.x), bn_affine(v.y, mu.y, is.y, ga.y, be.y), bn_affine(v.z, mu.z, is.z, ga.z, be.z),
-                           bn_affine(v.w, mu.w, is.w, ga.w, be.w));
-    if (pr) {
-      const float4 q = PM_LD4(pr + p * b + ch);
-      o.x += q.x, o.y += q.y, o.z += q.z, o.w += q.w;
-    }
-    if (mask) mask[p * cq + (ch >> 2)] = (unsigned char)((o.x > 0.f ? 1 : 0) | (o.y > 0.f ? 2 : 0) | (o.z > 0.f ? 4 : 0) | (o.w > 0.f ? 8 : 0));
-    if (relu) o.x = fmaxf(o.x, 0.f), o.y = fmaxf(o.y, 0.f), o.z = fmaxf(o.z, 0.f), o.w = fmaxf(o.w, 0.f);
-    PM_ST4(py + p * c + ch, o);
-  });
+  return bn_apply_launch<false>(x, mean, invstd, gamma, beta, res, nullptr, nullptr, nullptr, nullptr, relu, y, mask, (hipStream_t)stream);
+}
+
+extern "C" int pm_bn_apply_mask_affine(const pm_tensor* x, const float* mean, const float* invstd, const float* gamma, const float* beta, const pm_tensor* r,
+                                       const float* r_mean, const float* r_invstd, const float* r_gamma, const float* r_beta, int relu, const pm_tensor* y,
+                                       uint8_t* mask, void* stream) {
+  PM_REQUIRE(x && y && r, PM_EINVAL, "bn_apply_mask_affine: null");
+  if (int e = check_bn(x, "bn_apply_mask_affine")) return e;
+  if (int e = check_bn(y, "bn_apply_mask_affine")) return e;
+  if (int e = check_bn(r, "bn_apply_mask_affine")) return e;
+  PM_REQUIRE(pm_same_shape(x, y) && pm_same_shape(x, r) && mean && invstd && gamma && beta && r_mean && r_invstd && r_gamma && r_beta, PM_EINVAL,
+             "bn_apply_mask_affine: bad args");
+  return bn_apply_launch<true>(x, mean, invstd, gamma, beta, r, r_mean, r_invstd, r_gamma, r_beta, relu, y, mask, (hipStream_t)stream);
 }
 
 extern "C" int pm_bn_bwd_reduce(const pm_tensor* dy, const pm_tensor* y, const pm_tensor* x, const float* mean, const float* invstd, const float* gamma,
@@ -473,3 +530,85 @@
     PM_ST4(pdx + p * d + ch, r);
   });
 }
+
+extern "C" int pm_bn_bwd_apply_mask(const pm_tensor* dy, const uint8_t* mask, const pm_tensor* x, const float* mean, const float* invstd, const float* gamma,
+                                    const float* sums, float count, const pm_tensor* dx, void* stream) {
+  PM_REQUIRE(dy && x && dx && mask, PM_EINVAL, "bn_bwd_apply_mask: null");
+  if (int e = check_bn(dy, "bn_bwd_apply_mask")) return e;
+  if (int e = check_bn(x, "bn_bwd_apply_mask")) return e;
+  if (int e = check_bn(dx, "bn_bwd_apply_mask")) return e;
+  PM_REQUIRE(pm_same_shape(dy, x) && pm_same_shape(dx, x) && mean && invstd && gamma && sums, PM_EINVAL, "bn_bwd_apply_mask: bad args");
+  const float *pd = (const float*)dy->ptr, *px = (const float*)x->ptr;
+  float* pdx = (float*)dx->ptr;
+  const long a = dy->pitch, c = x->pitch, d = dx->pitch;
+  const int C = x->c, cq = C >> 2;
+  const bool dev_count = !(count > 0.f);
+  const float host_inv_n = dev_count ? 0.f : 1.f / count;
+  return pm_ew_launch(true, pm_pixels(x), C, (hipStream_t)stream, "bn_bwd_apply_mask", [=] __device__(long p, int ch) {
+    const float inv_n = dev_count ? 1.f / sums[2 * C] : host_inv_n;
+    float4 g = PM_LD4(pd + p * a + ch);
+    const unsigned mb = mask[p * cq + (ch >> 2)];
+    g.x = (mb & 1u) ? g.x : 0.f, g.y = (mb & 2u) ? g.y : 0.f, g.z = (mb & 4u) ? g.z : 0.f, g.w = (mb & 8u) ? g.w : 0.f;
+    const float4 v = PM_LD4(px + p * c + ch), mu = PM_LD4(mean + ch), is = PM_LD4(invstd + ch), ga = PM_LD4(gamma + ch);
+    const float4 s1 = PM_LD4(sums + ch), s2 = PM_LD4(sums + C + ch);
+    float4 r;
+    r.x = (g.x - s1.x * inv_n - (v.x - mu.x) * is.x * (s2.x * inv_n)) * (is.x * ga.x);
+    r.y = (g.y - s1.y * inv_n - (v.y - mu.y) * is.y * (s2.y * inv_n)) * (is.y * ga.y);
+    r.z = (g.z - s1.z * inv_n - (v.z - mu.z) * is.z * (s2.z * inv_n)) * (is.z * ga.z);
+    r.w = (g.w - s1.w * inv_n - (v.w - mu.w) * is.w * (s2.w * inv_n)) * (is.w * ga.w);
+    PM_ST4(pdx + p * d + ch, r);
+  });
+}
+
+namespace {
+int check_pool_bn(const pm_tensor* dyp, const uint8_t* argmax, const pm_tensor* x, const char* who) {
+  PM_REQUIRE(dyp && argmax && x, PM_EINVAL, "%s: null", who);
+  if (int e = check_bn(dyp, who)) return e;
+  if (int e = check_bn(x, who)) return e;
+  PM_REQUIRE(dyp->n == x->n && dyp->c == x->c && dyp->h == (x->h + 2 - 3) / 2 + 1 && dyp->w == (x->w + 2 - 3) / 2 + 1, PM_EINVAL,
+             "%s: dy is the gradient of the 3x3 / s2 / p1 max pool of a tensor shaped like x", who);
+  return PM_OK;
+}
+}
+
+extern "C" int pm_bn_bwd_reduce_pool(const pm_tensor* dyp, const uint8_t* argmax, const pm_tensor* x, const float* mean, const float* invstd, const float* gamma,
+                                     const float* beta, float* sums, void* ws, size_t ws_bytes, void* stream) {
+  if (int e = check_pool_bn(dyp, argmax, x, "bn_bwd_reduce_pool")) return e;
+  PM_REQUIRE(mean && invstd && gamma && beta && sums, PM_EINVAL, "bn_bwd_reduce_pool: bad args");
+  PM_REQUIRE(ws && ws_bytes >= pm_bn_workspace(x), PM_EWORKSPACE, "bn_bwd_reduce_pool: workspace too small");
+  const long P = pm_pixels(x);
+  const int rows = chunk_rows(P, x->c), nb = pm_cdiv(P, rows);
+  hipStream_t st = (hipStream_t)stream;
+  hipLaunchKernelGGL(bn_bwd_partial_pool, dim3(nb, pm_cdiv(x->c, CB)), dim3(256), 0, st, (const float*)dyp->ptr, (long)dyp->pitch, dyp->h, dyp->w, argmax, x->h, x->w,
+                     (const float*)x->ptr, (long)x->pitch, mean, invstd, gamma, beta, P, x->c, rows, (float*)ws);
+  hipLaunchKernelGGL(bn_bwd_final, dim3(pm_cdiv(x->c, FC)), dim3(256), 0, st, (const float*)ws, nb, x->c, sums);
+  return pm_check_launch("bn_bwd_reduce_pool");
+}
+
+extern "C" int pm_bn_bwd_apply_pool(const pm_tensor* dyp, const uint8_t* argmax, const pm_tensor* x, const float* mean, const float* invstd, const float* gamma,
+                                    const float* beta, const float* sums, float count, const pm_tensor* dx, void* stream) {
+  if (int e = check_pool_bn(dyp, argmax, x, "bn_bwd_apply_pool")) return e;
+  PM_REQUIRE(dx, PM_EINVAL, "bn_bwd_apply_pool: null");
+  if (int e = check_bn(dx, "bn_bwd_apply_pool")) return e;
+  PM_REQUIRE(pm_same_shape(dx, x) && mean && invstd && gamma && beta && sums, PM_EINVAL, "bn_bwd_apply_pool: bad args");
+  const float *pd = (const float*)dyp->ptr, *px = (const float*)x->ptr;
+  float* pdx = (float*)dx->ptr;
+  const long a = dyp->pitch, c = x->pitch, d = dx->pitch;
+  const int C = x->c, H = x->h, W = x->w, Ho = dyp->h, Wo = dyp->w;
+  const bool dev_count = !(count > 0.f);
+  const float host_inv_n = dev_count ? 0.f : 1.f / count;
+  return pm_ew_launch(true, pm_pixels(x), C, (hipStream_t)stream, "bn_bwd_apply_pool", [=] __device__(long p, int ch) {
+    const float inv_n = dev_count ? 1.f / sums[2 * C] : host_inv_n;
+    float4 g = pm_maxpool_gather4(pd, a, Ho, Wo, argmax, H, W, C, p, ch);
+    const float4 v = PM_LD4(px + p * c + ch), mu = PM_LD4(mean + ch), is = PM_LD4(invstd + ch), ga = PM_LD4(gamma + ch), be = PM_LD4(beta + ch);
+    g.x = bn_affine(v.x, mu.x, is.x, ga.x, be.x) > 0.f ? g.x : 0.f, g.y = bn_affine(v.y, mu.y, is.y, ga.y, be.y) > 0.f ? g.y : 0.f;
+    g.z = bn_affine(v.z, mu.z, is.z, ga.z, be.z) > 0.f ? g.z : 0.f, g.w = bn_affine(v.w, mu.w, is.w, ga.w, be.w) > 0.f ? g.w : 0.f;
+    const float4 s1 = PM_LD4(sums + ch), s2 = PM_LD4(sums + C + ch);
+    float4 r;
+    r.x = (g.x - s1.x * inv_n - (v.x - mu.x) * is.x * (s2.x * inv_n)) * (is.x * ga.x);
+    r.y = (g.y - s1.y * inv_n - (v.y - mu.y) * is.y * (s2.y * inv_n)) * (is.y * ga.y);
+    r.z = (g.z - s1.z * inv_n - (v.z - mu.z) * is.z * (s2.z * inv_n)) * (is.z * ga.z);
+    r.w = (g.w - s1.w * inv_n - (v.w - mu.w) * is.w * (s2.w * inv_n)) * (is.w * ga.w);
+    PM_ST4(pdx + p * d + ch, r);
+  });
+}
diff --git a/pinthememory_amd/csrc/conv_igemm.hip b/pinthememory_amd/csrc/conv_igemm.hip
--- a/pinthememory_amd/csrc/conv_igemm.hip
+++ b/pinthememory_amd/csrc/conv_igemm.hip
@@ -13,7 +13,7 @@
 __global__ __launch_bounds__(256) void splitk_reduce_vec_kernel(const float* __restrict__ ws, int ksplit, long slab, int M, int Nn,
                                                                 float* __restrict__ C, long c_pitch, const float* bias,
                                                                 const float* scale, const float* shift, const float* residual,
-                                                                long res_pitch, int relu) {
+                                                                long res_pitch, int relu, const unsigned char* res_mask) {
   constexpr int GP = 256 / ZL;
   __shared__ float4 red[ZL > 1 ? ZL : 1][GP];
   const int gl = threadIdx.x % GP, zl = threadIdx.x / GP;
@@ -54,7 +54,11 @@
           const uint2 q = *reinterpret_cast<const uint2*>(reinterpret_cast<const pm_bf16*>(residual) + (long)row * res_pitch + col);
           v.x += __uint_as_float(q.x << 16), v.y += __uint_as_float(q.x & 0xffff0000u), v.z += __uint_as_float(q.y << 16), v.w += __uint_as_float(q.y & 0xffff0000u);
         } else {
-          const float4 r = PM_LD4(residual + (long)row * res_pitch + col);
+          float4 r = PM_LD4(residual + (long)row * res_pitch + col);
+          if (res_mask) {
+            const unsigned mb = res_mask[grp];
+            r.x = (mb & 1u) ? r.x : 0.f, r.y = (mb & 2u) ? r.y : 0.f, r.z = (mb & 4u) ? r.z : 0.f, r.w = (mb & 8u) ? r.w : 0.f;
+          }
           v.x += r.x, v.y += r.y, v.z += r.z, v.w += r.w;
         }
       }
@@ -84,8 +88,9 @@
 }
 
 int splitk_reduce(const float* ws, int ksplit, long M, long Nn, float* C, long c_pitch, const float* bias, const float* scale, const float* shift,
-                  const float* residual, long res_pitch, int relu, hipStream_t st, bool out16 = false) {
+                  const float* residual, long res_pitch, int relu, hipStream_t st, bool out16 = false, const unsigned char* res_mask = nullptr) {
   const long total = M * Nn;
+  PM_REQUIRE(!res_mask || (residual && !out16), PM_EUNSUPPORTED, "splitk_reduce: a masked residual is an fp32 operand");
   if (out16) {
     PM_REQUIRE((Nn % 4 == 0) && (c_pitch % 4 == 0) && (res_pitch % 4 == 0) && pm_aligned16(ws) && (reinterpret_cast<uintptr_t>(C) & 7) == 0 &&
                    (reinterpret_cast<uintptr_t>(residual) & 7) == 0 && (!bias || pm_aligned16(bias)) && (!scale || (pm_aligned16(scale) && pm_aligned16(shift))),
@@ -94,16 +99,17 @@
     const int zl = (ksplit >= 32 && groups < (1 << 18)) ? 16 : (ksplit >= 8 && groups < (1 << 20) ? 4 : 1);
     const int nb = (int)std::min<long>((groups + 256 / zl - 1) / (256 / zl), 8192);
     if (zl == 16)
-      hipLaunchKernelGGL((splitk_reduce_vec_kernel<16, true>), dim3(nb), dim3(256), 0, st, ws, ksplit, total, (int)M, (int)Nn, C, c_pitch, bias, scale, shift, residual, res_pitch, relu);
+      hipLaunchKernelGGL((splitk_reduce_vec_kernel<16, true>), dim3(nb), dim3(256), 0, st, ws, ksplit, total, (int)M, (int)Nn, C, c_pitch, bias, scale, shift, residual, res_pitch, relu, res_mask);
     else if (zl == 4)
-      hipLaunchKernelGGL((splitk_reduce_vec_kernel<4, true>), dim3(nb), dim3(256), 0, st, ws, ksplit, total, (int)M, (int)Nn, C, c_pitch, bias, scale, shift, residual, res_pitch, relu);
+      hipLaunchKernelGGL((splitk_reduce_vec_kernel<4, true>), dim3(nb), dim3(256), 0, st, ws, ksplit, total, (int)M, (int)Nn, C, c_pitch, bias, scale, shift, residual, res_pitch, relu, res_mask);
     else
-      hipLaunchKernelGGL((splitk_reduce_vec_kernel<1, true>), dim3(nb), dim3(256), 0, st, ws, ksplit, total, (int)M, (int)Nn, C, c_pitch, bias, scale, shift, residual, res_pitch, relu);
+      hipLaunchKernelGGL((splitk_reduce_vec_kernel<1, true>), dim3(nb), dim3(256), 0, st, ws, ksplit, total, (int)M, (int)Nn, C, c_pitch, bias, scale, shift, residual, res_pitch, relu, res_mask);
     return pm_check_launch("splitk_reduce(bf16)");
   }
   const bool vec = (Nn % 4 == 0) && (c_pitch % 4 == 0) && (res_pitch % 4 == 0) && pm_aligned16(ws) && pm_aligned16(C) &&
                    (!bias || pm_aligned16(bias)) && (!scale || (pm_aligned16(scale) && pm_aligned16(shift))) && (!residual || pm_aligned16(residual));
   if (!vec) {
+    PM_REQUIRE(!res_mask, PM_EUNSUPPORTED, "splitk_reduce: a masked residual needs 16-byte aligned rows");
     const int nb = (int)std::min<long>((total + 255) / 256, 4096);
     hipLaunchKernelGGL(splitk_reduce_kernel, dim3(nb), dim3(256), 0, st, ws, ksplit, total, (int)M, (int)Nn, C, c_pitch, bias, scale, shift, residual,
                        res_pitch, relu);
@@ -113,11 +119,11 @@
     const int gp = 256 / zl;
     const int nb = (int)std::min<long>((groups + gp - 1) / gp, 8192);
     if (zl == 16)
-      hipLaunchKernelGGL(splitk_reduce_vec_kernel<16>, dim3(nb), dim3(256), 0, st, ws, ksplit, total, (int)M, (int)Nn, C, c_pitch, bias, scale, shift, residual, res_pitch, relu);
+      hipLaunchKernelGGL(splitk_reduce_vec_kernel<16>, dim3(nb), dim3(256), 0, st, ws, ksplit, total, (int)M, (int)Nn, C, c_pitch, bias, scale, shift, residual, res_pitch, relu, res_mask);
     else if (zl == 4)
-      hipLaunchKernelGGL(splitk_reduce_vec_kernel<4>, dim3(nb), dim3(256), 0, st, ws, ksplit, total, (int)M, (int)Nn, C, c_pitch, bias, scale, shift, residual, res_pitch, relu);
+      hipLaunchKernelGGL(splitk_reduce_vec_kernel<4>, dim3(nb), dim3(256), 0, st, ws, ksplit, total, (int)M, (int)Nn, C, c_pitch, bias, scale, shift, residual, res_pitch, relu, res_mask);
     else
-      hipLaunchKernelGGL(splitk_reduce_vec_kernel<1>, dim3(nb), dim3(256), 0, st, ws, ksplit, total, (int)M, (int)Nn, C, c_pitch, bias, scale, shift, residual, res_pitch, relu);
+      hipLaunchKernelGGL(splitk_reduce_vec_kernel<1>, dim3(nb), dim3(256), 0, st, ws, ksplit, total, (int)M, (int)Nn, C, c_pitch, bias, scale, shift, residual, res_pitch, relu, res_mask);
   }
   return pm_check_launch("splitk_reduce");
 }
@@ -377,7 +383,7 @@
   if constexpr (MODE != MODE_WGRAD) {
     if (pm_route.split && (k.prec == 0 || k.prec == 5) && !k.io16 && batch == 1 && p.ksplit == 1 && !k.stats && k.kh * k.kw == 1 && k.stride == 1 && k.pad == 0 && !k.sub) {
       pm_gemm_pw g;
-      g.A = k.A, g.B = k.B, g.C = k.C, g.bias = k.bias, g.scale = k.scale, g.shift = k.shift, g.residual = k.residual;
+      g.A = k.A, g.B = k.B, g.C = k.C, g.bias = k.bias, g.scale = k.scale, g.shift = k.shift, g.residual = k.residual, g.res_mask = k.res_mask;
       g.a_pitch = MODE == MODE_FWD ? k.x_pitch : k.y_pitch, g.c_pitch = k.c_pitch, g.res_pitch = k.res_pitch;
       g.b_sn = MODE == MODE_FWD ? k.K : 1, g.b_sk = MODE == MODE_FWD ? 1 : k.Nn;
       g.M = k.M, g.Nn = k.Nn, g.K = k.K, g.relu = k.relu;
@@ -446,7 +452,7 @@
   k.T_eff = p->kh * p->kw, k.tk_w = p->kw, k.ky0 = k.kx0 = 0, k.ksy = k.ksx = 1;
   k.sub = k.sub_cy = k.sub_cx = 0, k.Hc = x->h, k.Wc = x->w;
   k.bias = k.scale = k.shift = k.residual = nullptr;
-  k.res_pitch = 0, k.relu = 0, k.stats = nullptr, k.io16 = 0;
+  k.res_pitch = 0, k.res_mask = nullptr, k.relu = 0, k.stats = nullptr, k.io16 = 0;
   k.stage_ep = 1;
   k.spl_prio = 1;
   k.n_group = 8;
@@ -976,7 +982,8 @@
 }
 
 template <int MODE>
-int conv_direct(const pm_tensor* x, const pm_tensor* y, const float* w, const pm_conv_params* p, const Plan& pl, const pm_conv_epilogue& e, void* ws, hipStream_t st) {
+int conv_direct(const pm_tensor* x, const pm_tensor* y, const float* w, const pm_conv_params* p, const Plan& pl, const pm_conv_epilogue& e, void* ws, hipStream_t st,
+                const unsigned char* res_mask = nullptr) {
   const pm_tensor *xin = MODE == MODE_FWD ? x : y, *out = MODE == MODE_FWD ? y : x;
   long M, Nn, K;
   gemm_dims(MODE, x, y, p, M, Nn, K);
@@ -990,10 +997,11 @@
   if (pl.ksplit > 1) {
     k.C = (float*)ws, k.c_pitch = Nn, k.c_split = M * Nn;
     if (int err = launch<MODE>(k, pl, st)) return err;
-    return splitk_reduce((const float*)ws, pl.ksplit, M, Nn, (float*)out->ptr, (long)out->pitch, e.bias, e.scale, e.shift, e.residual, (long)e.residual_pitch, e.relu, st, k.io16 != 0);
+    return splitk_reduce((const float*)ws, pl.ksplit, M, Nn, (float*)out->ptr, (long)out->pitch, e.bias, e.scale, e.shift, e.residual, (long)e.residual_pitch, e.relu, st, k.io16 != 0,
+                         res_mask);
   }
   k.C = (float*)out->ptr, k.c_pitch = out->pitch, k.c_split = 0;
-  k.bias = e.bias, k.scale = e.scale, k.shift = e.shift, k.residual = e.residual, k.res_pitch = e.residual_pitch, k.relu = e.relu;
+  k.bias = e.bias, k.scale = e.scale, k.shift = e.shift, k.residual = e.residual, k.res_pitch = e.residual_pitch, k.res_mask = res_mask, k.relu = e.relu;
   k.stats = e.bn_partials;
   return launch<MODE>(k, pl, st);
 }
@@ -1225,6 +1233,11 @@
 
 extern "C" int pm_conv_bwd_data(const pm_tensor* dy, const float* w, const pm_tensor* dx, const pm_conv_params* p0, const pm_tensor* add,
                                 void* ws, size_t ws_bytes, void* stream) {
+  return pm_conv_bwd_data_masked(dy, w, dx, p0, add, nullptr, ws, ws_bytes, stream);
+}
+
+extern "C" int pm_conv_bwd_data_masked(const pm_tensor* dy, const float* w, const pm_tensor* dx, const pm_conv_params* p0, const pm_tensor* add,
+                                       const uint8_t* add_mask, void* ws, size_t ws_bytes, void* stream) {
   if (int e = check_common(dx, dy, p0)) return e;
   const pm_conv_params tp = tier_params(p0, dy, dx);
   const pm_conv_params* p = &tp;
@@ -1233,6 +1246,12 @@
   PM_REQUIRE(w && pm_aligned16(w), PM_EINVAL, "conv_bwd_data: weight null or unaligned");
   const ConvRoute r = route_conv(MODE_DGRAD, dx, dy, p);
   PM_REQUIRE(ws_bytes >= r.ws_bytes && (ws || r.ws_bytes == 0), PM_EWORKSPACE, "conv_bwd_data: workspace %zu < %zu", ws_bytes, r.ws_bytes);
+  if (add_mask) {
+    PM_REQUIRE(add && pm_is_f32(add) && pm_is_f32(dy) && pm_vec4(add) && pm_vec4(dx), PM_EINVAL, "conv_bwd_data: a masked `add` is an fp32 tensor with 16-byte rows and c %% 4 == 0");
+    PM_REQUIRE(r.kind == R_DIRECT, PM_EUNSUPPORTED,
+               "conv_bwd_data: a masked `add` is served by the fp32 implicit-GEMM route only (this call routes to %s)",
+               r.kind == R_WINO ? "Winograd" : (r.kind == R_BF16 ? "the bf16 kernels" : "the stride-2 class kernels"));
+  }
   hipStream_t st = (hipStream_t)stream;
   const pm_conv_epilogue e1 = {(int64_t)sizeof(pm_conv_epilogue), nullptr, nullptr, nullptr, add ? (const float*)add->ptr : nullptr, add ? add->pitch : 0, 0};
   switch (r.kind) {
@@ -1245,7 +1264,7 @@
     case R_WINO: return wino_conv(dy, w, dy->c, dx->c, true, dx, r.wino, e1, ws, st);
     default:
       PM_REQUIRE(pm_is_f32(dy), PM_EUNSUPPORTED, "conv_bwd_data: a bf16 dy needs at least 32 channels and a stride-1 geometry the forward form covers");
-      return conv_direct<MODE_DGRAD>(dx, dy, w, p, r.pl, e1, ws, st);
+      return conv_direct<MODE_DGRAD>(dx, dy, w, p, r.pl, e1, ws, st, add_mask);
   }
 }
 
diff --git a/pinthememory_amd/csrc/conv_igemm_kernel.h b/pinthememory_amd/csrc/conv_igemm_kernel.h
--- a/pinthememory_amd/csrc/conv_igemm_kernel.h
+++ b/pinthememory_amd/csrc/conv_igemm_kernel.h
@@ -32,6 +32,7 @@
   const float* shift;
   const float* residual;
   long res_pitch;
+  const unsigned char* res_mask;
   int relu;
   float* stats;
   int io16;
@@ -860,7 +861,11 @@
         if (row < a.M && cok) {
           if (aff) v.x = (v.x + bi[0]) * sc[0] + sh[0], v.y = (v.y + bi[1]) * sc[1] + sh[1], v.z = (v.z + bi[2]) * sc[2] + sh[2], v.w = (v.w + bi[3]) * sc[3] + sh[3];
           if (res) {
-            const float4 qv = PM_LD4(a.residual + row * a.res_pitch + col);
+            float4 qv = PM_LD4(a.residual + row * a.res_pitch + col);
+            if constexpr (MODE == MODE_DGRAD) if (a.res_mask) {
+              const unsigned mb = a.res_mask[row * (a.Nn >> 2) + (col >> 2)];
+              qv.x = (mb & 1u) ? qv.x : 0.f, qv.y = (mb & 2u) ? qv.y : 0.f, qv.z = (mb & 4u) ? qv.z : 0.f, qv.w = (mb & 8u) ? qv.w : 0.f;
+            }
             v.x += qv.x, v.y += qv.y, v.z += qv.z, v.w += qv.w;
           }
           if (relu) v.x = fmaxf(v.x, 0.f), v.y = fmaxf(v.y, 0.f), v.z = fmaxf(v.z, 0.f), v.w = fmaxf(v.w, 0.f);
diff --git a/pinthememory_amd/csrc/pm_common.h b/pinthememory_amd/csrc/pm_common.h
--- a/pinthememory_amd/csrc/pm_common.h
+++ b/pinthememory_amd/csrc/pm_common.h
@@ -133,6 +133,7 @@
   const float* B;
   float* C;
   const float *bias, *scale, *shift, *residual;
+  const unsigned char* res_mask;
   long a_pitch, c_pitch, res_pitch;
   int b_sn, b_sk;
   long M;
@@ -233,6 +234,34 @@
 #pragma unroll
     for (int e = 0; e < 8; e += 2) *reinterpret_cast<float4*>(dst + 2 * e) = make_float4(mu[e], m2[e], mu[e + 1], m2[e + 1]);
   }
+}
+
+__device__ __forceinline__ float pm_bn_affine(float v, float mu, float is, float ga, float be) {
+  const float s = is * ga;
+  return fmaf(v, s, fmaf(-mu, s, be));
+}
+
+__device__ __forceinline__ float4 pm_maxpool_gather4(const float* __restrict__ dy, long dp, int Ho, int Wo, const uint8_t* __restrict__ arg, int H, int W, int C, long ip,
+                                                     int ch) {
+  const int ix = (int)(ip % W), iy = (int)((ip / W) % H), n = (int)(ip / ((long)W * H));
+  float4 g = make_float4(0.f, 0.f, 0.f, 0.f);
+  const int oy_hi = min((iy + 1) >> 1, Ho - 1), ox_hi = min((ix + 1) >> 1, Wo - 1);
+  for (int oy = iy >> 1; oy <= oy_hi; ++oy) {
+    const int ky = iy + 1 - 2 * oy;
+    if (ky < 0 || ky > 2) continue;
+    for (int ox = ix >> 1; ox <= ox_hi; ++ox) {
+      const int kx = ix + 1 - 2 * ox;
+      if (kx < 0 || kx > 2) continue;
+      const long op = (long)(n * Ho + oy) * Wo + ox;
+      const unsigned a = *reinterpret_cast<const unsigned*>(arg + op * C + ch), want = (unsigned)(ky * 3 + kx);
+      const float4 d = *reinterpret_cast<const float4*>(dy + op * dp + ch);
+      g.x += (a & 255u) == want ? d.x : 0.f;
+      g.y += ((a >> 8) & 255u) == want ? d.y : 0.f;
+      g.z += ((a >> 16) & 255u) == want ? d.z : 0.f;
+      g.w += (a >> 24) == want ? d.w : 0.f;
+    }
+  }
+  return g;
 }
 
 __device__ __forceinline__ float pm_wave_sum(float v) {
diff --git a/pinthememory_amd/csrc/pool_resize.hip b/pinthememory_amd/csrc/pool_resize.hip
--- a/pinthememory_amd/csrc/pool_resize.hip
+++ b/pinthememory_amd/csrc/pool_resize.hip
@@ -2,9 +2,12 @@
 
 namespace {
 
-template <bool VEC>
+template <bool VEC, bool BN = false>
 __global__ __launch_bounds__(256) void maxpool_fwd_kernel(const float* __restrict__ x, long xp, int H, int W, float* __restrict__ y, long yp, int Ho,
-                                                          int Wo, int C, long total, uint8_t* __restrict__ arg) {
+                                                          int Wo, int C, long total, uint8_t* __restrict__ arg, const float* __restrict__ mean = nullptr,
+                                                          const float* __restrict__ invstd = nullptr, const float* __restrict__ gamma = nullptr,
+                                                          const float* __restrict__ beta = nullptr) {
+  static_assert(VEC || !BN, "the normalising form is vectorised");
   constexpr int V = VEC ? 4 : 1;
   const int cg = C / V;
   for (long i = (long)blockIdx.x * 256 + threadIdx.x; i < total; i += (long)gridDim.x * 256) {
@@ -15,6 +18,8 @@
     uint8_t bi[V];
 #pragma unroll
     for (int v = 0; v < V; ++v) best[v] = -INFINITY, bi[v] = 0;
+    float4 mu, is, ga, be;
+    if constexpr (BN) mu = PM_LD4(mean + ch), is = PM_LD4(invstd + ch), ga = PM_LD4(gamma + ch), be = PM_LD4(beta + ch);
     bool first = true;
 #pragma unroll
     for (int ky = 0; ky < 3; ++ky) {
@@ -30,6 +35,10 @@
           const float4 q = PM_LD4(p);
           v[0] = q.x;
           if (V > 1) v[1 % V] = q.y, v[2 % V] = q.z, v[3 % V] = q.w;
+          if constexpr (BN) {
+            v[0] = fmaxf(pm_bn_affine(v[0], mu.x, is.x, ga.x, be.x), 0.f), v[1 % V] = fmaxf(pm_bn_affine(v[1 % V], mu.y, is.y, ga.y, be.y), 0.f);
+            v[2 % V] = fmaxf(pm_bn_affine(v[2 % V], mu.z, is.z, ga.z, be.z), 0.f), v[3 % V] = fmaxf(pm_bn_affine(v[3 % V], mu.w, is.w, ga.w, be.w), 0.f);
+          }
         } else {
           v[0] = *p;
         }
@@ -52,24 +61,7 @@
   for (long i = (long)blockIdx.x * 256 + threadIdx.x; i < total; i += (long)gridDim.x * 256) {
     const long ip = i / cg;
     const int ch = (int)(i - ip * cg) * 4;
-    const int ix = (int)(ip % W), iy = (int)((ip / W) % H), n = (int)(ip / ((long)W * H));
-    float4 g = make_float4(0.f, 0.f, 0.f, 0.f);
-    const int oy_hi = min((iy + 1) >> 1, Ho - 1), ox_hi = min((ix + 1) >> 1, Wo - 1);
-    for (int oy = iy >> 1; oy <= oy_hi; ++oy) {
-      const int ky = iy + 1 - 2 * oy;
-      if (ky < 0 || ky > 2) continue;
-      for (int ox = ix >> 1; ox <= ox_hi; ++ox) {
-        const int kx = ix + 1 - 2 * ox;
-        if (kx < 0 || kx > 2) continue;
-        const long op = (long)(n * Ho + oy) * Wo + ox;
-        const unsigned a = *reinterpret_cast<const unsigned*>(arg + op * C + ch), want = (unsigned)(ky * 3 + kx);
-        const float4 d = PM_LD4(dy + op * dp + ch);
-        g.x += (a & 255u) == want ? d.x : 0.f;
-        g.y += ((a >> 8) & 255u) == want ? d.y : 0.f;
-        g.z += ((a >> 16) & 255u) == want ? d.z : 0.f;
-        g.w += (a >> 24) == want ? d.w : 0.f;
-      }
-    }
+    const float4 g = pm_maxpool_gather4(dy, dp, Ho, Wo, arg, H, W, C, ip, ch);
     PM_ST4(dx + ip * xp + ch, g);
   }
 }
@@ -357,6 +349,19 @@
   return pm_check_launch("maxpool_fwd");
 }
 
+extern "C" int pm_maxpool3x3s2_bn_relu_fwd(const pm_tensor* x, const float* mean, const float* invstd, const float* gamma, const float* beta, const pm_tensor* y,
+                                           uint8_t* argmax, void* stream) {
+  PM_REQUIRE(x && y && argmax && x->ptr && y->ptr && mean && invstd && gamma && beta, PM_EINVAL, "maxpool_bn_relu_fwd: null");
+  PM_REQUIRE(y->h == (x->h + 2 - 3) / 2 + 1 && y->w == (x->w + 2 - 3) / 2 + 1 && x->n == y->n && x->c == y->c, PM_EINVAL, "maxpool_bn_relu_fwd: shape mismatch");
+  PM_REQUIRE_F32(x, "maxpool_bn_relu_fwd"); PM_REQUIRE_F32(y, "maxpool_bn_relu_fwd");
+  PM_REQUIRE(pm_vec4(x) && pm_vec4(y), PM_EINVAL, "maxpool_bn_relu_fwd: tensors must be 16B aligned with pitch %% 4 == 0 and c %% 4 == 0");
+  const long total = pm_pixels(y) * y->c / 4;
+  if (total == 0) return PM_OK;
+  hipLaunchKernelGGL((maxpool_fwd_kernel<true, true>), dim3(grid_for(total)), dim3(256), 0, (hipStream_t)stream, (const float*)x->ptr, (long)x->pitch, x->h, x->w,
+                     (float*)y->ptr, (long)y->pitch, y->h, y->w, x->c, total, argmax, mean, invstd, gamma, beta);
+  return pm_check_launch("maxpool_bn_relu_fwd");
+}
+
 extern "C" int pm_maxpool3x3s2_bwd(const pm_tensor* dy, const uint8_t* argmax, const pm_tensor* dx, void* stream) {
   PM_REQUIRE(dy && dx && argmax && dy->ptr && dx->ptr && dy->n == dx->n && dy->c == dx->c, PM_EINVAL, "maxpool_bwd: bad args");
   if (pm_is_bf16(dy) && pm_is_bf16(dx)) return pm16_maxpool_bwd(dy, argmax, dx, (hipStream_t)stream);
diff --git a/pinthememory_amd/csrc/pwstream.hip b/pinthememory_amd/csrc/pwstream.hip
--- a/pinthememory_amd/csrc/pwstream.hip
+++ b/pinthememory_amd/csrc/pwstream.hip
@@ -15,8 +15,9 @@
   const float* B;
   float* C;
   const float *bias, *scale, *shift, *residual;
+  const unsigned char* res_mask;
   long a_pitch, c_pitch, res_pitch;
-  unsigned a_bytes, c_bytes, res_bytes;
+  unsigned a_bytes, c_bytes, res_bytes, mask_bytes;
   int b_sn, b_sk;
   int M, Nn, row_tiles, relu;
 };
@@ -74,8 +75,10 @@
   const __amdgpu_buffer_rsrc_t rA = __builtin_amdgcn_make_buffer_rsrc(const_cast<float*>(a.A), 0, (int)a.a_bytes, 0x00020000);
   const __amdgpu_buffer_rsrc_t rC = __builtin_amdgcn_make_buffer_rsrc(a.C, 0, (int)a.c_bytes, 0x00020000);
   const __amdgpu_buffer_rsrc_t rR = __builtin_amdgcn_make_buffer_rsrc(const_cast<float*>(a.residual ? a.residual : a.A), 0, (int)(a.residual ? a.res_bytes : 0u), 0x00020000);
-  const unsigned a_row = (unsigned)(a.a_pitch * 4), c_row = (unsigned)(a.c_pitch * 4), r_row = (unsigned)(a.res_pitch * 4);
-  const bool aff = a.bias || a.scale, res = a.residual != nullptr, relu = a.relu != 0;
+  const __amdgpu_buffer_rsrc_t rM = __builtin_amdgcn_make_buffer_rsrc(const_cast<unsigned char*>(a.res_mask ? a.res_mask : reinterpret_cast<const unsigned char*>(a.A)), 0,
+                                                                      (int)(a.res_mask ? a.mask_bytes : 0u), 0x00020000);
+  const unsigned a_row = (unsigned)(a.a_pitch * 4), c_row = (unsigned)(a.c_pitch * 4), r_row = (unsigned)(a.res_pitch * 4), m_row = (unsigned)(a.Nn >> 2);
+  const bool aff = a.bias || a.scale, res = a.residual != nullptr, msk = a.res_mask != nullptr, relu = a.relu != 0;
   const int first = grp * 4 + wave, stride = groups * 4;
   v4f raw[NB][2 * KG];
   auto load = [&](v4f* dst, int tile) {
@@ -127,7 +130,14 @@
         const unsigned row = (unsigned)(tile * 32 + rr + 8 * ps);
         v4f v = *reinterpret_cast<const v4f*>(stg + (rr + 8 * ps) * 144 + cg * 16);
         if (aff) v = (v + bi) * sc + sh;
-        if (res) v += __builtin_bit_cast(v4f, __builtin_amdgcn_raw_buffer_load_b128(rR, (int)(row * r_row + (unsigned)(n0 + c) * 4u), 0, 0));
+        if (res) {
+          v4f q = __builtin_bit_cast(v4f, __builtin_amdgcn_raw_buffer_load_b128(rR, (int)(row * r_row + (unsigned)(n0 + c) * 4u), 0, 0));
+          if (msk) {
+            const unsigned mb = __builtin_amdgcn_raw_buffer_load_b8(rM, (int)(row * m_row + (unsigned)((n0 + c) >> 2)), 0, 0);
+            q.x = (mb & 1u) ? q.x : 0.f, q.y = (mb & 2u) ? q.y : 0.f, q.z = (mb & 4u) ? q.z : 0.f, q.w = (mb & 8u) ? q.w : 0.f;
+          }
+          v += q;
+        }
         if (relu) v.x = fmaxf(v.x, 0.f), v.y = fmaxf(v.y, 0.f), v.z = fmaxf(v.z, 0.f), v.w = fmaxf(v.w, 0.f);
         __builtin_amdgcn_raw_buffer_store_b128(__builtin_bit_cast(__attribute__((ext_vector_type(4))) unsigned, v), rC, (int)(row * c_row + (unsigned)(n0 + c) * 4u), 0, 0);
       }
@@ -179,6 +189,7 @@
   k.a_bytes = (unsigned)((g->M - 1) * g->a_pitch * 4 + (long)g->K * 4);
   k.c_bytes = (unsigned)((g->M - 1) * g->c_pitch * 4 + (long)g->Nn * 4);
   k.res_bytes = g->residual ? (unsigned)((g->M - 1) * g->res_pitch * 4 + (long)g->Nn * 4) : 0u;
+  k.res_mask = g->residual ? g->res_mask : nullptr, k.mask_bytes = k.res_mask ? (unsigned)(g->M * (g->Nn >> 2)) : 0u;
   k.b_sn = g->b_sn, k.b_sk = g->b_sk, k.M = (int)g->M, k.Nn = g->Nn, k.row_tiles = (int)((g->M + 31) / 32), k.relu = g->relu;
 
   const int slabs = g->Nn / 64, grid = 8 * slabs * std::max(1, 64 / slabs);
diff --git a/pinthememory_amd/hip/kernels.py b/pinthememory_amd/hip/kernels.py
--- a/pinthememory_amd/hip/kernels.py
+++ b/pinthememory_amd/hip/kernels.py
@@ -252,7 +252,7 @@
     return y
 
 
-def conv_bwd_data(dy, w_krsc, x_shape, stride, pad, dil, add=None, dtype=None):
+def conv_bwd_data(dy, w_krsc, x_shape, stride, pad, dil, add=None, dtype=None, add_mask=None):
     cout, kh, kw, cin = w_krsc.shape
     dx = new(x_shape, dy, dtype=dtype)
     dyd, dxd = tdesc(dy), tdesc(dx)
@@ -263,7 +263,10 @@
     ws = workspace(nb, dy.device) if nb else None
     ad = tdesc(add) if add is not None else None
     u_ent = _wino_u(p, w_krsc, nbu, dgrad=True) if CONV_PREC == 2 else None
-    check(lib.pm_conv_bwd_data(byref(dyd), w_krsc.data_ptr(), byref(dxd), byref(p), byref(ad) if ad else None, ptr(ws), nb, stream()), 'pm_conv_bwd_data')
+    if add_mask is not None:
+        check(lib.pm_conv_bwd_data_masked(byref(dyd), w_krsc.data_ptr(), byref(dxd), byref(p), byref(ad), add_mask.data_ptr(), ptr(ws), nb, stream()), 'pm_conv_bwd_data_masked')
+    else:
+        check(lib.pm_conv_bwd_data(byref(dyd), w_krsc.data_ptr(), byref(dxd), byref(p), byref(ad) if ad else None, ptr(ws), nb, stream()), 'pm_conv_bwd_data')
     if u_ent is not None:
         ent, version = u_ent
         cur = L.stream_obj()
@@ -372,6 +375,22 @@
     check(_lib().pm_bn_apply_mask(byref(tdesc(x)), mean.data_ptr(), invstd.data_ptr(), gamma.data_ptr(), beta.data_ptr(), byref(rd) if rd else None,
                                   1 if relu else 0, byref(tdesc(y)), ptr(mask), stream()), 'pm_bn_apply_mask')
     return (y, mask) if want_mask else y
+
+
+def bn_apply_res_affine(x, mean, invstd, gamma, beta, r, r_mean, r_invstd, r_gamma, r_beta, relu=False, want_mask=False):
+    y = torch.empty_like(x, memory_format=torch.contiguous_format)
+    mask = torch.empty((x.shape[0] * x.shape[1] * x.shape[2], x.shape[3] // 4), dtype=torch.uint8, device=x.device) if want_mask else None
+    check(_lib().pm_bn_apply_mask_affine(byref(tdesc(x)), mean.data_ptr(), invstd.data_ptr(), gamma.data_ptr(), beta.data_ptr(), byref(tdesc(r)), r_mean.data_ptr(),
+                                         r_invstd.data_ptr(), r_gamma.data_ptr(), r_beta.data_ptr(), 1 if relu else 0, byref(tdesc(y)), ptr(mask), stream()),
+          'pm_bn_apply_mask_affine')
+    return (y, mask) if want_mask else y
+
+
+def bn_bwd_apply_mask(dy, mask, x, mean, invstd, gamma, sums, count):
+    dx = torch.empty(x.shape, dtype=x.dtype, device=x.device)
+    check(_lib().pm_bn_bwd_apply_mask(byref(tdesc(dy)), mask.data_ptr(), byref(tdesc(x)), mean.data_ptr(), invstd.data_ptr(), gamma.data_ptr(), sums.data_ptr(),
+                                      float(count), byref(tdesc(dx)), stream()), 'pm_bn_bwd_apply_mask')
+    return dx
 
 
 def bn_bwd_reduce_mask(dy, mask, x, mean, invstd, want_gmask=True, with_count=False):
@@ -460,6 +479,34 @@
     arg = torch.empty(y.shape, dtype=torch.uint8, device=x.device)
     check(_lib().pm_maxpool3x3s2_fwd(byref(tdesc(x)), byref(tdesc(y)), arg.data_ptr(), stream()), 'pm_maxpool3x3s2_fwd')
     return y, arg
+
+
+def maxpool_bn_relu_fwd(x, mean, invstd, gamma, beta):
+    n, h, w, c = x.shape
+    y = torch.empty((n, (h - 1) // 2 + 1, (w - 1) // 2 + 1, c), dtype=x.dtype, device=x.device)
+    arg = torch.empty(y.shape, dtype=torch.uint8, device=x.device)
+    check(_lib().pm_maxpool3x3s2_bn_relu_fwd(byref(tdesc(x)), mean.data_ptr(), invstd.data_ptr(), gamma.data_ptr(), beta.data_ptr(), byref(tdesc(y)), arg.data_ptr(), stream()),
+          'pm_maxpool3x3s2_bn_relu_fwd')
+    return y, arg
+
+
+def bn_relu_bwd_pool(dyp, arg, x, mean, invstd, gamma, beta, with_count=False, reduce_sums=None):
+    c = x.shape[3]
+    sums = torch.empty(2 * c + (1 if with_count else 0), dtype=torch.float32, device=x.device)
+    if with_count:
+        sums[2 * c:].fill_(float(x.shape[0] * x.shape[1] * x.shape[2]))
+    xd, dd = tdesc(x), tdesc(dyp)
+    lib = _lib()
+    nb = _sizes(('bn', x.shape, x.dtype), lambda: lib.pm_bn_workspace(byref(xd)))
+    ws = workspace(nb, x.device)
+    check(lib.pm_bn_bwd_reduce_pool(byref(dd), arg.data_ptr(), byref(xd), mean.data_ptr(), invstd.data_ptr(), gamma.data_ptr(), beta.data_ptr(), sums.data_ptr(), ptr(ws), nb,
+                                    stream()), 'pm_bn_bwd_reduce_pool')
+    total = reduce_sums(sums) if reduce_sums is not None else sums
+    count = -1.0 if with_count else float(x.shape[0] * x.shape[1] * x.shape[2])
+    dx = torch.empty(x.shape, dtype=x.dtype, device=x.device)
+    check(lib.pm_bn_bwd_apply_pool(byref(dd), arg.data_ptr(), byref(xd), mean.data_ptr(), invstd.data_ptr(), gamma.data_ptr(), beta.data_ptr(), total.data_ptr(), count,
+                                   byref(tdesc(dx)), stream()), 'pm_bn_bwd_apply_pool')
+    return dx, sums
 
 
 def maxpool_bwd(dy, arg, x_shape):
diff --git a/pinthememory_amd/hip/lib.py b/pinthememory_amd/hip/lib.py
--- a/pinthememory_amd/hip/lib.py
+++ b/pinthememory_amd/hip/lib.py
@@ -70,6 +70,7 @@
     'pm_conv_workspace': (_sz, [_T, _T, _P, _i]),
     'pm_conv_fwd': (_i, [_T, _vp, _T, _P, _E, _vp, _sz, _vp]),
     'pm_conv_bwd_data': (_i, [_T, _vp, _T, _P, _T, _vp, _sz, _vp]),
+    'pm_conv_bwd_data_masked': (_i, [_T, _vp, _T, _P, _T, _vp, _vp, _sz, _vp]),
     'pm_conv_bwd_weight': (_i, [_T, _T, _vp, _vp, _P, _vp, _sz, _vp]),
     'pm_set_winograd': (_i, [_i]),
     'pm_set_winograd_fused': (_i, [_i]),
@@ -90,6 +91,8 @@
     'pm_bn_apply': (_i, [_T, _vp, _vp, _vp, _vp, _T, _i, _T, _vp]),
     'pm_bn_apply_mask': (_i, [_T, _vp, _vp, _vp, _vp, _T, _i, _T, _vp, _vp]),
     'pm_bn_bwd_reduce_mask': (_i, [_T, _vp, _T, _vp, _vp, _T, _vp, _vp, _sz, _vp]),
+    'pm_bn_apply_mask_affine': (_i, [_T, _vp, _vp, _vp, _vp, _T, _vp, _vp, _vp, _vp, _i, _T, _vp, _vp]),
+    'pm_bn_bwd_apply_mask': (_i, [_T, _vp, _T, _vp, _vp, _vp, _vp, _f, _T, _vp]),
     'pm_bn_bwd_reduce': (_i, [_T, _T, _T, _vp, _vp, _vp, _vp, _i, _T, _vp, _vp, _sz, _vp]),
     'pm_bn_bwd_apply': (_i, [_T, _T, _T, _vp, _vp, _vp, _vp, _vp, _f, _i, _T, _T, _vp]),
     'pm_relu_bwd': (_i, [_T, _T, _T, _vp]),
@@ -99,6 +102,9 @@
     'pm_scale_shift_act': (_i, [_T, _vp, _vp, _T, _i, _T, _vp]),
     'pm_maxpool3x3s2_fwd': (_i, [_T, _T, _vp, _vp]),
     'pm_maxpool3x3s2_bwd': (_i, [_T, _vp, _T, _vp]),
+    'pm_maxpool3x3s2_bn_relu_fwd': (_i, [_T, _vp, _vp, _vp, _vp, _T, _vp, _vp]),
+    'pm_bn_bwd_reduce_pool': (_i, [_T, _vp, _T, _vp, _vp, _vp, _vp, _vp, _vp, _sz, _vp]),
+    'pm_bn_bwd_apply_pool': (_i, [_T, _vp, _T, _vp, _vp, _vp, _vp, _vp, _f, _T, _vp]),
     'pm_global_avgpool_fwd': (_i, [_T, _T, _vp]),
     'pm_global_avgpool_bwd': (_i, [_T, _T, _i, _vp]),
     'pm_resize_bilinear_fwd': (_i, [_T, _T, _vp]),
diff --git a/pinthememory_amd/hip/ops.py b/pinthememory_amd/hip/ops.py
--- a/pinthememory_amd/hip/ops.py
+++ b/pinthememory_amd/hip/ops.py
@@ -185,7 +185,7 @@
             and len({y.shape[3] for y in ys}) == 1)
 
 
-def _bn_train_fwd(y, gamma, beta, bn, residual, relu, out=None, partials=None, want_mask=False):
+def _bn_train_stats(y, bn, partials=None):
     c = y.shape[3]
     pixels = y.shape[0] * y.shape[1] * y.shape[2]
     if bn.group is None and BN_FUSED_FINALIZE:
@@ -202,6 +202,11 @@
         if bn.group is not None:
             mom = D.merge_moments(mom, c, bn.group)
         mean, invstd = K.bn_finalize(mom, c, bn.eps, bn.running_mean, bn.running_var, bn.momentum)
+    return mean, invstd
+
+
+def _bn_train_fwd(y, gamma, beta, bn, residual, relu, out=None, partials=None, want_mask=False):
+    mean, invstd = _bn_train_stats(y, bn, partials)
     if want_mask:
         o, mask = K.bn_apply(y, mean, invstd, gamma, beta, residual=residual, relu=relu, out=out, want_mask=True)
         return o, mean, invstd, mask
@@ -228,6 +233,14 @@
     return dy, dres, local[c:2 * c], local[:c]
 
 
+def _bn_bwd_masked(dv, mask, y, mean, invstd, gamma, group):
+    c = y.shape[3]
+    local, _ = K.bn_bwd_reduce_mask(dv, mask, y, mean, invstd, want_gmask=False, with_count=group is not None)
+    sums = local if group is None else D.all_reduce_sum_copy(local, group)
+    count = float(y.shape[0] * y.shape[1] * y.shape[2]) if group is None else -1.0
+    return K.bn_bwd_apply_mask(dv, mask, y, mean, invstd, gamma, sums, count), local[c:2 * c], local[:c]
+
+
 class _Bottleneck(torch.autograd.Function):
 
     @staticmethod
@@ -246,15 +259,24 @@
             kd = K.krsc(wd)
             yd = K.conv_fwd(xv, kd, *geoms[3], bn_partials=ps)
             merged = _mergeable([bns[3], bns[2]], [yd, y3])
+            fold = y3.dtype == torch.float32 and yd.dtype == torch.float32
             if merged:
                 (md, idd), (m3, i3) = _bn_train_stats_multi([yd, y3], [bns[3], bns[2]], [ps[3], ps[2]])
-                res = K.bn_apply(yd, md, idd, gd, bd, residual=None, relu=False)
+                res = None if fold else K.bn_apply(yd, md, idd, gd, bd, residual=None, relu=False)
+            elif fold:
+                md, idd = _bn_train_stats(yd, bns[3], ps[3])
+                m3, i3 = _bn_train_stats(y3, bns[2], ps[2])
+                res = None
             else:
                 res, md, idd = _bn_train_fwd(yd, gd, bd, bns[3], None, False, partials=ps[3])
         else:
             kd = yd = md = idd = None
             res = xv
-        if merged:
+        if res is None:
+            out, mask3 = K.bn_apply_res_affine(y3, m3, i3, g3, b3, yd, md, idd, gd, bd, relu=True, want_mask=True)
+            if not RELU_MASK_BYTES:
+                mask3 = None
+        elif merged:
             out, mask3 = K.bn_apply(y3, m3, i3, g3, b3, residual=res, relu=True, want_mask=True) if RELU_MASK_BYTES else (K.bn_apply(y3, m3, i3, g3, b3, residual=res, relu=True), None)
         elif RELU_MASK_BYTES:
             out, m3, i3, mask3 = _bn_train_fwd(y3, g3, b3, bns[2], res, True, partials=ps[2], want_mask=True)
@@ -283,6 +305,9 @@
             dres, dg3, db3 = gm, s3[c3:2 * c3], s3[:c3]
             dyd, _ = K.bn_bwd_apply(gm, None, yd, md, idd, gd, gdsum, -1.0, 0, False, None)
             pair = (dyd, sd[c3:2 * c3], sd[:c3])
+        elif mask3 is not None and dv.dtype == torch.float32 and K.CONV_PREC != 2:
+            dy3, dg3, db3 = _bn_bwd_masked(dv, mask3, y3, m3, i3, g3, gr[2])
+            dres = None
         else:
             dy3, dres, dg3, db3 = _bn_train_bwd(dv, out, y3, m3, i3, g3, b3, True, gr[2], True, True, mask=mask3)
         dw3, _ = _wgrad(o2, dy3, tuple(k3.shape), ge[2], deferred=df[2])
@@ -293,16 +318,18 @@
         dy1, _, dg1, db1 = _bn_train_bwd(do1, o1, y1, m1, i1, g1, b1, True, gr[0], False, False)
         dw1, _ = _wgrad(xv, dy1, tuple(k1.shape), ge[0], deferred=df[0])
         dwd = dgd = dbd = None
-        skip = dres
+        skip, skip_mask = (dres, None) if dres is not None else (dv, mask3)
         if ctx.has_ds:
             if pair is not None:
                 dyd, dgd, dbd = pair
+            elif dres is None:
+                dyd, dgd, dbd = _bn_bwd_masked(dv, mask3, yd, md, idd, gd, gr[3])
             else:
                 dyd, _, dgd, dbd = _bn_train_bwd(dres, None, yd, md, idd, gd, None, False, gr[3], False, False)
             dwdk, _ = _wgrad(xv, dyd, tuple(kd.shape), ge[3], deferred=df[3])
             dwd = dwdk.permute(0, 3, 1, 2)
-            skip = K.conv_bwd_data(dyd, kd, tuple(xv.shape), *ge[3]) if ctx.needs_input_grad[0] else None
-        dx = nchw(K.conv_bwd_data(dy1, k1, tuple(xv.shape), *ge[0], add=skip)) if ctx.needs_input_grad[0] else None
+            skip, skip_mask = (K.conv_bwd_data(dyd, kd, tuple(xv.shape), *ge[3]) if ctx.needs_input_grad[0] else None), None
+        dx = nchw(K.conv_bwd_data(dy1, k1, tuple(xv.shape), *ge[0], add=skip, add_mask=skip_mask)) if ctx.needs_input_grad[0] else None
         p = lambda d: d.permute(0, 3, 1, 2)
         return dx, p(dw1), dg1, db1, p(dw2), dg2, db2, p(dw3), dg3, db3, dwd, dgd, dbd, None, None, None
 
@@ -409,6 +436,41 @@
         return dx, dw, db, dgamma, dbeta, (nchw(dres) if dres is not None else None), None, None, None, None, None
 
 
+class _Stem(torch.autograd.Function):
+
+    @staticmethod
+    def forward(ctx, x, w, gamma, beta, geom, bn):
+        xv, wk = nhwc(x), K.krsc(w)
+        kv, ps = [], []
+        y = K.conv_fwd(xv, wk, *geom, keep_v=kv if ctx.needs_input_grad[1] else None, bn_partials=ps)
+        mean, invstd = _bn_train_stats(y, bn, ps[0])
+        out, arg = K.maxpool_bn_relu_fwd(y, mean, invstd, gamma, beta)
+        ctx.geom, ctx.group = geom, bn.group
+        ctx.save_for_backward(xv, wk, y, mean, invstd, gamma, beta, arg, kv[0] if kv else None)
+        return nchw(out)
+
+    @staticmethod
+    def backward(ctx, dout):
+        xv, wk, y, mean, invstd, gamma, beta, arg, vk = ctx.saved_tensors
+        c = y.shape[3]
+        grp = ctx.group
+        dy, local = K.bn_relu_bwd_pool(_grad_view(dout), arg, y, mean, invstd, gamma, beta, with_count=grp is not None,
+                                       reduce_sums=(lambda s: D.all_reduce_sum_copy(s, grp)) if grp is not None else None)
+        dx = nchw(K.conv_bwd_data(dy, wk, tuple(xv.shape), *ctx.geom, dtype=xv.dtype)) if ctx.needs_input_grad[0] else None
+        dw = None
+        if ctx.needs_input_grad[1]:
+            dwk, _ = _wgrad(xv, dy, tuple(wk.shape), ctx.geom, wino_v=vk)
+            dw = dwk.permute(0, 3, 1, 2)
+        return dx, dw, local[c:2 * c], local[:c], None, None
+
+
+def stem_tail(x, w, conv, bn):
+    st = BNState(bn)
+    if st.training and torch.is_grad_enabled() and K.ACT_DTYPE == torch.float32 and x.dtype == torch.float32 and w.shape[0] % 4 == 0:
+        return _Stem.apply(x, w, bn.weight, bn.bias, _geom(conv), st)
+    return maxpool3x3s2(_ConvBnAct.apply(x, w, None, bn.weight, bn.bias, None, _geom(conv), st, True, None))
+
+
 class _ConvBnActN(torch.autograd.Function):
 
     @staticmethod
diff --git a/pinthememory_amd/network/Resnet.py b/pinthememory_amd/network/Resnet.py
--- a/pinthememory_amd/network/Resnet.py
+++ b/pinthememory_amd/network/Resnet.py
@@ -86,8 +86,7 @@
     from ..hip import kernels as K
     x4 = ops.nchw(K.nchw_to_nhwc(x.float(), c_pad=4)) if x.shape[1] == 3 else x
     w4 = F.pad(conv1.weight, (0, 0, 0, 0, 0, 4 - conv1.weight.shape[1])) if conv1.weight.shape[1] == 3 else conv1.weight
-    y = ops._ConvBnAct.apply(x4, w4, None, bn1.weight, bn1.bias, None, ops._geom(conv1), ops.BNState(bn1), True, None)
-    return ops.maxpool3x3s2(y)
+    return ops.stem_tail(x4, w4, conv1, bn1)
 
 
 def _pretrained(model, name):
```

After: 155.3, median of 6. +1.5%, better.
